# haliphinx/TCE-RVOS

Hardware: AMD Instinct MI355X
Metric: clips/s (T=5, 360×640, Swin-T) at 1/2/4/8 MI355X; mask IoU vs ref (higher is better)
Workload: dtype f32 (3xf16-split MFMA, f32 accumulate); 1 GPU; swin_t_p4w7 T=5 360x640 + 32-token text, B=1 clip per forward, flags --with_box_refine --binary --f_token 8 --qtrans (BASELINE config 2); clips_in_flight_per_gpu=1, clips_per_forward=1, same_clip_in_group=False, ranks_per_gpu=1, parallelism=clip-sharded x1

## Files before the change

### include/tce_rvos.h

```cpp
#ifndef TCE_RVOS_H
#define TCE_RVOS_H
#include <stdint.h>

#ifdef __cplusplus
extern "C" {
#endif

typedef void* tceStream;

int tce_abi_version(void);
const char* tce_last_error(void);

typedef struct {
  const float* A;
  const float* A2;
  const float* W;
  const float* bias;
  const float* res;
  float* C;
  int32_t M, N, K;
  int32_t lda, lda2, ldw, ldc, ldres;
  int32_t act, res_mode;
  int32_t batch;
  int64_t sA, sA2, sW, sBias, sC, sRes;
  int32_t conv;
  int32_t T, H, Wd, Cin, Ho, Wo, kh, kw, stride, pad;
} tceGemmArgs;
int tce_gemm_f32(const tceGemmArgs* args, tceStream stream);
int tce_gemm_splitk_f32(const tceGemmArgs* args, int32_t splits, float* workspace, tceStream stream);
int tce_gemm_splitk_ln_f32(const tceGemmArgs* args, int32_t splits, float* workspace, const float* gamma, const float* beta,
                           float eps, tceStream stream);
int tce_gemm_select_tile(int32_t M, int32_t N, int32_t batch);
int tce_gemm_select_tile_ex(int32_t M, int32_t N, int32_t K, int32_t batch, int32_t conv);
int tce_set_gemm_mode(int32_t mode);
int tce_get_gemm_mode(void);
int tce_set_gemm_mode_thread(int32_t mode);

int tce_set_range_flag(int32_t* flag);

int tce_layernorm_f32(const float* x, const float* r, const float* gamma, const float* beta, float* out,
                      int64_t M, int32_t C, float eps, tceStream stream);

int tce_groupnorm_nsplit(int32_t HW);
int tce_groupnorm_f32(const float* x, const float* gamma, const float* beta, float* out, float* ws, int32_t T,
                      int32_t HW, int32_t C, int32_t G, float eps, int32_t relu, tceStream stream);
int tce_groupnorm_up_add_f32(const float* x, const float* gamma, const float* beta, const float* add, float* out, float* ws,
                             int32_t T, int32_t h, int32_t w, int32_t ho, int32_t wo, int32_t C, int32_t G, float eps,
                             int32_t relu, tceStream stream);

int tce_resnet_stem_f32(const float* frames, const float* w_k64, const float* bias, float* out, int32_t T, int32_t H,
                        int32_t W, tceStream stream);
int tce_maxpool3x3s2_cl_f32(const float* x, float* out, int32_t T, int32_t H, int32_t W, int32_t C, tceStream stream);

int tce_patch_embed_f32(const float* frames, const float* w, const float* b, const float* gamma,
                        const float* beta, float* out, int32_t T, int32_t H, int32_t W, int32_t C, float eps,
                        tceStream stream);

int tce_window_attn_f32(const float* qkv, const float* qkv_bias, const float* bias_table, float* out, int32_t T,
                        int32_t H, int32_t W, int32_t C, int32_t nH, int32_t shift, tceStream stream);

int tce_window_attn3d_f32(const float* qkv, const float* qkv_bias, const float* bias_table, float* out, int32_t T,
                          int32_t H, int32_t W, int32_t C, int32_t nH, int32_t shifted, tceStream stream);

int tce_patch_merge_ln_f32(const float* x, const float* gamma, const float* beta, float* out, int32_t T, int32_t H,
                           int32_t W, int32_t C, float eps, tceStream stream);

int tce_mha_f32(const float* Q, const float* K, const float* V, float* O, int32_t batch, int32_t nheads,
                int32_t Lq, int32_t Lk, int32_t ldq, int32_t ldk, int32_t ldv, int32_t ldo, int64_t sQ, int64_t sK,
                int64_t sV, int64_t sO, const uint8_t* kmask, float scale, tceStream stream);

int64_t tce_mha_ws_bytes(int32_t batch, int32_t nheads, int32_t Lk);
int tce_mha_ws_f32(const float* Q, const float* K, const float* V, float* O, void* ws, int32_t batch, int32_t nheads,
                   int32_t Lq, int32_t Lk, int32_t ldq, int32_t ldk, int32_t ldv, int32_t ldo, int64_t sQ, int64_t sK,
                   int64_t sV, int64_t sO, const uint8_t* kmask, float scale, tceStream stream);

int tce_ms_deform_attn_forward_f32(const float* value, const int64_t* spatial_shapes, const int64_t* level_start_index,
                                   const float* sampling_loc, const float* attn_weight, float* out, int32_t N,
                                   int32_t S, int32_t M, int32_t D, int32_t Lq, int32_t L, int32_t P,
                                   tceStream stream);

int tce_ms_deform_attn_backward_f32(const float* value, const int64_t* spatial_shapes, const int64_t* level_start_index,
                                    const float* sampling_loc, const float* attn_weight, const float* grad_output,
                                    float* grad_value, float* grad_sampling_loc, float* grad_attn_weight, int32_t N,
                                    int32_t S, int32_t M, int32_t D, int32_t Lq, int32_t L, int32_t P, tceStream stream);

int tce_msda_fused_f32(const float* value, const float* proj, const float* ref, float* out,
                       const int32_t* shapes_hw , int32_t N, int32_t S, int32_t M, int32_t Lq,
                       int32_t L, int32_t P, int32_t ref_dim, int32_t ref_per_frame, tceStream stream);
int tce_msda_fused_valid_f32(const float* value, const float* proj, const float* ref, float* out,
                             const int32_t* shapes_hw, const int32_t* valid_hw, int32_t N, int32_t S, int32_t M, int32_t Lq,
                             int32_t L, int32_t P, int32_t ref_dim, int32_t ref_per_frame, tceStream stream);

int tce_msda_fewq_raw_f32(const float* src, const float* wv, const float* bv, const float* proj, const float* ref, float* out,
                          const int32_t* shapes_hw, const int32_t* valid_hw, int32_t N, int32_t S, int32_t M, int32_t Lq,
                          int32_t L, int32_t P, int32_t ref_dim, int32_t ref_per_frame, tceStream stream);

int tce_contrastive_f32(const float* memory, const float* sent, float* out, float* ws, int32_t T, int32_t S, int32_t C,
                        int32_t frames_per_clip, tceStream stream);

int tce_pos_sine2d_f32(float* out, const float* add, int32_t T, int32_t h, int32_t w, int32_t F, tceStream stream);
int tce_pos_sine2d_valid_f32(float* out, const float* add, int32_t T, int32_t h, int32_t w, int32_t F, int32_t hv, int32_t wv,
                             tceStream stream);

int tce_resize_nearest_f32(const float* in, const float* add, float* out, int32_t T, int32_t h, int32_t w, int32_t ho,
                           int32_t wo, int32_t C, tceStream stream);
int tce_resize_bilinear_f32(const float* in, const float* add, float* out, int32_t T, int32_t h, int32_t w,
                            int32_t ho, int32_t wo, int32_t C, tceStream stream);
int tce_resize_bilinear_ln_f32(const float* in, const float* add, const float* gamma, const float* beta, float eps, float* out,
                               int32_t T, int32_t h, int32_t w, int32_t ho, int32_t wo, int32_t C, tceStream stream);

int tce_add_f32(const float* a, const float* b, float* out, int64_t n, int64_t nb, tceStream stream);
int tce_tile_f32(const float* src, float* out, int64_t n_src, int64_t reps, tceStream stream);
int tce_sigmoid_f32(const float* x, float* out, int64_t n, tceStream stream);

#define TCE_COPY_MAX_SEGS 16
typedef struct tceCopySeg {
  const void* src;
  void* dst;
  int64_t rows, row_words, src_pitch_words;
} tceCopySeg;
int tce_copy_segments(const tceCopySeg* segs, int32_t n, tceStream stream);
int tce_box_refine_f32(const float* tmp, const float* ref, float* out, int32_t n, int32_t ref_dim, tceStream stream);

int tce_mask_pack_f32(const float* params, float* w0f, float* tail, int32_t nl, int32_t T, int32_t Q, int32_t Cm,
                      tceStream stream);
int tce_mask_tail_f32(const float* G, const float* tail, const float* refs , int32_t ref_ld,
                      float* masks, int32_t nl, int32_t T, int32_t Q, int32_t h, int32_t w, float img_h, float img_w,
                      int32_t stride_px, tceStream stream);

int tce_select_masks_u8(const float* logits, const float* masks, uint8_t* out, int32_t* best_query, int32_t T,
                        int32_t Q, int32_t K, int32_t h, int32_t w, int32_t H0, int32_t W0, float threshold,
                        tceStream stream);

int tce_resize_h_u8(const uint8_t* in, const int32_t* coef, const int32_t* bounds, uint8_t* tmp, int64_t rows,
                    int32_t Win, int32_t Wout, int32_t ksize, tceStream stream);
int tce_resize_v_norm_f32(const uint8_t* tmp, const int32_t* coef, const int32_t* bounds, const float* lut, float* out,
                          int32_t T, int32_t Hin, int32_t W, int32_t Hout, int32_t ksize, tceStream stream);

int tce_embed_ln_f32(const int64_t* ids, const int64_t* pos_ids, const float* word, const float* pos, const float* type0,
                     const float* gamma, const float* beta, float* out, int32_t L, int32_t C, float eps, int32_t pad_id,
                     tceStream stream);
int tce_embed_ln_seqs_f32(const int64_t* ids, const float* word, const float* pos, const float* type0, const float* gamma,
                          const float* beta, float* out, int32_t nseq, int32_t seq_len, int32_t C, float eps, int32_t pad_id,
                          tceStream stream);
int tce_mha_small64_f32(const float* qkv, float* out, int32_t L, int32_t nheads, float scale, tceStream stream);
int tce_tanh_f32(const float* x, float* out, int64_t n, tceStream stream);

int32_t tce_thin_linear_splits(int32_t M, int32_t N, int32_t K);
int tce_thin_partials_f32(const float* x, int64_t ldx, int32_t xsplits, const float* bias_x, int32_t act_x, const float* W,
                          int64_t ldw, float* ws, int32_t M, int32_t N, int32_t K, tceStream stream);
int tce_splitk_reduce_f32(const float* ws, int32_t splits, int32_t M, int32_t N, const float* bias, int32_t act, const float* res,
                          int32_t ldres, int32_t res_mode, float* C, int32_t ldc, const float* gamma, const float* beta, float eps,
                          tceStream stream);
int tce_mha_small64_splits_f32(const float* qkv_planes, int32_t splits, const float* bias, float* out, int32_t L, int32_t nheads,
                               float scale, tceStream stream);
int tce_mha_small64_seqs_f32(const float* qkv_planes, int32_t splits, const float* bias, float* out, int32_t nseq, int32_t L,
                             int32_t nheads, float scale, tceStream stream);
int tce_mha_small64_lens_f32(const float* qkv_planes, int32_t splits, const float* bias, float* out, int32_t nseq, int32_t L,
                             int32_t nheads, float scale, const int32_t* lens, tceStream stream);
int tce_caption_lens_f32(const int64_t* ids, int32_t nseq, int32_t Lmax, int32_t pad_id, int32_t D, int32_t* lens, uint8_t* kmask,
                         float* pos, tceStream stream);

int64_t tce_ffn_packed_bytes(int32_t C, int32_t Hd);
int tce_ffn_pack_f32(const float* W1, const float* b1, const float* W2, void* packed, int32_t C, int32_t Hd,
                     tceStream stream);
int tce_ffn_pack_batched_f32(const float* W1, const float* b1, const float* W2, void* packed, int32_t C, int32_t Hd,
                             int32_t batch, tceStream stream);
int tce_ffn_fused_f32(const float* x, int64_t ldx, const void* packed, const float* b2, const float* g_in,
                      const float* be_in, float eps_in, const float* g_out, const float* be_out, float eps_out,
                      float* out, int64_t ldo, int32_t M, int32_t C, int32_t Hd, int32_t act, tceStream stream);
int64_t tce_ffn_split_ws_floats(int32_t M, int32_t C, int32_t Hd, int32_t act);
int tce_ffn_set_wg_cap(int32_t cap);
int32_t tce_ffn_capped_grid(int32_t cap, int32_t batch, int32_t blocks, int32_t* persistent);
int32_t tce_ffn_split_counters(int32_t M, int32_t C, int32_t Hd, int32_t act);
int tce_ffn_fused_split_f32(const float* x, int64_t ldx, const void* packed, const float* b2, const float* g_in, const float* be_in,
                            float eps_in, const float* g_out, const float* be_out, float eps_out, float* out, int64_t ldo, int32_t M,
                            int32_t C, int32_t Hd, int32_t act, float* ws, int64_t ws_floats, int32_t* counters, int32_t n_counters,
                            tceStream stream);

typedef struct {
  const float* x;
  const float* a2;
  const void* packed;
  const float* bias;
  const float* res;
  float* out;
  const float *g_in, *be_in, *g_out, *be_out;
  int64_t ldx, lda2, ldres, ldo;
  int64_t sX, sA2, sRes, sOut;
  int32_t M, N, K, batch, a2_rows, act, res_mode;
  float eps_in, eps_out;
} tceRowLinArgs;
int64_t tce_rowlin_packed_bytes(int32_t N, int32_t K);
int tce_rowlin_pack_f32(const float* W, int64_t ldw, void* packed, int32_t N, int32_t K, tceStream stream);
int tce_rowlin_f32(const tceRowLinArgs* args, tceStream stream);

int64_t tce_conv3x3_packed_bytes(int32_t Cin, int32_t N);
int tce_conv3x3_pack_f32(const float* w, void* packed, int32_t Cin, int32_t N, tceStream stream);
int tce_conv3x3_f32(const float* x, int64_t ldx, const void* packed, const float* bias, float* out, int64_t ldo, int32_t T,
                    int32_t H, int32_t W, int32_t Cin, int32_t N, tceStream stream);
int64_t tce_conv3x3_split_ws_floats(int32_t M, int32_t Cin, int32_t N);
int32_t tce_conv3x3_split_pieces(int32_t M, int32_t Cin, int32_t N);
int32_t tce_conv3x3_split_kstep(int32_t pieces, int32_t s);
int tce_conv3x3_split_f32(const float* x, int64_t ldx, const void* packed, const float* bias, float* out, int64_t ldo, int32_t T,
                          int32_t H, int32_t W, int32_t Cin, int32_t N, float* ws, int64_t ws_floats, tceStream stream);

typedef struct {
  const float* x;
  const float* a2;
  const void* packed;
  const float* bo;
  const float* res;
  float* out;
  const float *g_out, *be_out;
  int64_t ldx, lda2, ldres, ldo;
  int64_t sX, sRes, sOut, sW;
  int32_t M, batch, a2_rows, res_mode, group;
  float eps_out;
  int32_t w_div;
} tceXattnArgs;
int tce_xattn_prepare_f32(const float* k, const float* v, const float* wqT_ext, const float* wo, float* W1, float* b1,
                          float* W2, int32_t L, int32_t group, int32_t batch, tceStream stream);
int tce_xattn_fused_f32(const tceXattnArgs* args, tceStream stream);

typedef struct {
  const void* packed;
  const float* b2;
  const float* g_out;
  const float* be_out;
  float* mid;
  int64_t ldmid, sMid;
  int32_t hidden, act;
  float eps_out;
} tceXattnFfnArgs;
int tce_ffn_pack_chain_f32(const float* W1, const float* b1, const float* W2, void* packed, int32_t C, int32_t Hd, tceStream stream);
int tce_xattn_ffn_fused_f32(const tceXattnArgs* args, const tceXattnFfnArgs* ffn, tceStream stream);
int tce_xattn_pack_f32(const float* k, const float* v, const float* wqT_ext, const float* wo, void* packed, int32_t L, int32_t group,
                       int32_t batch, tceStream stream);
int tce_xattn_prepare_lens_f32(const float* k, const float* v, const float* wqT_ext, const float* wo, float* W1, float* b1, float* W2,
                               int32_t L, int32_t group, int32_t batch, const int32_t* lens, tceStream stream);
int tce_xattn_pack_lens_f32(const float* k, const float* v, const float* wqT_ext, const float* wo, void* packed, int32_t L,
                            int32_t group, int32_t batch, const int32_t* lens, tceStream stream);

int64_t tce_swin_attn_packed_bytes(int32_t C);
int tce_swin_attn_pack_f32(const float* Wqkv, const float* Wproj, void* packed, int32_t C, tceStream stream);
int tce_swin_attn_fused_f32(const float* x, int64_t ldx, const void* packed, const float* qkv_bias, const float* proj_bias,
                            const float* bias_table, const float* gamma1, const float* beta1, float eps, float* out, int64_t ldo,
                            int32_t T, int32_t H, int32_t W, int32_t C, int32_t shift, tceStream stream);

int tce_graph_begin(tceStream stream);
int tce_graph_end(tceStream stream, void** graph_exec_out);
int tce_graph_launch(void* graph_exec, tceStream stream);
int tce_graph_destroy(void* graph_exec);
int tce_graph_group(void* const* graphs, int32_t n, void** graph_exec_out);

typedef struct {
  const float* W;
  const float* bias;
  float* out;
  int32_t N, ldw, ldo;
  int32_t use_a2;
  int32_t act;
} tceFewRowSeg;
typedef struct {
  const float* x;
  const float* a2;
  const float* res;
  int64_t ldx, lda2, ldres;
  int32_t a2_rows, R, K, nseg;
  tceFewRowSeg seg[3];
  const float* g_in;
  const float* be_in;
  float* xn_out;
  int64_t ldxn;
  float eps_in;
} tceFewRowArgs;
int tce_fewrow_linear_f32(const tceFewRowArgs* args, tceStream stream);

#ifdef __cplusplus
}
#endif
#endif
```

### tce-rvos_amd/_lib.py

```python
import ctypes as C
import os

HERE = os.path.dirname(os.path.abspath(__file__))
LIB_PATH = os.environ.get("TCE_LIB") or os.path.join(HERE, "lib", "libtce_rvos.so")

c_f = C.c_void_p
i32, i64, f32 = C.c_int32, C.c_int64, C.c_float


class GemmArgs(C.Structure):
    _fields_ = [("A", c_f), ("A2", c_f), ("W", c_f), ("bias", c_f), ("res", c_f), ("C", c_f),
                ("M", i32), ("N", i32), ("K", i32),
                ("lda", i32), ("lda2", i32), ("ldw", i32), ("ldc", i32), ("ldres", i32),
                ("act", i32), ("res_mode", i32), ("batch", i32),
                ("sA", i64), ("sA2", i64), ("sW", i64), ("sBias", i64), ("sC", i64), ("sRes", i64),
                ("conv", i32), ("T", i32), ("H", i32), ("Wd", i32), ("Cin", i32), ("Ho", i32), ("Wo", i32),
                ("kh", i32), ("kw", i32), ("stride", i32), ("pad", i32)]


class RowLinArgs(C.Structure):
    _fields_ = [("x", c_f), ("a2", c_f), ("packed", c_f), ("bias", c_f), ("res", c_f), ("out", c_f),
                ("g_in", c_f), ("be_in", c_f), ("g_out", c_f), ("be_out", c_f),
                ("ldx", i64), ("lda2", i64), ("ldres", i64), ("ldo", i64),
                ("sX", i64), ("sA2", i64), ("sRes", i64), ("sOut", i64),
                ("M", i32), ("N", i32), ("K", i32), ("batch", i32), ("a2_rows", i32), ("act", i32), ("res_mode", i32),
                ("eps_in", f32), ("eps_out", f32)]


class XattnArgs(C.Structure):
    _fields_ = [("x", c_f), ("a2", c_f), ("packed", c_f), ("bo", c_f), ("res", c_f), ("out", c_f),
                ("g_out", c_f), ("be_out", c_f),
                ("ldx", i64), ("lda2", i64), ("ldres", i64), ("ldo", i64),
                ("sX", i64), ("sRes", i64), ("sOut", i64), ("sW", i64),
                ("M", i32), ("batch", i32), ("a2_rows", i32), ("res_mode", i32), ("group", i32), ("eps_out", f32), ("w_div", i32)]



class XattnFfnArgs(C.Structure):
    _fields_ = [("packed", c_f), ("b2", c_f), ("g_out", c_f), ("be_out", c_f), ("mid", c_f), ("ldmid", i64), ("sMid", i64),
                ("hidden", i32), ("act", i32), ("eps_out", f32)]


class FewRowSeg(C.Structure):
    _fields_ = [("W", c_f), ("bias", c_f), ("out", c_f), ("N", i32), ("ldw", i32), ("ldo", i32), ("use_a2", i32), ("act", i32)]


class FewRowArgs(C.Structure):
    _fields_ = [("x", c_f), ("a2", c_f), ("res", c_f),
                ("ldx", i64), ("lda2", i64), ("ldres", i64),
                ("a2_rows", i32), ("R", i32), ("K", i32), ("nseg", i32), ("seg", FewRowSeg * 3),
                ("g_in", c_f), ("be_in", c_f), ("xn_out", c_f), ("ldxn", i64), ("eps_in", f32)]


class CopySeg(C.Structure):
    _fields_ = [("src", c_f), ("dst", c_f), ("rows", i64), ("row_words", i64), ("src_pitch_words", i64)]


class LabelObj(C.Structure):
    _fields_ = [("logits", c_f), ("masks", c_f)]


A2D_GROUP_MAX = 16


class A2dGroupSample(C.Structure):
    _fields_ = [("masks", c_f), ("logits", c_f), ("out", c_f), ("scores", c_f), ("fh", i32), ("fw", i32), ("H0", i32), ("W0", i32),
                ("logit_stride", i32), ("reserved", i32)]


REFEXP_GROUP_MAX = 16
REFEXP_MAX_CAND = 1024


class RefexpSample(C.Structure):
    _fields_ = [("logits", c_f), ("boxes_in", c_f), ("masks", c_f), ("scores", c_f), ("order", c_f), ("boxes_out", c_f), ("out", c_f),
                ("fh", i32), ("fw", i32), ("H0", i32), ("W0", i32)]


SIGNATURES = {
    "tce_abi_version": (i32, []),
    "tce_last_error": (C.c_char_p, []),
    "tce_gemm_f32": (i32, [C.POINTER(GemmArgs), c_f]),
    "tce_gemm_splitk_f32": (i32, [C.POINTER(GemmArgs), i32, c_f, c_f]),
    "tce_gemm_splitk_ln_f32": (i32, [C.POINTER(GemmArgs), i32, c_f, c_f, c_f, f32, c_f]),
    "tce_gemm_select_tile": (i32, [i32, i32, i32]),
    "tce_gemm_select_tile_ex": (i32, [i32, i32, i32, i32, i32]),
    "tce_set_gemm_mode": (i32, [i32]),
    "tce_set_gemm_mode_thread": (i32, [i32]),
    "tce_set_range_flag": (i32, [c_f]),
    "tce_get_gemm_mode": (i32, []),
    "tce_layernorm_f32": (i32, [c_f, c_f, c_f, c_f, c_f, i64, i32, f32, c_f]),
    "tce_groupnorm_nsplit": (i32, [i32]),
    "tce_groupnorm_f32": (i32, [c_f, c_f, c_f, c_f, c_f, i32, i32, i32, i32, f32, i32, c_f]),
    "tce_groupnorm_up_add_f32": (i32, [c_f, c_f, c_f, c_f, c_f, c_f, i32, i32, i32, i32, i32, i32, i32, f32, i32, c_f]),
    "tce_resnet_stem_f32": (i32, [c_f, c_f, c_f, c_f, i32, i32, i32, c_f]),
    "tce_maxpool3x3s2_cl_f32": (i32, [c_f, c_f, i32, i32, i32, i32, c_f]),
    "tce_resize_h_u8": (i32, [c_f, c_f, c_f, c_f, i64, i32, i32, i32, c_f]),
    "tce_resize_v_norm_f32": (i32, [c_f, c_f, c_f, c_f, c_f, i32, i32, i32, i32, i32, c_f]),
    "tce_patch_embed_f32": (i32, [c_f, c_f, c_f, c_f, c_f, c_f, i32, i32, i32, i32, f32, c_f]),
    "tce_window_attn_f32": (i32, [c_f, c_f, c_f, c_f, i32, i32, i32, i32, i32, i32, c_f]),
    "tce_window_attn3d_f32": (i32, [c_f, c_f, c_f, c_f, i32, i32, i32, i32, i32, i32, c_f]),
    "tce_patch_merge_ln_f32": (i32, [c_f, c_f, c_f, c_f, i32, i32, i32, i32, f32, c_f]),
    "tce_mha_f32": (i32, [c_f, c_f, c_f, c_f, i32, i32, i32, i32, i32, i32, i32, i32, i64, i64, i64, i64, c_f, f32, c_f]),
    "tce_mha_ws_bytes": (i64, [i32, i32, i32]),
    "tce_mha_ws_f32": (i32, [c_f, c_f, c_f, c_f, c_f, i32, i32, i32, i32, i32, i32, i32, i32, i64, i64, i64, i64, c_f, f32, c_f]),
    "tce_ms_deform_attn_forward_f32": (i32, [c_f, c_f, c_f, c_f, c_f, c_f, i32, i32, i32, i32, i32, i32, i32, c_f]),
    "tce_ms_deform_attn_backward_f32": (i32, [c_f, c_f, c_f, c_f, c_f, c_f, c_f, c_f, c_f, i32, i32, i32, i32, i32, i32, i32, c_f]),
    "tce_msda_fused_f32": (i32, [c_f, c_f, c_f, c_f, C.POINTER(i32), i32, i32, i32, i32, i32, i32, i32, i32, c_f]),
    "tce_msda_fused_valid_f32": (i32, [c_f, c_f, c_f, c_f, C.POINTER(i32), C.POINTER(i32), i32, i32, i32, i32, i32, i32, i32,
                                       i32, c_f]),
    "tce_msda_fewq_raw_f32": (i32, [c_f, c_f, c_f, c_f, c_f, c_f, C.POINTER(i32), C.POINTER(i32), i32, i32, i32, i32, i32, i32, i32,
                                    i32, c_f]),
    "tce_contrastive_f32": (i32, [c_f, c_f, c_f, c_f, i32, i32, i32, i32, c_f]),
    "tce_pos_sine2d_f32": (i32, [c_f, c_f, i32, i32, i32, i32, c_f]),
    "tce_pos_sine2d_valid_f32": (i32, [c_f, c_f, i32, i32, i32, i32, i32, i32, c_f]),
    "tce_resize_nearest_f32": (i32, [c_f, c_f, c_f, i32, i32, i32, i32, i32, i32, c_f]),
    "tce_resize_bilinear_f32": (i32, [c_f, c_f, c_f, i32, i32, i32, i32, i32, i32, c_f]),
    "tce_resize_bilinear_ln_f32": (i32, [c_f, c_f, c_f, c_f, f32, c_f, i32, i32, i32, i32, i32, i32, c_f]),
    "tce_add_f32": (i32, [c_f, c_f, c_f, i64, i64, c_f]),
    "tce_tile_f32": (i32, [c_f, c_f, i64, i64, c_f]),
    "tce_sigmoid_f32": (i32, [c_f, c_f, i64, c_f]),
    "tce_copy_segments": (i32, [C.POINTER(CopySeg), i32, c_f]),
    "tce_box_refine_f32": (i32, [c_f, c_f, c_f, i32, i32, c_f]),
    "tce_mask_pack_f32": (i32, [c_f, c_f, c_f, i32, i32, i32, i32, c_f]),
    "tce_mask_tail_f32": (i32, [c_f, c_f, c_f, i32, c_f, i32, i32, i32, i32, i32, f32, f32, i32, c_f]),
    "tce_select_masks_u8": (i32, [c_f, c_f, c_f, c_f, i32, i32, i32, i32, i32, i32, i32, f32, c_f]),
    "tce_embed_ln_f32": (i32, [c_f, c_f, c_f, c_f, c_f, c_f, c_f, c_f, i32, i32, f32, i32, c_f]),
    "tce_mha_small64_f32": (i32, [c_f, c_f, i32, i32, f32, c_f]),
    "tce_mha_small64_seqs_f32": (i32, [c_f, i32, c_f, c_f, i32, i32, i32, f32, c_f]),
    "tce_embed_ln_seqs_f32": (i32, [c_f, c_f, c_f, c_f, c_f, c_f, c_f, i32, i32, i32, f32, i32, c_f]),
    "tce_mha_small64_lens_f32": (i32, [c_f, i32, c_f, c_f, i32, i32, i32, f32, c_f, c_f]),
    "tce_caption_lens_f32": (i32, [c_f, i32, i32, i32, i32, c_f, c_f, c_f, c_f]),
    "tce_tanh_f32": (i32, [c_f, c_f, i64, c_f]),
    "tce_ffn_packed_bytes": (i64, [i32, i32]),
    "tce_ffn_pack_f32": (i32, [c_f, c_f, c_f, c_f, i32, i32, c_f]),
    "tce_ffn_fused_f32": (i32, [c_f, i64, c_f, c_f, c_f, c_f, f32, c_f, c_f, f32, c_f, i64, i32, i32, i32, i32, c_f]),
    "tce_ffn_split_ws_floats": (i64, [i32, i32, i32, i32]),
    "tce_ffn_split_counters": (i32, [i32, i32, i32, i32]),
    "tce_ffn_set_wg_cap": (i32, [i32]),
    "tce_ffn_capped_grid": (i32, [i32, i32, i32, C.POINTER(i32)]),
    "tce_ffn_fused_split_f32": (i32, [c_f, i64, c_f, c_f, c_f, c_f, f32, c_f, c_f, f32, c_f, i64, i32, i32, i32, i32, c_f, i64, c_f, i32, c_f]),
    "tce_xattn_prepare_f32": (i32, [c_f, c_f, c_f, c_f, c_f, c_f, c_f, i32, i32, i32, c_f]),
    "tce_ffn_pack_batched_f32": (i32, [c_f, c_f, c_f, c_f, i32, i32, i32, c_f]),
    "tce_xattn_fused_f32": (i32, [C.POINTER(XattnArgs), c_f]),
    "tce_xattn_ffn_fused_f32": (i32, [C.POINTER(XattnArgs), C.POINTER(XattnFfnArgs), c_f]),
    "tce_ffn_pack_chain_f32": (i32, [c_f, c_f, c_f, c_f, i32, i32, c_f]),
    "tce_xattn_pack_f32": (i32, [c_f, c_f, c_f, c_f, c_f, i32, i32, i32, c_f]),
    "tce_xattn_prepare_lens_f32": (i32, [c_f, c_f, c_f, c_f, c_f, c_f, c_f, i32, i32, i32, c_f, c_f]),
    "tce_xattn_pack_lens_f32": (i32, [c_f, c_f, c_f, c_f, c_f, i32, i32, i32, c_f, c_f]),
    "tce_rowlin_packed_bytes": (i64, [i32, i32]),
    "tce_rowlin_pack_f32": (i32, [c_f, i64, c_f, i32, i32, c_f]),
    "tce_rowlin_f32": (i32, [C.POINTER(RowLinArgs), c_f]),
    "tce_conv3x3_packed_bytes": (i64, [i32, i32]),
    "tce_conv3x3_pack_f32": (i32, [c_f, c_f, i32, i32, c_f]),
    "tce_conv3x3_f32": (i32, [c_f, i64, c_f, c_f, c_f, i64, i32, i32, i32, i32, i32, c_f]),
    "tce_conv3x3_split_ws_floats": (i64, [i32, i32, i32]),
    "tce_conv3x3_split_pieces": (i32, [i32, i32, i32]),
    "tce_conv3x3_split_kstep": (i32, [i32, i32]),
    "tce_conv3x3_split_f32": (i32, [c_f, i64, c_f, c_f, c_f, i64, i32, i32, i32, i32, i32, c_f, i64, c_f]),
    "tce_fewrow_linear_f32": (i32, [C.POINTER(FewRowArgs), c_f]),
    "tce_thin_linear_splits": (i32, [i32, i32, i32]),
    "tce_thin_partials_f32": (i32, [c_f, i64, i32, c_f, i32, c_f, i64, c_f, i32, i32, i32, c_f]),
    "tce_splitk_reduce_f32": (i32, [c_f, i32, i32, i32, c_f, i32, c_f, i32, i32, c_f, i32, c_f, c_f, f32, c_f]),
    "tce_mha_small64_splits_f32": (i32, [c_f, i32, c_f, c_f, i32, i32, f32, c_f]),
    "tce_swin_attn_packed_bytes": (i64, [i32]),
    "tce_swin_attn_pack_f32": (i32, [c_f, c_f, c_f, i32, c_f]),
    "tce_swin_attn_fused_f32": (i32, [c_f, i64, c_f, c_f, c_f, c_f, c_f, c_f, f32, c_f, i64, i32, i32, i32, i32, i32, c_f]),
    "tce_graph_begin": (i32, [c_f]),
    "tce_graph_end": (i32, [c_f, C.POINTER(C.c_void_p)]),
    "tce_graph_launch": (i32, [C.c_void_p, c_f]),
    "tce_graph_destroy": (i32, [C.c_void_p]),
    "tce_graph_group": (i32, [C.POINTER(C.c_void_p), i32, C.POINTER(C.c_void_p)]),
}

DEBUG_SIGNATURES = {
    "tce_gemm_force_tile": (i32, [i32]),
    "tce_debug_set_stamp_buffer": (i32, [c_f]),
    "tce_debug_set_epilogue": (i32, [i32]),
    "tce_debug_ffn_set_stamp_buffer": (i32, [c_f]),
    "tce_debug_ffn_set_half": (i32, [i32]),
    "tce_debug_msda_set_lds": (i32, [i32]),
    "tce_debug_window_attn_set_mfma": (i32, [i32]),
    "tce_debug_mha_set_split": (i32, [i32]),
    "tce_debug_msda_set_fewq": (i32, [i32]),
    "tce_debug_conv3x3_set_waves": (i32, [i32]),
    "tce_debug_conv3x3_set_pieces": (i32, [i32]),
}

VIDEO_SIGNATURES = {
    "tce_label_objects_u8": (i32, [C.POINTER(LabelObj), i32, c_f, c_f, i32, i32, i32, i32, i32, i32, i32, f32, f32, c_f]),
}

EVAL_SIGNATURES = {
    "tce_a2d_masks_u8": (i32, [c_f, c_f, i32, i32, i32, i32, i32, i32, i32, f32, c_f]),
    "tce_rle_ws_bytes": (i64, [i32, i32, i32]),
    "tce_rle_counts_u32": (i32, [c_f, c_f, c_f, c_f, i32, i32, i32, c_f]),
    "tce_a2d_group_masks_u8": (i32, [C.POINTER(A2dGroupSample), i32, i32, i32, i32, f32, c_f]),
}

SCORE_SIGNATURES = {
    "tce_jf_ws_bytes": (i64, [i32, i32, i32, i32, i32]),
    "tce_jf_counts_i32": (i32, [c_f, c_f, c_f, c_f, i32, i32, i32, i32, i32, c_f]),
    "tce_rle_decode_ws_bytes": (i64, [i32, i32, i32, i32]),
    "tce_rle_decode_u8": (i32, [c_f, c_f, c_f, c_f, i32, i32, i32, i32, c_f]),
    "tce_mask_overlap_ws_bytes": (i64, [i32, i32, i32]),
    "tce_mask_overlap_i32": (i32, [c_f, c_f, c_f, c_f, i32, i32, i32, c_f]),
}

PNG_SIGNATURES = {
    "tce_png_stream_bound": (i64, [i32, i32, i32]),
    "tce_png_ws_bytes": (i64, [i32, i32, i32, i32]),
    "tce_png_deflate_u8": (i32, [c_f, c_f, c_f, c_f, i32, i32, i32, i32, i32, c_f]),
    "tce_png_deflate_dyn_u8": (i32, [c_f, c_f, c_f, c_f, i32, i32, i32, i32, i32, c_f]),
}

VIS_SIGNATURES = {
    "tce_vis_overlay_u8": (i32, [c_f, c_f, c_f, c_f, c_f, c_f, i32, i32, i32, i32, c_f]),
    "tce_png_filter_rgb_u8": (i32, [c_f, c_f, i32, i32, i32, c_f]),
    "tce_png_deflate_rows_u8": (i32, [c_f, c_f, c_f, c_f, i32, i32, i32, i32, c_f]),
}

PNGFILE_SIGNATURES = {
    "tce_png_file_bound": (i64, [i32, i64]),
    "tce_png_file_ws_bytes": (i64, [i32, i64]),
    "tce_png_file_u8": (i32, [c_f, c_f, c_f, i32, c_f, c_f, c_f, i32, i64, i64, c_f]),
}

REFEXP_SIGNATURES = {
    "tce_refexp_group_u8": (i32, [C.POINTER(RefexpSample), i32, i32, i32, i32, i32, f32, c_f]),
    "tce_refexp_giou_f32": (i32, [c_f, c_f, c_f, c_f, i32, i32, c_f]),
}

HEADERS = {"tce_rvos.h": SIGNATURES, "tce_rvos_debug.h": DEBUG_SIGNATURES, "tce_rvos_video.h": VIDEO_SIGNATURES,
           "tce_rvos_eval.h": EVAL_SIGNATURES, "tce_rvos_score.h": SCORE_SIGNATURES, "tce_rvos_png.h": PNG_SIGNATURES,
           "tce_rvos_vis.h": VIS_SIGNATURES, "tce_rvos_pngfile.h": PNGFILE_SIGNATURES, "tce_rvos_refexp.h": REFEXP_SIGNATURES}

_LIB = None


class TceError(RuntimeError):
    pass


def lib():
    global _LIB
    if _LIB is None:
        if not os.path.exists(LIB_PATH):
            raise TceError(f"{LIB_PATH} not found: build the HIP extension first "
                           f"(python -c 'import __graft_entry__ as g; g.build()'); there is no fallback path")
        hwq = os.environ.get("GPU_MAX_HW_QUEUES")
        if hwq not in (None, "", "4"):
            import warnings
            warnings.warn(f"tce_rvos_amd: GPU_MAX_HW_QUEUES={hwq} is set; the HIP runtime's default (4) is the only value this "
                          f"launch program runs well with (1-3 crash the runtime, 5-16 double the clip time)", RuntimeWarning)
        l = C.CDLL(LIB_PATH)
        for name, (res, args) in [kv for table in HEADERS.values() for kv in table.items()]:
            fn = getattr(l, name)
            fn.restype, fn.argtypes = res, args
        _LIB = l
    return _LIB


def lib_raw():
    l = lib()
    return l.__dict__.get("_real", l)


def check(status, what=""):
    if status != 0:
        msg = lib().tce_last_error().decode(errors="replace")
        raise TceError(f"{what} failed ({status}): {msg}")
```

### tce-rvos_amd/csrc/conv3x3.hip

```cpp
#include "common.h"
#include "gemm_epilogue.h"
#include "frag.h"
#include "tiles.h"
#include "../../include/tce_rvos.h"
#include "../../include/tce_rvos_debug.h"

namespace {

constexpr int CONV_PAD_STAGES = 6;

struct ConvArgs {
  const float* x;
  const unsigned char* wpk;
  const float* bias;
  float* out;
  long long ldx, ldo;
  int H, W, M;
  int* range_flag;
  int single;
  int m_off;
  int nb, pieces;
  float* ws;
};

constexpr int CONV_ITERS = 12;
__host__ __device__ constexpr int conv3x3_piece_iter(const int pieces, const int s) { return s * CONV_ITERS / pieces; }

#ifndef CONV_ABL
#define CONV_ABL 0
#endif

template <int BYTE_OFF>
__device__ __forceinline__ void gload16(f32x4& dst, const float* ptr) {
  asm volatile("global_load_dwordx4 %0, %1, off offset:%2" : "=v"(dst) : "v"(ptr), "n"(BYTE_OFF) : "memory");
}

template <int CIN, bool SINGLE, int WAVES = 4, bool SPLIT = false>
__global__ void __launch_bounds__(64 * WAVES, WAVES / 4) conv3x3_kernel(const ConvArgs p) {
  constexpr int NTL = 8;
  constexpr int PW = 16 / WAVES;
  constexpr int STAGE = 2 * NTL * PIECE;
  constexpr int R = 4;
  constexpr int XS = WAVES == 4 ? 6 : 4, LX = XS + 1;
  constexpr int NW = WAVES == 4 ? CONV_PAD_STAGES - 2 : 3, LW = NW + 2;
  constexpr int INFLIGHT = (2 + PW) * (LW - 3);
  static_assert(LW <= CONV_PAD_STAGES, "the packed stream's zero padding covers the weight lead");
  constexpr int BODY = 12;
  constexpr int ITERS = 3 * (CIN / 64);
  constexpr int KS = BODY * ITERS;
  static_assert(CIN % 64 == 0, "channel chunks come in groups of four");
  static_assert(BODY % R == 0 && BODY % XS == 0 && BODY % NW == 0 && LX >= LW, "ring positions are compile-time");
  static_assert(WAVES * WT_BYTES <= R * STAGE, "the epilogue's staging tiles alias the ring");
  static_assert(!SPLIT || (ITERS == CONV_ITERS && WAVES == 4 && !SINGLE), "split pieces: CIN = 256, 128-pixel workgroups, split fp16");
  __shared__ __attribute__((aligned(16))) unsigned char smem[R * STAGE];

  const int tid = threadIdx.x, lane = tid & 63;
  const int wave = __builtin_amdgcn_readfirstlane(tid >> 6);
  const int hf = lane >> 5;
  const int blk = SPLIT ? (int)blockIdx.x % p.nb : (int)blockIdx.x;
  const int piece = SPLIT ? (int)blockIdx.x / p.nb : 0;
  const int i0 = SPLIT ? conv3x3_piece_iter(p.pieces, piece) : 0;
  const int i1 = SPLIT ? conv3x3_piece_iter(p.pieces, piece + 1) : ITERS;
  const int m0 = p.m_off + blk * (32 * WAVES) + wave * 32;

  const int m = m0 + (lane & 31);
  const int px = m % p.W, py = (m / p.W) % p.H;
  const float* const zeros = reinterpret_cast<const float*>(p.wpk + (long long)(KS + CONV_PAD_STAGES) * STAGE) + 8 * hf;
  const float* const xme = p.x + (long long)min(m, p.M - 1) * p.ldx + 8 * hf;
  auto iter_ptrs = [&](const int it, const float* (&q)[3]) {
    const int dy = it / (CIN / 64) - 1, cq = it % (CIN / 64);
    const bool row_ok = it < i1 && m < p.M && (unsigned)(py + dy) < (unsigned)p.H;
#pragma unroll
    for (int d = 0; d < 3; ++d) {
      const bool ok = row_ok && (unsigned)(px + d - 1) < (unsigned)p.W;
      q[d] = (ok ? xme + (long long)(dy * p.W + d - 1) * p.ldx : zeros) + 64 * cq;
    }
  };

  const float* wp = reinterpret_cast<const float*>(p.wpk + ((long long)i0 * BODY * STAGE) + (long long)(PW * wave) * PIECE + lane * 16);
  unsigned char* const wdst = smem + (PW * wave) * PIECE + lane * 16;
  f32x4 wr[NW][PW];
  auto wload = [&](f32x4 (&dst)[PW]) {
    if (!(CONV_ABL & 8)) {
      gload16<0>(dst[0], wp);
      gload16<PIECE>(dst[1], wp);
      if constexpr (PW == 4) {
        gload16<2 * PIECE>(dst[2], wp);
        gload16<3 * PIECE>(dst[3], wp);
      }
    }
    wp += STAGE / 4;
  };
  auto wstore = [&](const f32x4 (&src)[PW], const int stage) {
#pragma unroll
    for (int q = 0; q < PW; ++q) *reinterpret_cast<f32x4*>(wdst + stage * STAGE + q * PIECE) = src[q];
  };

  f32x4 xr[XS][2];
  const float* cur[3];
  const float* nxt[3];
  iter_ptrs(i0, cur);
  iter_ptrs(i0 + 1, nxt);
  auto xload = [&](auto jjc, f32x4 (&dst)[2]) {
    constexpr int JJ = decltype(jjc)::value;
    constexpr int J = JJ % BODY;
    const float* const src = JJ < BODY ? cur[J % 3] : nxt[J % 3];
    if (CONV_ABL & 16) return;
    gload16<64 * (J / 3)>(dst[0], src);
    gload16<64 * (J / 3) + 16>(dst[1], src);
  };
  auto wait_loads = [&](auto nc, f32x4 (&xs)[2], f32x4 (&ws)[PW]) {
    constexpr int N = (CONV_ABL & 24) ? 0 : decltype(nc)::value;
    if constexpr (PW == 4) {
      asm volatile("s_waitcnt vmcnt(%6)"
                   : "+v"(xs[0]), "+v"(xs[1]), "+v"(ws[0]), "+v"(ws[1]), "+v"(ws[2]), "+v"(ws[3])
                   : "n"(N)
                   : "memory");
    } else {
      asm volatile("s_waitcnt vmcnt(%4)" : "+v"(xs[0]), "+v"(xs[1]), "+v"(ws[0]), "+v"(ws[1]) : "n"(N) : "memory");
    }
  };
  using nfl = std::integral_constant<int, INFLIGHT>;

  f32x16 acc[NTL];
#pragma unroll
  for (int t = 0; t < NTL; ++t)
#pragma unroll
    for (int i = 0; i < 16; ++i) acc[t][i] = 0.f;
  h16x8 bh, bl;
  static_for<0, LX>([&](auto mc) {
    constexpr int m = decltype(mc)::value - LX;
    if constexpr (m + 2 >= 0) {
      wait_loads(nfl{}, xr[(m + 2) % XS], wr[(m + 2) % NW]);
      wstore(wr[(m + 2) % NW], (m + 2) % R);
      if constexpr (m + 2 == 0) {
        const float f[8] = {xr[0][0][0], xr[0][0][1], xr[0][0][2], xr[0][0][3], xr[0][1][0], xr[0][1][1], xr[0][1][2], xr[0][1][3]};
        const HL b = split8(f, SINGLE ? 1 : 0);
        bh = b.hi;
        bl = b.lo;
        asm volatile("" : "+v"(bh), "+v"(bl));
      }
    }
    if constexpr (m + LX >= 0) xload(std::integral_constant<int, m + LX>{}, xr[(m + LX) % XS]);
    if constexpr (m + LW >= 0) wload(wr[(m + LW) % NW]);
  });
  __syncthreads();
  h16x8 fh[4], fl[4];
  {
    const unsigned char* const st = smem + lane * 16;
    fh[0] = *reinterpret_cast<const h16x8*>(st);
    fl[0] = *reinterpret_cast<const h16x8*>(st + PIECE);
    fh[1] = *reinterpret_cast<const h16x8*>(st + 2 * PIECE);
    fl[1] = *reinterpret_cast<const h16x8*>(st + 3 * PIECE);
  }

  for (int it = i0; it < i1; ++it) {
    static_for<0, BODY>([&](auto jc) {
      constexpr int j = decltype(jc)::value;
      constexpr int nslot = (j + 1) % XS;
      const unsigned char* const st = smem + (j % R) * STAGE + lane * 16;
      unsigned nh[4], nl[4];
      auto tile = [&](auto tc) {
        constexpr int t = decltype(tc)::value;
#if CONV_ABL & 4
        const h16x8 k0 = fh[t % 4], k1 = fl[t % 4], k2 = bh, k3 = bl;
        asm volatile("" : : "v"(k0), "v"(k1), "v"(k2), "v"(k3));
#else
        if constexpr (!SINGLE) {
          acc[t] = __builtin_amdgcn_mfma_f32_32x32x16_f16(fh[t % 4], bl, acc[t], 0, 0, 0);
          acc[t] = __builtin_amdgcn_mfma_f32_32x32x16_f16(fl[t % 4], bh, acc[t], 0, 0, 0);
        }
        acc[t] = __builtin_amdgcn_mfma_f32_32x32x16_f16(fh[t % 4], bh, acc[t], 0, 0, 0);
#endif
      };
      static_for<0, 6>([&](auto tc) {
        constexpr int t = decltype(tc)::value;
        fh[(t + 2) % 4] = *reinterpret_cast<const h16x8*>(st + (2 * t + 4) * PIECE);
        fl[(t + 2) % 4] = *reinterpret_cast<const h16x8*>(st + (2 * t + 5) * PIECE);
        __builtin_amdgcn_sched_barrier(0);
        tile(tc);
        if constexpr (t < 4) {
          const float a = xr[nslot][t >> 1][2 * (t & 1)], b = xr[nslot][t >> 1][2 * (t & 1) + 1];
          if constexpr (SINGLE) {
            nh[t] = __builtin_bit_cast(unsigned, fp16x2_t{(__fp16)a, (__fp16)b});
            nl[t] = 0u;
          } else {
            const fp16x2_t h = __builtin_amdgcn_cvt_pkrtz(a, b);
            nh[t] = __builtin_bit_cast(unsigned, h);
            nl[t] = __builtin_bit_cast(unsigned, __builtin_amdgcn_cvt_pkrtz(a - (float)h[0], b - (float)h[1]));
          }
          asm volatile("" : "+v"(nh[t]), "+v"(nl[t]));
        }
        __builtin_amdgcn_sched_barrier(0);
      });
      wait_loads(nfl{}, xr[(j + 2) % XS], wr[(j + 2) % NW]);
      wstore(wr[(j + 2) % NW], (j + 2) % R);
      if (!(CONV_ABL & 2)) __syncthreads();
      xload(std::integral_constant<int, j + LX>{}, xr[(j + LX) % XS]);
      wload(wr[(j + LW) % NW]);
      {
        const unsigned char* const sn = smem + ((j + 1) % R) * STAGE + lane * 16;
        fh[0] = *reinterpret_cast<const h16x8*>(sn);
        fl[0] = *reinterpret_cast<const h16x8*>(sn + PIECE);
        fh[1] = *reinterpret_cast<const h16x8*>(sn + 2 * PIECE);
        fl[1] = *reinterpret_cast<const h16x8*>(sn + 3 * PIECE);
      }
      __builtin_amdgcn_sched_barrier(0);
      tile(std::integral_constant<int, 6>{});
      tile(std::integral_constant<int, 7>{});
      __builtin_amdgcn_sched_barrier(0);
      bh = __builtin_bit_cast(h16x8, u32x4{nh[0], nh[1], nh[2], nh[3]});
      bl = __builtin_bit_cast(h16x8, u32x4{nl[0], nl[1], nl[2], nl[3]});
    });
#pragma unroll
    for (int d = 0; d < 3; ++d) cur[d] = nxt[d];
    iter_ptrs(it + 2, nxt);
  }
  asm volatile("s_waitcnt vmcnt(0)" ::: "memory");
  __syncthreads();

  float* const wt = reinterpret_cast<float*>(smem + wave * WT_BYTES);
  tce_amax_t amax = 0;
  if constexpr (SPLIT) {
    float* const part = p.ws + (long long)piece * (p.M - p.m_off) * 256;
#pragma unroll
    for (int t = 0; t < NTL; ++t) tile_store(acc[t], part, 256, m0 - p.m_off, p.M - p.m_off, 32 * t, wt, lane, amax);
    return;
  }
  const ResTile none = {};
#pragma unroll
  for (int t = 0; t < NTL; ++t) {
    tile_bias_res<0>(acc[t], tile_bias_load(p.bias, 32 * t, lane), none, wt, lane);
    tile_store(acc[t], p.out, p.ldo, m0, p.M, 32 * t, wt, lane, amax);
  }
  tce_range_report(p.range_flag, amax);
}

__global__ void __launch_bounds__(256) conv3x3_reduce_kernel(const float* __restrict__ ws, const int pieces, const int rows,
                                                             const float* __restrict__ bias, float* __restrict__ out,
                                                             const long long ldo, const int m_off, int* range_flag) {
  const long long n4 = (long long)rows * 64, stride = (long long)gridDim.x * 256;
  tce_amax_t amax = 0;
  for (long long i = (long long)blockIdx.x * 256 + threadIdx.x; i < n4; i += stride) {
    const f32x4* src = reinterpret_cast<const f32x4*>(ws) + i;
    f32x4 v = src[0];
    for (int s = 1; s < pieces; ++s) v += src[(long long)s * n4];
    const int c4 = (int)(i & 63);
    if (bias) v += reinterpret_cast<const f32x4*>(bias)[c4];
    amax = tce_amax4(amax, v);
    *reinterpret_cast<f32x4*>(out + (m_off + (i >> 6)) * ldo + 4 * c4) = v;
  }
  tce_range_report(range_flag, amax);
}

__global__ void __launch_bounds__(256) conv3x3_pack_kernel(const float* __restrict__ w, unsigned char* __restrict__ out,
                                                           const int CIN, const long long units, const int single) {
  const long long u = (long long)blockIdx.x * 256 + threadIdx.x;
  if (u >= units) return;
  const int lane = (int)(u & 63);
  const long long pg = u >> 6;
  const int piece = (int)(pg & 15);
  const long long s = pg >> 4;
  const int r = lane & 31, hf = lane >> 5, t = piece >> 1;
  u32x4 o = {0u, 0u, 0u, 0u};
  if (s < 9 * CIN / 16) {
    const int it = (int)(s / 12), j = (int)(s % 12);
    const int dy = it / (CIN / 64), cc = 4 * (it % (CIN / 64)) + j / 3, dx = j % 3;
    float v[8];
#pragma unroll
    for (int e = 0; e < 8; ++e) v[e] = w[(long long)(32 * t + r) * (9 * CIN) + (3 * dy + dx) * CIN + 16 * cc + 8 * hf + e];
    const HL f = split8(v, single);
    o = __builtin_bit_cast(u32x4, (piece & 1) ? f.lo : f.hi);
  }
  reinterpret_cast<u32x4*>(out)[u] = o;
}

inline bool conv3x3_shape_ok(int Cin, int N) { return Cin == 256 && N == 256; }
inline long long conv3x3_units(int Cin) { return (long long)(9 * Cin / 16 + CONV_PAD_STAGES) * 16 * 64 + 128; }

}

extern "C" int64_t tce_conv3x3_packed_bytes(int32_t Cin, int32_t N) { return conv3x3_shape_ok(Cin, N) ? conv3x3_units(Cin) * 16 : -1; }

extern "C" int tce_conv3x3_pack_f32(const float* w, void* packed, int32_t Cin, int32_t N, tceStream stream) {
  TCE_CHECK_ARG(conv3x3_shape_ok(Cin, N), "tce_conv3x3_pack_f32: unsupported shape Cin=%d N=%d (256 -> 256)", Cin, N);
  TCE_CHECK_ARG(w && packed && tce_aligned16(packed), "tce_conv3x3_pack_f32: null / misaligned pointer");
  const long long units = conv3x3_units(Cin);
  hipLaunchKernelGGL(conv3x3_pack_kernel, dim3(tce_cdiv(units, 256)), dim3(256), 0, (hipStream_t)stream, w,
                     (unsigned char*)packed, Cin, units, tce_gemm_single_pass());
  TCE_CHECK_LAUNCH("tce_conv3x3_pack_f32");
  return TCE_OK;
}

static int g_conv3_waves = 0;
extern "C" int tce_debug_conv3x3_set_waves(int32_t waves) {
  TCE_CHECK_ARG(waves == 0 || waves == 4 || waves == 8, "tce_debug_conv3x3_set_waves: 0 (automatic), 4 or 8");
  g_conv3_waves = waves;
  return TCE_OK;
}

struct Conv3Plan {
  int wide = 4;
  int full8 = 0;
  int m_narrow = 0;
  int nb = 0;
  int pieces = 1;
  long long ws_floats = 0;
};
inline Conv3Plan conv3x3_plan(const int M, const int cus, const int single, const int force_waves, const int split, const int force_pieces) {
  Conv3Plan pl;
  const int r4 = tce_cdiv(tce_cdiv(M, 128), cus), r8 = tce_cdiv(tce_cdiv(M, 256), cus);
  const int full8 = tce_cdiv(M, 256) / cus;
  const int rem_px = M - full8 * 256 * cus;
  const int mixed4 = 7 * full8 + 4 * tce_cdiv(tce_cdiv(rem_px, 128), cus);
  if (!force_waves && !single && full8 >= 1 && rem_px > 0 && mixed4 < 4 * r4 && mixed4 < 7 * r8) {
    pl.full8 = full8 * cus;
    pl.m_narrow = full8 * 256 * cus;
  } else {
    pl.wide = force_waves ? force_waves : (4 * r4 > 7 * r8 ? 8 : 4);
    if (single) pl.wide = 4;
    if (pl.wide == 8) return pl;
  }
  pl.nb = tce_cdiv(M - pl.m_narrow, 128);
  if (!split || single || pl.nb >= cus) return pl;
  const double OVH = 0.5, LAUNCH = 0.3, RED_BPI = 8.0 * (3u << 20);
  const long long px = M - pl.m_narrow;
  auto cost = [&](int p) {
    const double walk = (double)tce_cdiv((long long)pl.nb * p, cus) * (tce_cdiv(CONV_ITERS, p) + OVH);
    return p == 1 ? walk : walk + LAUNCH + (double)(p + 1) * px * 1024.0 / RED_BPI;
  };
  int best = 1;
  for (int p = 2; p <= 6; ++p)
    if ((long long)pl.nb * p <= 2ll * cus && cost(p) < cost(best)) best = p;
  if (force_pieces > 0) best = force_pieces;
  if (best > 1) {
    pl.pieces = best;
    pl.ws_floats = (long long)best * px * 256;
  }
  return pl;
}

static int g_conv3_pieces = 0;
extern "C" int tce_debug_conv3x3_set_pieces(int32_t pieces) {
  TCE_CHECK_ARG(pieces >= 0 && pieces <= CONV_ITERS, "tce_debug_conv3x3_set_pieces: 0 (automatic) .. 12");
  g_conv3_pieces = pieces;
  return TCE_OK;
}

static int conv3_force_waves() {
  static const int env_force = []() { const char* e = getenv("TCE_CONV3_WAVES"); return e ? atoi(e) : 0; }();
  return g_conv3_waves ? g_conv3_waves : env_force;
}

static Conv3Plan conv3x3_plan_for(const int M, const bool split) {
  return conv3x3_plan(M, tce_cu_count(), tce_gemm_single_pass(), conv3_force_waves(), split, g_conv3_pieces);
}

extern "C" int64_t tce_conv3x3_split_ws_floats(int32_t M, int32_t Cin, int32_t N) {
  return conv3x3_shape_ok(Cin, N) && M > 0 ? conv3x3_plan_for(M, true).ws_floats : 0;
}
extern "C" int32_t tce_conv3x3_split_pieces(int32_t M, int32_t Cin, int32_t N) {
  return conv3x3_shape_ok(Cin, N) && M > 0 ? conv3x3_plan_for(M, true).pieces : 0;
}
extern "C" int32_t tce_conv3x3_split_kstep(int32_t pieces, int32_t s) {
  return pieces >= 1 && pieces <= CONV_ITERS && s >= 0 && s <= pieces ? 12 * conv3x3_piece_iter(pieces, s) : -1;
}

static int conv3x3_launch(const float* x, int64_t ldx, const void* packed, const float* bias, float* out, int64_t ldo, int32_t T,
                          int32_t H, int32_t W, int32_t Cin, int32_t N, float* ws, int64_t ws_floats, const bool split, tceStream stream,
                          const char* name) {
  TCE_CHECK_ARG(conv3x3_shape_ok(Cin, N), "%s: unsupported shape Cin=%d N=%d (256 -> 256)", name, Cin, N);
  TCE_CHECK_ARG(x && packed && out && T > 0 && H > 0 && W > 0 && (long long)T * H * W < (1ll << 31),
                "%s: null pointer or bad sizes", name);
  TCE_CHECK_ARG(ldx >= Cin && ldx % 4 == 0 && ldo >= N && ldo % 4 == 0, "%s: bad row pitch", name);
  TCE_CHECK_ARG(tce_aligned16(x) && tce_aligned16(out) && tce_aligned16(packed) && (!bias || tce_aligned16(bias)),
                "%s: pointers must be 16-byte aligned", name);
  ConvArgs a;
  a.x = x; a.wpk = (const unsigned char*)packed; a.bias = bias; a.out = out;
  a.ldx = ldx; a.ldo = ldo; a.H = H; a.W = W; a.M = T * H * W;
  a.range_flag = tce_range_flag(); a.single = tce_gemm_single_pass();
  a.m_off = 0; a.nb = 0; a.pieces = 1; a.ws = nullptr;
  hipStream_t s = (hipStream_t)stream;
  const Conv3Plan pl = conv3x3_plan_for(a.M, split);
  if (pl.pieces > 1)
    TCE_CHECK_ARG(ws && tce_aligned16(ws) && ws_floats >= pl.ws_floats,
                  "%s: workspace of %lld floats needed (tce_conv3x3_split_ws_floats), %lld given", name, pl.ws_floats, (long long)ws_floats);
  if (pl.full8) hipLaunchKernelGGL((conv3x3_kernel<256, false, 8>), dim3(pl.full8), dim3(512), 0, s, a);
  a.m_off = pl.m_narrow;
  if (pl.wide == 8) hipLaunchKernelGGL((conv3x3_kernel<256, false, 8>), dim3(tce_cdiv(a.M, 256)), dim3(512), 0, s, a);
  else if (a.single) hipLaunchKernelGGL((conv3x3_kernel<256, true>), dim3(pl.nb), dim3(256), 0, s, a);
  else if (pl.pieces == 1) hipLaunchKernelGGL((conv3x3_kernel<256, false>), dim3(pl.nb), dim3(256), 0, s, a);
  else {
    a.nb = pl.nb; a.pieces = pl.pieces; a.ws = ws;
    hipLaunchKernelGGL((conv3x3_kernel<256, false, 4, true>), dim3(pl.nb * pl.pieces), dim3(256), 0, s, a);
    const int rows = a.M - a.m_off;
    hipLaunchKernelGGL(conv3x3_reduce_kernel, dim3(std::min(tce_cdiv((long long)rows * 64, 256), 8 * tce_cu_count())), dim3(256), 0, s,
                       (const float*)ws, pl.pieces, rows, bias, out, ldo, a.m_off, a.range_flag);
  }
  TCE_CHECK_LAUNCH(name);
  return TCE_OK;
}

extern "C" int tce_conv3x3_f32(const float* x, int64_t ldx, const void* packed, const float* bias, float* out, int64_t ldo,
                               int32_t T, int32_t H, int32_t W, int32_t Cin, int32_t N, tceStream stream) {
  return conv3x3_launch(x, ldx, packed, bias, out, ldo, T, H, W, Cin, N, nullptr, 0, false, stream, "tce_conv3x3_f32");
}

extern "C" int tce_conv3x3_split_f32(const float* x, int64_t ldx, const void* packed, const float* bias, float* out, int64_t ldo,
                                     int32_t T, int32_t H, int32_t W, int32_t Cin, int32_t N, float* ws, int64_t ws_floats,
                                     tceStream stream) {
  return conv3x3_launch(x, ldx, packed, bias, out, ldo, T, H, W, Cin, N, ws, ws_floats, true, stream, "tce_conv3x3_split_f32");
}
```

### tce-rvos_amd/csrc/norm.hip

```cpp
#include "common.h"
#include "gemm_epilogue.h"
#include "../../include/tce_rvos.h"

namespace {

__global__ void __launch_bounds__(256) layernorm_kernel(const float* __restrict__ x, const float* __restrict__ r,
                                                        const float* __restrict__ gamma,
                                                        const float* __restrict__ beta, float* __restrict__ out,
                                                        long long M, int C, float eps) {
  const int lane = threadIdx.x & 63;
  const long long row = (long long)blockIdx.x * 4 + (threadIdx.x >> 6);
  if (row >= M) return;
  const f32x4* xr = reinterpret_cast<const f32x4*>(x + row * C);
  const f32x4* rr = r ? reinterpret_cast<const f32x4*>(r + row * C) : nullptr;
  const int n4 = C >> 2;
  float s = 0.f;
  for (int i = lane; i < n4; i += 64) {
    f32x4 v = xr[i];
    if (rr) v += rr[i];
    s += (v[0] + v[1]) + (v[2] + v[3]);
  }
  const float mean = wave_sum(s) / (float)C;
  float q = 0.f;
  for (int i = lane; i < n4; i += 64) {
// ... 401 lines not shown
        sMean[g] = mean;
        sRstd[g] = rsqrtf(m2 / n + eps);
      }
    }
  }
  __syncthreads();
  for (int c = threadIdx.x; c < C; c += 256) {
    const int g = c / cg;
    const float mean = sMean[g], rstd = sRstd[g];
    const float sc = rstd * gamma[c];
    scale[c] = sc;
    shift[c] = beta[c] - mean * sc;
  }
  __syncthreads();
}

__global__ void __launch_bounds__(256) groupnorm_apply_kernel(const float* __restrict__ x,
                                                              const float* __restrict__ ws,
                                                              const float* __restrict__ gamma,
                                                              const float* __restrict__ beta, float* __restrict__ out,
                                                              int HW, int C, int G, int relu, int rows_per_block,
                                                              int nsplit, float eps) {
  extern __shared__ float sm[];
  float* scale = sm;
  float* shift = sm + C;
  const int t = blockIdx.y;
  groupnorm_scale_shift(ws, gamma, beta, scale, shift, t, C, G, nsplit, eps);
  const int c4 = C >> 2;
  const long long r0 = (long long)blockIdx.x * rows_per_block;
  const long long r1 = min((long long)HW, r0 + rows_per_block);
  const f32x4* x4 = reinterpret_cast<const f32x4*>(x + (long long)t * HW * C);
  f32x4* o4 = reinterpret_cast<f32x4*>(out + (long long)t * HW * C);
  const f32x4* sc4 = reinterpret_cast<const f32x4*>(scale);
  const f32x4* sh4 = reinterpret_cast<const f32x4*>(shift);
  for (long long i = r0 * c4 + threadIdx.x; i < r1 * c4; i += 256) {
    const int c = (int)(i % c4);
    const f32x4 v = x4[i], a = sc4[c], b = sh4[c];
    f32x4 o;
#pragma unroll
    for (int j = 0; j < 4; ++j) {
      o[j] = v[j] * a[j] + b[j];
      if (relu) o[j] = fmaxf(o[j], 0.f);
    }
    o4[i] = o;
  }
}

__global__ void __launch_bounds__(256) groupnorm_apply_up_kernel(const float* __restrict__ x, const float* __restrict__ ws,
                                                                 const float* __restrict__ gamma, const float* __restrict__ beta,
                                                                 const float* add, float* out, int h, int w, int ho, int wo,
                                                                 int C, int G, int relu, int rows_per_block, int nsplit, float eps) {
  extern __shared__ float sm[];
  float* scale = sm;
  float* shift = sm + C;
  const int t = blockIdx.y;
  groupnorm_scale_shift(ws, gamma, beta, scale, shift, t, C, G, nsplit, eps);
  const int c4 = C >> 2;
  const long long HWo = (long long)ho * wo;
  const long long r0 = (long long)blockIdx.x * rows_per_block;
  const long long r1 = min(HWo, r0 + rows_per_block);
  const f32x4* x4 = reinterpret_cast<const f32x4*>(x + (long long)t * h * w * C);
  const f32x4* a4 = reinterpret_cast<const f32x4*>(add + (long long)t * HWo * C);
  f32x4* o4 = reinterpret_cast<f32x4*>(out + (long long)t * HWo * C);
  const f32x4* sc4 = reinterpret_cast<const f32x4*>(scale);
  const f32x4* sh4 = reinterpret_cast<const f32x4*>(shift);
  const float sy = (float)h / (float)ho, sx = (float)w / (float)wo;
  for (long long i = r0 * c4 + threadIdx.x; i < r1 * c4; i += 256) {
    const int c = (int)(i % c4);
    const int ro = (int)(i / c4);
    const int yo = ro / wo, xo = ro - yo * wo;
    const int yi = min((int)floorf((float)yo * sy), h - 1), xi = min((int)floorf((float)xo * sx), w - 1);
    const f32x4 v = x4[((long long)yi * w + xi) * c4 + c], a = sc4[c], b = sh4[c];
    f32x4 o;
#pragma unroll
    for (int j = 0; j < 4; ++j) {
      o[j] = v[j] * a[j] + b[j];
      if (relu) o[j] = fmaxf(o[j], 0.f);
    }
    o += a4[i];
    o4[i] = o;
  }
}


}

extern "C" int tce_layernorm_f32(const float* x, const float* r, const float* gamma, const float* beta, float* out,
                                 int64_t M, int32_t C, float eps, tceStream stream) {
  TCE_CHECK_ARG(x && gamma && beta && out, "tce_layernorm_f32: null pointer");
  TCE_CHECK_ARG(M > 0 && C > 0 && C % 4 == 0, "tce_layernorm_f32: need M>0, C%%4==0 (M=%lld C=%d)", (long long)M, C);
  TCE_CHECK_ARG(tce_aligned16(x) && tce_aligned16(out) && tce_aligned16(gamma) && tce_aligned16(beta) &&
                    (!r || tce_aligned16(r)),
                "tce_layernorm_f32: pointers must be 16-byte aligned");
  if (C <= 128)
    hipLaunchKernelGGL(layernorm_reg_kernel<32>, dim3(tce_cdiv(M, 8)), dim3(256), 0, (hipStream_t)stream, x, r, gamma, beta,
                       out, (long long)M, C, eps);
  else if (C <= 256)
    hipLaunchKernelGGL(layernorm_reg_kernel<64>, dim3(tce_cdiv(M, 4)), dim3(256), 0, (hipStream_t)stream, x, r, gamma, beta,
                       out, (long long)M, C, eps);
  else
    hipLaunchKernelGGL(layernorm_kernel, dim3(tce_cdiv(M, 4)), dim3(256), 0, (hipStream_t)stream, x, r, gamma, beta, out,
                     (long long)M, C, eps);
  TCE_CHECK_LAUNCH("tce_layernorm_f32");
  return TCE_OK;
}

extern "C" int tce_patch_merge_ln_f32(const float* x, const float* gamma, const float* beta, float* out, int32_t T,
                                      int32_t H, int32_t W, int32_t C, float eps, tceStream stream) {
  TCE_CHECK_ARG(x && gamma && beta && out, "tce_patch_merge_ln_f32: null pointer");
  TCE_CHECK_ARG(T > 0 && H > 0 && W > 0 && C > 0 && C % 4 == 0, "tce_patch_merge_ln_f32: bad shape");
  TCE_CHECK_ARG(tce_aligned16(x) && tce_aligned16(out) && tce_aligned16(gamma) && tce_aligned16(beta),
                "tce_patch_merge_ln_f32: pointers must be 16-byte aligned");
  const long long rows = (long long)T * ((H + 1) / 2) * ((W + 1) / 2);
  hipLaunchKernelGGL(patch_merge_ln_kernel, dim3(tce_cdiv(rows, 4)), dim3(256), 0, (hipStream_t)stream, x, gamma, beta,
                     out, T, H, W, C, eps);
  TCE_CHECK_LAUNCH("tce_patch_merge_ln_f32");
  return TCE_OK;
}

extern "C" int tce_patch_embed_f32(const float* frames, const float* w, const float* b, const float* gamma,
                                   const float* beta, float* out, int32_t T, int32_t H, int32_t W, int32_t C, float eps,
                                   tceStream stream) {
  TCE_CHECK_ARG(frames && w && b && gamma && beta && out, "tce_patch_embed_f32: null pointer");
  TCE_CHECK_ARG(T > 0 && H > 0 && W > 0 && C > 0 && C <= 256, "tce_patch_embed_f32: need 0 < C <= 256 (C=%d)", C);
  const int Hp = (H + 3) / 4, Wp = (W + 3) / 4;
  const long long ntok = (long long)T * Hp * Wp;
  if (tce_get_gemm_mode() != 0 &&
      tce_patch_embed_mfma(frames, w, b, gamma, beta, out, H, W, C, eps, ntok, Hp, Wp, (hipStream_t)stream)) {
    TCE_CHECK_LAUNCH("tce_patch_embed_f32");
    return TCE_OK;
  }
  int* const rf = tce_get_gemm_mode() != 0 ? tce_range_flag() : nullptr;
  if (C % 8 == 0 && C <= 120 && tce_aligned16(frames) && tce_aligned16(out) && tce_aligned16(gamma) && tce_aligned16(beta)) {
    constexpr int TOK = 128;
    const size_t lds = (size_t)(TOK * (C + 4) + 2 * TOK) * sizeof(float);
    hipLaunchKernelGGL((patch_embed_lane_kernel<8, TOK>), dim3(tce_cdiv(ntok, TOK)), dim3(TOK), lds, (hipStream_t)stream, frames, w, b,
                       gamma, beta, out, H, W, C, eps, ntok, Hp, Wp, rf);
    TCE_CHECK_LAUNCH("tce_patch_embed_f32");
    return TCE_OK;
  }
  const int tpb = 64;
  const size_t smem = (size_t)(48 * C + 4 * 48) * sizeof(float);
  hipLaunchKernelGGL((patch_embed_kernel<4>), dim3(tce_cdiv(ntok, tpb)), dim3(256), smem, (hipStream_t)stream, frames, w,
                     b, gamma, beta, out, T, H, W, C, eps, tpb, rf);
  TCE_CHECK_LAUNCH("tce_patch_embed_f32");
  return TCE_OK;
}

static int groupnorm_rows_per(int HW) { return HW >= 4096 ? 128 : (HW >= 512 ? 32 : 8); }
extern "C" int tce_groupnorm_nsplit(int32_t HW) { return tce_cdiv(HW, groupnorm_rows_per(HW)); }

static void groupnorm_stats_launch(const float* x, float* ws, int T, int HW, int C, int G, hipStream_t s);

extern "C" int tce_groupnorm_up_add_f32(const float* x, const float* gamma, const float* beta, const float* add, float* out,
                                        float* ws, int32_t T, int32_t h, int32_t w, int32_t ho, int32_t wo, int32_t C, int32_t G,
                                        float eps, int32_t relu, tceStream stream) {
  TCE_CHECK_ARG(x && gamma && beta && add && out && ws, "tce_groupnorm_up_add_f32: null pointer");
  TCE_CHECK_ARG(T > 0 && h > 0 && w > 0 && ho > 0 && wo > 0 && C > 0 && G > 0 && G <= 64 && C % G == 0 && C % 4 == 0,
                "tce_groupnorm_up_add_f32: bad shape (G <= 64)");
  TCE_CHECK_ARG(tce_aligned16(x) && tce_aligned16(out) && tce_aligned16(add), "tce_groupnorm_up_add_f32: x/add/out must be 16-byte aligned");
  TCE_CHECK_ARG(x != out, "tce_groupnorm_up_add_f32: out may alias add, not x");
  const int HW = h * w, nsplit = tce_cdiv(HW, groupnorm_rows_per(HW));
  hipStream_t s = (hipStream_t)stream;
  groupnorm_stats_launch(x, ws, T, HW, C, G, s);
  const int rows_per_block = 64;
  hipLaunchKernelGGL(groupnorm_apply_up_kernel, dim3(tce_cdiv(ho * wo, rows_per_block), T), dim3(256), (size_t)2 * C * sizeof(float), s,
                     x, ws, gamma, beta, add, out, h, w, ho, wo, C, G, relu, rows_per_block, nsplit, eps);
  TCE_CHECK_LAUNCH("tce_groupnorm_up_add_f32");
  return TCE_OK;
}

static void groupnorm_stats_launch(const float* x, float* ws, int T, int HW, int C, int G, hipStream_t s) {
  const int rows_per = groupnorm_rows_per(HW), nsplit = tce_cdiv(HW, rows_per);
  if (C == 256 && (G == 8 || G == 16 || G == 32 || G == 64)) {
    const dim3 grid(nsplit, T);
    if (rows_per == 128) hipLaunchKernelGGL(groupnorm_stats_rows_kernel<32>, grid, dim3(256), 0, s, x, ws, HW, G, rows_per, nsplit);
    else if (rows_per == 32) hipLaunchKernelGGL(groupnorm_stats_rows_kernel<8>, grid, dim3(256), 0, s, x, ws, HW, G, rows_per, nsplit);
    else hipLaunchKernelGGL(groupnorm_stats_rows_kernel<2>, grid, dim3(256), 0, s, x, ws, HW, G, rows_per, nsplit);
  } else {
    hipLaunchKernelGGL(groupnorm_stats_kernel, dim3(T * G, nsplit), dim3(256), 0, s, x, ws, HW, C, G, nsplit);
  }
}

extern "C" int tce_groupnorm_f32(const float* x, const float* gamma, const float* beta, float* out, float* ws, int32_t T,
                                 int32_t HW, int32_t C, int32_t G, float eps, int32_t relu, tceStream stream) {
  TCE_CHECK_ARG(x && gamma && beta && out && ws, "tce_groupnorm_f32: null pointer");
  TCE_CHECK_ARG(T > 0 && HW > 0 && C > 0 && G > 0 && G <= 64 && C % G == 0 && C % 4 == 0, "tce_groupnorm_f32: bad shape (G <= 64)");
  TCE_CHECK_ARG(tce_aligned16(x) && tce_aligned16(out), "tce_groupnorm_f32: x/out must be 16-byte aligned");
  const int rows_per = groupnorm_rows_per(HW), nsplit = tce_cdiv(HW, rows_per);
  hipStream_t s = (hipStream_t)stream;
  if (C == 256 && (G == 8 || G == 16 || G == 32 || G == 64)) {
    const dim3 grid(nsplit, T);
    if (rows_per == 128) hipLaunchKernelGGL(groupnorm_stats_rows_kernel<32>, grid, dim3(256), 0, s, x, ws, HW, G, rows_per, nsplit);
    else if (rows_per == 32) hipLaunchKernelGGL(groupnorm_stats_rows_kernel<8>, grid, dim3(256), 0, s, x, ws, HW, G, rows_per, nsplit);
    else hipLaunchKernelGGL(groupnorm_stats_rows_kernel<2>, grid, dim3(256), 0, s, x, ws, HW, G, rows_per, nsplit);
  } else {
    hipLaunchKernelGGL(groupnorm_stats_kernel, dim3(T * G, nsplit), dim3(256), 0, s, x, ws, HW, C, G, nsplit);
  }
  const int rows_per_block = 64;
  hipLaunchKernelGGL(groupnorm_apply_kernel, dim3(tce_cdiv(HW, rows_per_block), T), dim3(256),
                     (size_t)2 * C * sizeof(float), s, x, ws, gamma, beta, out, HW, C, G, relu, rows_per_block, nsplit, eps);
  TCE_CHECK_LAUNCH("tce_groupnorm_f32");
  return TCE_OK;
}
```

### tce-rvos_amd/hazard.py

```python
import contextlib
import traceback

import numpy as np
import torch

from . import _lib

F = 4


def strided(ptr, run_bytes, *dims):
    if not ptr or run_bytes <= 0 or any(c <= 0 for c, _ in dims):
        return np.zeros((0, 2), dtype=np.int64)
    starts = np.array([int(ptr)], dtype=np.int64)
    for count, stride in dims:
        if count == 1 or stride == 0:
            continue
        starts = (starts[:, None] + (np.arange(int(count), dtype=np.int64) * int(stride))[None, :]).reshape(-1)
    iv = np.stack([starts, starts + int(run_bytes)], 1)
    return merge(iv)


def dense(ptr, nbytes):
    return strided(ptr, int(nbytes))
# ... 50 lines not shown

def _table(ptr, what):
    n = TABLES.get(_p(ptr))
    if n is None:
        raise RuntimeError(f"hazard checker: the extent of {what} at {_p(ptr):#x} is unknown (hazard.recording(tables=...))")
    return dense(_p(ptr), n)


def _gemm(g, ws=None, splits=1, ln=None):
    b = max(1, g.batch)
    if g.conv:
        rd = [dense(_p(g.A), g.T * g.H * g.Wd * g.Cin * F)]
    else:
        rd = [strided(_p(g.A), g.K * F, (b, g.sA * F), (g.M, g.lda * F))]
        if g.A2:
            rd.append(strided(_p(g.A2), g.K * F, (b, g.sA2 * F), (g.M, g.lda2 * F)))
    rd.append(strided(_p(g.W), g.K * F, (b, g.sW * F), (g.N, g.ldw * F)))
    if g.bias:
        rd.append(strided(_p(g.bias), g.N * F, (b, g.sBias * F)))
    if g.res and g.res_mode:
        rd.append(strided(_p(g.res), g.N * F, (b, g.sRes * F), (g.M, g.ldres * F)))
    wr = [strided(_p(g.C), g.N * F, (b, g.sC * F), (g.M, g.ldc * F))]
    if ws:
        w = dense(_p(ws), splits * g.M * g.N * F)
        rd.append(w)
        wr.append(w)
    if ln:
        rd += [dense(_p(ln[0]), g.N * F), dense(_p(ln[1]), g.N * F)]
    return rd, wr


def _rowlin(q):
    b = max(1, q.batch)
    L = _lib.lib_raw()
    rd = [strided(_p(q.x), q.K * F, (b, q.sX * F), (q.M, q.ldx * F)),
          dense(_p(q.packed), L.tce_rowlin_packed_bytes(q.N, q.K))]
    if q.a2:
        rd.append(strided(_p(q.a2), q.K * F, (b, q.sA2 * F), (q.a2_rows if q.a2_rows > 0 else q.M, q.lda2 * F)))
    if q.bias:
        rd.append(dense(_p(q.bias), q.N * F))
    if q.res and q.res_mode:
        rd.append(strided(_p(q.res), q.N * F, (b, q.sRes * F), (q.M, q.ldres * F)))
    for g_, n in ((q.g_in, q.K), (q.be_in, q.K), (q.g_out, q.N), (q.be_out, q.N)):
        if g_:
            rd.append(dense(_p(g_), n * F))
    return rd, [strided(_p(q.out), q.N * F, (b, q.sOut * F), (q.M, q.ldo * F))]


def _xattn(q):
    b = max(1, q.batch)
    L = _lib.lib_raw()
    nb = L.tce_ffn_packed_bytes(256, 8 * q.group)
    wd = q.w_div if q.w_div > 0 else 1
    rd = [strided(_p(q.x), 256 * F, (b, q.sX * F), (q.M, q.ldx * F)),
          strided(_p(q.packed), nb, ((b + wd - 1) // wd if q.sW else 1, q.sW)), dense(_p(q.bo), 256 * F)]
    if q.a2:
        rd.append(strided(_p(q.a2), 256 * F, (q.a2_rows if q.a2_rows > 0 else q.M, q.lda2 * F)))
    if q.res:
        rd.append(strided(_p(q.res), 256 * F, (b, q.sRes * F), (q.M, q.ldres * F)))
    for g_ in (q.g_out, q.be_out):
        if g_:
            rd.append(dense(_p(g_), 256 * F))
    return rd, [strided(_p(q.out), 256 * F, (b, q.sOut * F), (q.M, q.ldo * F))]


def _xattn_ffn(q, f):
    rd, wr = _xattn(q)
    b = max(1, q.batch)
    rd += [dense(_p(f.packed), _lib.lib_raw().tce_ffn_packed_bytes(256, f.hidden)), dense(_p(f.b2), 256 * F)]
    for g_ in (f.g_out, f.be_out):
        if g_:
            rd.append(dense(_p(g_), 256 * F))
    wr.append(strided(_p(f.mid), 256 * F, (b, f.sMid * F), (q.M, f.ldmid * F)))
    return rd, wr


def _fewrow(q):
    rd = [strided(_p(q.x), q.K * F, (q.R, q.ldx * F))]
    wr = []
    use_a2 = False
    for i in range(q.nseg):
        sg = q.seg[i]
        rd.append(strided(_p(sg.W), q.K * F, (sg.N, sg.ldw * F)))
        if sg.bias:
            rd.append(dense(_p(sg.bias), sg.N * F))
        wr.append(strided(_p(sg.out), sg.N * F, (q.R, sg.ldo * F)))
        use_a2 = use_a2 or bool(sg.use_a2)
    if q.a2 and use_a2:
        rd.append(strided(_p(q.a2), q.K * F, (q.a2_rows if q.a2_rows > 0 else q.R, q.lda2 * F)))
    if q.res:
        rd.append(strided(_p(q.res), q.seg[0].N * F, (q.R, q.ldres * F)))
    if q.g_in:
        rd += [dense(_p(q.g_in), q.K * F), dense(_p(q.be_in), q.K * F)]
        if q.xn_out:
            wr.append(strided(_p(q.xn_out), q.K * F, (q.R, q.ldxn * F)))
    return rd, wr


def _mha(Q, K, V, O, ws, batch, nh, Lq, Lk, ldq, ldk, ldv, ldo, sQ, sK, sV, sO, kmask):
    run = nh * 32 * F
    rd = [strided(_p(Q), run, (batch, sQ * F), (Lq, ldq * F)), strided(_p(K), run, (batch, sK * F), (Lk, ldk * F)),
          strided(_p(V), run, (batch, sV * F), (Lk, ldv * F))]
    if kmask:
        rd.append(dense(_p(kmask), batch * Lk))
    wr = [strided(_p(O), run, (batch, sO * F), (Lq, ldo * F))]
    if ws:
        w = dense(_p(ws), _lib.lib_raw().tce_mha_ws_bytes(batch, nh, Lk))
        rd.append(w)
        wr.append(w)
    return rd, wr


def _msda(value, proj, ref, out, N, S, M, Lq, L, P, ref_dim, ref_per_frame):
    return ([dense(_p(value), N * S * M * 32 * F), dense(_p(proj), N * Lq * M * L * P * 3 * F),
             dense(_p(ref), (N if ref_per_frame else 1) * Lq * ref_dim * F)], [dense(_p(out), N * Lq * M * 32 * F)])


def _copy_segments(a):
    segs, n = a[0], a[1]
    rd, wr = [], []
    for i in range(n):
        sg = segs[i]
        rd.append(strided(_p(sg.src), sg.row_words * 4, (sg.rows, sg.src_pitch_words * 4)))
        wr.append(dense(_p(sg.dst), sg.rows * sg.row_words * 4))
    return rd, wr


def _ffn_fused(a):
    x, ldx, packed, b2, g_in, be_in, _, g_out, be_out, _, out, ldo, M, Cn, Hd = a[:15]
    rd = [strided(_p(x), Cn * F, (M, ldx * F)), dense(_p(packed), _lib.lib_raw().tce_ffn_packed_bytes(Cn, Hd)),
          dense(_p(b2), Cn * F)]
    for g_ in (g_in, be_in, g_out, be_out):
        if g_:
            rd.append(dense(_p(g_), Cn * F))
    return rd, [strided(_p(out), Cn * F, (M, ldo * F))]


def _ffn_fused_split(a):
    rd, wr = _ffn_fused(a)
    ws, ws_floats, cnt, ncnt = a[16:20]
    return rd + [dense(_p(cnt), ncnt * 4)], wr + [dense(_p(ws), ws_floats * F), dense(_p(cnt), ncnt * 4)]


def _ffn_pack(a, batched):
    W1, b1, W2, packed, Cn, Hd = a[:6]
    b = a[6] if batched else 1
    nb = _lib.lib_raw().tce_ffn_packed_bytes(Cn, Hd)
    rd = [dense(_p(W1), b * Hd * Cn * F), dense(_p(W2), b * Hd * Cn * F)]
    if b1:
        rd.append(dense(_p(b1), b * Hd * F))
    return rd, [dense(_p(packed), b * nb)]


def _groupnorm(a):
    x, gamma, beta, out, ws, T, HW, Cn, G = a[:9]
    nsplit = _lib.lib_raw().tce_groupnorm_nsplit(HW)
    w = dense(_p(ws), T * G * (nsplit * 3 + 2) * F)
    return ([dense(_p(x), T * HW * Cn * F), dense(_p(gamma), Cn * F), dense(_p(beta), Cn * F), w],
            [dense(_p(out), T * HW * Cn * F), w])


def _groupnorm_up_add(a):
    x, gamma, beta, add, out, ws, T, h, w_, ho, wo, Cn, G = a[:13]
    nsplit = _lib.lib_raw().tce_groupnorm_nsplit(h * w_)
    w = dense(_p(ws), T * G * (nsplit * 3 + 2) * F)
    return ([dense(_p(x), T * h * w_ * Cn * F), dense(_p(gamma), Cn * F), dense(_p(beta), Cn * F), dense(_p(add), T * ho * wo * Cn * F), w],
            [dense(_p(out), T * ho * wo * Cn * F), w])


def _mask_pack(a):
    params, w0f, tail, nl, T, Q, Cm = a[:7]
    npar = 8 * (Cm + 2) + 64 + 8 + 8 + 8 + 1
    return [dense(_p(params), nl * T * Q * npar * F)], [dense(_p(w0f), T * nl * Q * 8 * Cm * F), dense(_p(tail), nl * T * Q * 112 * F)]


def _mask_tail(a):
    G, tail, refs, ref_ld, masks, nl, T, Q, h, w = a[:10]
    return ([dense(_p(G), T * h * w * nl * Q * 8 * F), dense(_p(tail), nl * T * Q * 112 * F), dense(_p(refs), nl * T * Q * ref_ld * F)],
            [dense(_p(masks), nl * T * Q * h * w * F)])


def _resize(a):
    src, add, out, T, h, w, ho, wo, Cn = a[:9]
    rd = [dense(_p(src), T * h * w * Cn * F)]
    if add:
        rd.append(dense(_p(add), T * ho * wo * Cn * F))
    return rd, [dense(_p(out), T * ho * wo * Cn * F)]


def _resize_ln(a):
    src, add, gamma, beta, _, out, T, h, w, ho, wo, Cn = a[:12]
    return ([dense(_p(src), T * h * w * Cn * F), dense(_p(add), T * ho * wo * Cn * F), dense(_p(gamma), Cn * F), dense(_p(beta), Cn * F)],
            [dense(_p(out), T * ho * wo * Cn * F)])


def _win(a, rows):
    qkv, qb, table, out, T, H, W, Cn, nH = a[:9]
    return ([dense(_p(qkv), T * H * W * 3 * Cn * F), dense(_p(qb), 3 * Cn * F), dense(_p(table), rows * nH * F)],
            [dense(_p(out), T * H * W * Cn * F)])


def _embed(ids, pos_ids, word, pos, type0, gamma, beta, out, L, Cn, pad_id, seq_len):
    rd = [dense(_p(ids), L * 8), _table(word, "the word embedding table"), dense(_p(type0), Cn * F), dense(_p(gamma), Cn * F),
          dense(_p(beta), Cn * F)]
    if pos_ids:
        rd += [dense(_p(pos_ids), L * 8), _table(pos, "the position embedding table")]
    else:
        rd.append(dense(_p(pos), (pad_id + seq_len + 1) * Cn * F))
    return rd, [dense(_p(out), L * Cn * F)]


def _pos(a, valid):
    out, add, T, h, w, Fh = a[:6]
    return ([dense(_p(add), 2 * Fh * F)] if add else []), [dense(_p(out), T * h * w * 2 * Fh * F)]


def _label_objects(a):
    objs, n, labels, best, T, Q, K, h, w, H0, W0 = a[:11]
    rd = []
    for i in range(n):
        rd += [dense(_p(objs[i].logits), T * Q * K * F), dense(_p(objs[i].masks), T * Q * h * w * F)]
    return rd, [dense(_p(labels), T * H0 * W0), dense(_p(best), n * 4)]


def _a2d_masks(a):
    masks, out, N, h, w, fh, fw, H0, W0 = a[:9]
    return [dense(_p(masks), N * h * w * F)], [dense(_p(out), N * H0 * W0)]


def _rle_counts(a):
    masks, counts, nruns, ws, P, H, W = a[:7]
    wsb = dense(_p(ws), _lib.lib_raw().tce_rle_ws_bytes(P, H, W))
    return [dense(_p(masks), P * H * W), wsb], [dense(_p(counts), P * (H * W + 1) * 4), dense(_p(nruns), P * 4), wsb]


def _jf_counts(a):
    pred, gt, counts, ws, T, n, H, W, radius = a[:9]
    wsb = dense(_p(ws), _lib.lib_raw().tce_jf_ws_bytes(T, n, H, W, radius))
    return [dense(_p(pred), T * H * W), dense(_p(gt), T * H * W), wsb], [dense(_p(counts), n * T * 6 * 4), wsb]


def _rle_decode(a):
    counts, nruns, out, ws, P, H, W, stride = a[:8]
    wsb = dense(_p(ws), _lib.lib_raw().tce_rle_decode_ws_bytes(P, H, W, stride))
    return [dense(_p(counts), P * stride * 4), dense(_p(nruns), P * 4), wsb], [dense(_p(out), P * H * W), wsb]


def _mask_overlap(a):
    pred, gt, counts, ws, N, H, W = a[:7]
    wsb = dense(_p(ws), _lib.lib_raw().tce_mask_overlap_ws_bytes(N, H, W))
    return [dense(_p(pred), N * H * W), dense(_p(gt), H * W), wsb], [dense(_p(counts), N * 3 * 4), wsb]


def _png_deflate(a):
    planes, streams, nbytes, ws, P, H, W, S = a[:8]
    L = _lib.lib_raw()
    wsb = dense(_p(ws), L.tce_png_ws_bytes(P, H, W, S))
    return [dense(_p(planes), P * H * W), wsb], [dense(_p(streams), P * L.tce_png_stream_bound(H, W, S)), dense(_p(nbytes), P * 4), wsb]


def _png_filter_rgb(a):
    img, rows, P, H, W = a[:5]
    return [dense(_p(img), P * H * W * 3)], [dense(_p(rows), P * H * (3 * W + 1))]


def _png_deflate_rows(a):
    rows, streams, nbytes, ws, P, H, R, S = a[:8]
    L = _lib.lib_raw()
    wsb = dense(_p(ws), L.tce_png_ws_bytes(P, H, R - 1, S))
    return [dense(_p(rows), P * H * R), wsb], [dense(_p(streams), P * L.tce_png_stream_bound(H, R - 1, S)), dense(_p(nbytes), P * 4), wsb]


def _vis_overlay(a):
    frames, out, masks, boxes, points, colors, L, N, H0, W0 = a[:10]
    return ([dense(_p(frames), N * H0 * W0 * 3), dense(_p(masks), L * N * H0 * W0), dense(_p(boxes), L * N * 4 * F),
             dense(_p(points), L * N * 2 * F), dense(_p(colors), L * 3)], [dense(_p(out), N * H0 * W0 * 3)])


def _a2d_group_masks(a):
    samples, B, N, h, w = a[:5]
    rd, wr = [], []
    for b in range(B):
        e = samples[b]
        rd += [dense(_p(e.masks), N * h * w * F), strided(_p(e.logits), F, (N, e.logit_stride * F))]
        wr += [dense(_p(e.out), N * e.H0 * e.W0), dense(_p(e.scores), N * F)]
    return rd, wr


def _png_file(a):
    streams, nbytes, head, head_bytes, files, file_bytes, ws, P, sstride, fstride = a[:10]
    L = _lib.lib_raw()
    wsb = dense(_p(ws), L.tce_png_file_ws_bytes(P, sstride))
    return ([dense(_p(streams), P * sstride), dense(_p(nbytes), P * 4), dense(_p(head), head_bytes), wsb],
            [strided(_p(files), L.tce_png_file_bound(head_bytes, sstride), (P, fstride)), dense(_p(file_bytes), P * 4), wsb])


def _refexp_group(a):
    samples, B, Q, K, h, w = a[:6]
    rd, wr = [], []
    for b in range(B):
        e = samples[b]
        if _p(e.logits):
            rd += [dense(_p(e.logits), Q * K * F), dense(_p(e.boxes_in), Q * 4 * F)]
            wr += [dense(_p(e.scores), Q * F), dense(_p(e.order), Q * 4), dense(_p(e.boxes_out), Q * 4 * F)]
        else:
            rd.append(dense(_p(e.order), Q * 4))
        if _p(e.masks) and _p(e.out):
            rd.append(dense(_p(e.masks), Q * h * w * F))
            wr.append(dense(_p(e.out), Q * e.H0 * e.W0))
    return rd, wr


def _refexp_giou(a):
    boxes, gt, giou, best, M, Q = a[:6]
    return [dense(_p(boxes), M * Q * 4 * F), dense(_p(gt), M * 4 * F)], [dense(_p(giou), M * Q * F), dense(_p(best), M * Q * F)]


MODELS = {
    "tce_gemm_f32": lambda a: _gemm(_st(a[0])),
    "tce_gemm_splitk_f32": lambda a: _gemm(_st(a[0]), ws=a[2], splits=a[1]),
    "tce_gemm_splitk_ln_f32": lambda a: _gemm(_st(a[0]), ws=a[2], splits=a[1], ln=(a[3], a[4])),
    "tce_layernorm_f32": lambda a: ([dense(_p(a[0]), a[5] * a[6] * F), dense(_p(a[1]), a[5] * a[6] * F), dense(_p(a[2]), a[6] * F),
                                     dense(_p(a[3]), a[6] * F)], [dense(_p(a[4]), a[5] * a[6] * F)]),
    "tce_groupnorm_f32": _groupnorm,
    "tce_groupnorm_up_add_f32": _groupnorm_up_add,
    "tce_resnet_stem_f32": lambda a: ([dense(_p(a[0]), a[4] * 3 * a[5] * a[6] * F), dense(_p(a[1]), 147 * 64 * F), dense(_p(a[2]), 64 * F)],
                                      [dense(_p(a[3]), a[4] * ((a[5] - 1) // 2 + 1) * ((a[6] - 1) // 2 + 1) * 64 * F)]),
    "tce_maxpool3x3s2_cl_f32": lambda a: ([dense(_p(a[0]), a[2] * a[3] * a[4] * a[5] * F)],
                                          [dense(_p(a[1]), a[2] * ((a[3] - 1) // 2 + 1) * ((a[4] - 1) // 2 + 1) * a[5] * F)]),
    "tce_patch_embed_f32": lambda a: ([dense(_p(a[0]), a[6] * 3 * a[7] * a[8] * F), dense(_p(a[1]), a[9] * 48 * F),
                                       dense(_p(a[2]), a[9] * F), dense(_p(a[3]), a[9] * F), dense(_p(a[4]), a[9] * F)],
                                      [dense(_p(a[5]), a[6] * ((a[7] + 3) // 4) * ((a[8] + 3) // 4) * a[9] * F)]),
    "tce_window_attn_f32": lambda a: _win(a, 169),
    "tce_window_attn3d_f32": lambda a: _win(a, 15 * 169),
    "tce_patch_merge_ln_f32": lambda a: ([dense(_p(a[0]), a[4] * a[5] * a[6] * a[7] * F), dense(_p(a[1]), 4 * a[7] * F),
                                          dense(_p(a[2]), 4 * a[7] * F)],
                                         [dense(_p(a[3]), a[4] * ((a[5] + 1) // 2) * ((a[6] + 1) // 2) * 4 * a[7] * F)]),
    "tce_mha_f32": lambda a: _mha(a[0], a[1], a[2], a[3], None, *a[4:17]),
    "tce_mha_ws_f32": lambda a: _mha(a[0], a[1], a[2], a[3], a[4], *a[5:18]),
    "tce_ms_deform_attn_forward_f32": lambda a: (
        [dense(_p(a[0]), a[6] * a[7] * a[8] * a[9] * F), dense(_p(a[1]), a[11] * 16), dense(_p(a[2]), a[11] * 8),
         dense(_p(a[3]), a[6] * a[10] * a[8] * a[11] * a[12] * 2 * F), dense(_p(a[4]), a[6] * a[10] * a[8] * a[11] * a[12] * F)],
        [dense(_p(a[5]), a[6] * a[10] * a[8] * a[9] * F)]),
    "tce_ms_deform_attn_backward_f32": lambda a: (
        [dense(_p(a[0]), a[9] * a[10] * a[11] * a[12] * F), dense(_p(a[1]), a[14] * 16), dense(_p(a[2]), a[14] * 8),
         dense(_p(a[3]), a[9] * a[13] * a[11] * a[14] * a[15] * 2 * F),
         dense(_p(a[4]), a[9] * a[13] * a[11] * a[14] * a[15] * F), dense(_p(a[5]), a[9] * a[13] * a[11] * a[12] * F)],
        [dense(_p(a[6]), a[9] * a[10] * a[11] * a[12] * F), dense(_p(a[7]), a[9] * a[13] * a[11] * a[14] * a[15] * 2 * F),
         dense(_p(a[8]), a[9] * a[13] * a[11] * a[14] * a[15] * F)]),
    "tce_msda_fused_f32": lambda a: _msda(a[0], a[1], a[2], a[3], *a[5:13]),
    "tce_msda_fused_valid_f32": lambda a: _msda(a[0], a[1], a[2], a[3], *a[6:14]),
    "tce_msda_fewq_raw_f32": lambda a: (
        [dense(_p(a[0]), a[8] * a[9] * 256 * F), dense(_p(a[1]), 256 * 256 * F), dense(_p(a[2]), 256 * F),
         dense(_p(a[3]), a[8] * a[11] * a[10] * a[12] * a[13] * 3 * F), dense(_p(a[4]), (a[8] if a[15] else 1) * a[11] * a[14] * F)],
        [dense(_p(a[5]), a[8] * a[11] * 256 * F)]),
    "tce_contrastive_f32": lambda a: ([dense(_p(a[0]), a[4] * a[5] * a[6] * F), dense(_p(a[1]), (a[4] // a[7]) * a[6] * F)],
                                      [dense(_p(a[2]), a[4] * F), dense(_p(a[3]), a[4] * 32 * a[6] * F)]),
    "tce_pos_sine2d_f32": lambda a: _pos(a, False),
    "tce_pos_sine2d_valid_f32": lambda a: _pos(a, True),
    "tce_resize_nearest_f32": _resize,
    "tce_resize_bilinear_f32": _resize,
    "tce_resize_bilinear_ln_f32": _resize_ln,
    "tce_add_f32": lambda a: ([dense(_p(a[0]), a[3] * F), dense(_p(a[1]), a[4] * F)], [dense(_p(a[2]), a[3] * F)]),
    "tce_tile_f32": lambda a: ([dense(_p(a[0]), a[2] * F)], [dense(_p(a[1]), a[2] * a[3] * F)]),
    "tce_sigmoid_f32": lambda a: ([dense(_p(a[0]), a[2] * F)], [dense(_p(a[1]), a[2] * F)]),
    "tce_tanh_f32": lambda a: ([dense(_p(a[0]), a[2] * F)], [dense(_p(a[1]), a[2] * F)]),
    "tce_copy_segments": _copy_segments,
    "tce_box_refine_f32": lambda a: ([dense(_p(a[0]), a[3] * 4 * F), dense(_p(a[1]), a[3] * a[4] * F)], [dense(_p(a[2]), a[3] * 4 * F)]),
    "tce_mask_pack_f32": _mask_pack,
    "tce_mask_tail_f32": _mask_tail,
    "tce_select_masks_u8": lambda a: ([dense(_p(a[0]), a[4] * a[5] * a[6] * F), dense(_p(a[1]), a[4] * a[5] * a[7] * a[8] * F)],
                                      [dense(_p(a[2]), a[4] * a[9] * a[10]), dense(_p(a[3]), 4)]),
    "tce_resize_h_u8": lambda a: ([dense(_p(a[0]), a[4] * a[5] * 3), dense(_p(a[1]), a[6] * a[7] * 4), dense(_p(a[2]), a[6] * 8)],
                                  [dense(_p(a[3]), a[4] * a[6] * 3)]),
    "tce_resize_v_norm_f32": lambda a: ([dense(_p(a[0]), a[5] * a[6] * a[7] * 3), dense(_p(a[1]), a[8] * a[9] * 4), dense(_p(a[2]), a[8] * 8),
                                         dense(_p(a[3]), 3 * 256 * F)],
                                        [dense(_p(a[4]), a[5] * 3 * a[8] * a[7] * F)]),
    "tce_embed_ln_f32": lambda a: _embed(*a[:10], a[11], a[8]),
    "tce_mha_small64_f32": lambda a: ([dense(_p(a[0]), a[2] * 3 * a[3] * 64 * F)], [dense(_p(a[1]), a[2] * a[3] * 64 * F)]),
    "tce_ffn_pack_f32": lambda a: _ffn_pack(a, False),
    "tce_ffn_pack_batched_f32": lambda a: _ffn_pack(a, True),
    "tce_ffn_fused_f32": _ffn_fused,
    "tce_ffn_fused_split_f32": _ffn_fused_split,
    "tce_xattn_prepare_f32": lambda a: (
        [dense(_p(a[0]), a[9] * a[7] * 256 * F), dense(_p(a[1]), a[9] * a[7] * 256 * F), dense(_p(a[2]), 257 * 256 * F),
         dense(_p(a[3]), 256 * 256 * F)],
        [dense(_p(a[4]), a[9] * 8 * a[8] * 256 * F), dense(_p(a[5]), a[9] * 8 * a[8] * F), dense(_p(a[6]), a[9] * 8 * a[8] * 256 * F)]),
    "tce_xattn_fused_f32": lambda a: _xattn(_st(a[0])),
    "tce_xattn_ffn_fused_f32": lambda a: _xattn_ffn(_st(a[0]), _st(a[1])),
    "tce_ffn_pack_chain_f32": lambda a: _ffn_pack(a, False),
    "tce_xattn_pack_f32": lambda a: (
        [dense(_p(a[0]), a[7] * a[5] * 256 * F), dense(_p(a[1]), a[7] * a[5] * 256 * F), dense(_p(a[2]), 257 * 256 * F), dense(_p(a[3]), 256 * 256 * F)],
        [dense(_p(a[4]), a[7] * _lib.lib_raw().tce_ffn_packed_bytes(256, 8 * a[6]))]),
    "tce_xattn_prepare_lens_f32": lambda a: (
        [dense(_p(a[0]), a[9] * a[7] * 256 * F), dense(_p(a[1]), a[9] * a[7] * 256 * F), dense(_p(a[2]), 257 * 256 * F),
         dense(_p(a[3]), 256 * 256 * F), dense(_p(a[10]), a[9] * 4)],
        [dense(_p(a[4]), a[9] * 8 * a[8] * 256 * F), dense(_p(a[5]), a[9] * 8 * a[8] * F), dense(_p(a[6]), a[9] * 8 * a[8] * 256 * F)]),
    "tce_xattn_pack_lens_f32": lambda a: (
        [dense(_p(a[0]), a[7] * a[5] * 256 * F), dense(_p(a[1]), a[7] * a[5] * 256 * F), dense(_p(a[2]), 257 * 256 * F), dense(_p(a[3]), 256 * 256 * F),
         dense(_p(a[8]), a[7] * 4)],
        [dense(_p(a[4]), a[7] * _lib.lib_raw().tce_ffn_packed_bytes(256, 8 * a[6]))]),
    "tce_rowlin_pack_f32": lambda a: ([strided(_p(a[0]), a[4] * F, (a[3], a[1] * F))],
                                      [dense(_p(a[2]), _lib.lib_raw().tce_rowlin_packed_bytes(a[3], a[4]))]),
    "tce_rowlin_f32": lambda a: _rowlin(_st(a[0])),
    "tce_conv3x3_pack_f32": lambda a: ([dense(_p(a[0]), a[3] * 9 * a[2] * F)],
                                       [dense(_p(a[1]), _lib.lib_raw().tce_conv3x3_packed_bytes(a[2], a[3]))]),
    "tce_conv3x3_f32": lambda a: (
        [strided(_p(a[0]), a[9] * F, (a[6] * a[7] * a[8], a[1] * F)), dense(_p(a[2]), _lib.lib_raw().tce_conv3x3_packed_bytes(a[9], a[10])),
         dense(_p(a[3]), a[10] * F)],
        [strided(_p(a[4]), a[10] * F, (a[6] * a[7] * a[8], a[5] * F))]),
    "tce_conv3x3_split_f32": lambda a: (
        [strided(_p(a[0]), a[9] * F, (a[6] * a[7] * a[8], a[1] * F)), dense(_p(a[2]), _lib.lib_raw().tce_conv3x3_packed_bytes(a[9], a[10])),
         dense(_p(a[3]), a[10] * F)],
        [strided(_p(a[4]), a[10] * F, (a[6] * a[7] * a[8], a[5] * F)),
         dense(_p(a[11]), _lib.lib_raw().tce_conv3x3_split_ws_floats(a[6] * a[7] * a[8], a[9], a[10]) * F)]),
    "tce_fewrow_linear_f32": lambda a: _fewrow(_st(a[0])),
    "tce_thin_partials_f32": lambda a: (
        [(strided(_p(a[0]), a[10] * F, (a[8], a[1] * F)) if a[2] == 0 else dense(_p(a[0]), a[2] * a[8] * a[10] * F)),
         dense(_p(a[3]), a[10] * F), strided(_p(a[5]), a[10] * F, (a[9], a[6] * F))],
        [dense(_p(a[7]), (a[10] // 256) * a[8] * a[9] * F)]),
    "tce_splitk_reduce_f32": lambda a: (
        [dense(_p(a[0]), a[1] * a[2] * a[3] * F), dense(_p(a[4]), a[3] * F), dense(_p(a[11]), a[3] * F), dense(_p(a[12]), a[3] * F)] +
        ([strided(_p(a[6]), a[3] * F, (a[2], a[7] * F))] if a[8] else []),
        [strided(_p(a[9]), a[3] * F, (a[2], a[10] * F))]),
    "tce_mha_small64_splits_f32": lambda a: ([dense(_p(a[0]), a[1] * a[4] * 3 * a[5] * 64 * F), dense(_p(a[2]), 3 * a[5] * 64 * F)],
                                             [dense(_p(a[3]), a[4] * a[5] * 64 * F)]),
    "tce_mha_small64_seqs_f32": lambda a: ([dense(_p(a[0]), a[1] * a[4] * a[5] * 3 * a[6] * 64 * F), dense(_p(a[2]), 3 * a[6] * 64 * F)],
                                           [dense(_p(a[3]), a[4] * a[5] * a[6] * 64 * F)]),
    "tce_mha_small64_lens_f32": lambda a: ([dense(_p(a[0]), a[1] * a[4] * a[5] * 3 * a[6] * 64 * F), dense(_p(a[2]), 3 * a[6] * 64 * F),
                                            dense(_p(a[8]), a[4] * 4)],
                                           [dense(_p(a[3]), a[4] * a[5] * a[6] * 64 * F)]),
    "tce_caption_lens_f32": lambda a: ([dense(_p(a[0]), a[1] * a[2] * 8)],
                                       [dense(_p(a[5]), a[1] * 4), dense(_p(a[6]), a[1] * a[2]), dense(_p(a[7]), a[1] * a[2] * a[4] * F)]),
    "tce_embed_ln_seqs_f32": lambda a: _embed(a[0], None, a[1], a[2], a[3], a[4], a[5], a[6], a[7] * a[8], a[9], a[11], a[8]),
    "tce_swin_attn_pack_f32": lambda a: ([dense(_p(a[0]), 3 * a[3] * a[3] * F), dense(_p(a[1]), a[3] * a[3] * F)],
                                         [dense(_p(a[2]), _lib.lib_raw().tce_swin_attn_packed_bytes(a[3]))]),
    "tce_swin_attn_fused_f32": lambda a: (
        [strided(_p(a[0]), a[14] * F, (a[11] * a[12] * a[13], a[1] * F)), dense(_p(a[2]), _lib.lib_raw().tce_swin_attn_packed_bytes(a[14])),
         dense(_p(a[3]), 3 * a[14] * F), dense(_p(a[4]), a[14] * F), dense(_p(a[5]), 169 * (a[14] // 32) * F),
         dense(_p(a[6]), a[14] * F), dense(_p(a[7]), a[14] * F)],
        [strided(_p(a[9]), a[14] * F, (a[11] * a[12] * a[13], a[10] * F))]),
    "tce_label_objects_u8": _label_objects,
    "tce_a2d_masks_u8": _a2d_masks,
    "tce_rle_counts_u32": _rle_counts,
    "tce_jf_counts_i32": _jf_counts,
    "tce_rle_decode_u8": _rle_decode,
    "tce_mask_overlap_i32": _mask_overlap,
    "tce_png_deflate_u8": _png_deflate,
    "tce_png_deflate_dyn_u8": _png_deflate,
    "tce_a2d_group_masks_u8": _a2d_group_masks,
    "tce_vis_overlay_u8": _vis_overlay,
    "tce_png_filter_rgb_u8": _png_filter_rgb,
    "tce_png_deflate_rows_u8": _png_deflate_rows,
    "tce_png_file_u8": _png_file,
    "tce_refexp_group_u8": _refexp_group,
    "tce_refexp_giou_f32": _refexp_giou,
}

NOT_LAUNCHES = {"tce_abi_version", "tce_last_error", "tce_gemm_select_tile", "tce_gemm_select_tile_ex", "tce_set_gemm_mode", "tce_set_gemm_mode_thread",
                "tce_get_gemm_mode", "tce_set_range_flag", "tce_groupnorm_nsplit", "tce_mha_ws_bytes", "tce_ffn_packed_bytes", "tce_ffn_split_ws_floats", "tce_ffn_split_counters",
                "tce_ffn_set_wg_cap", "tce_ffn_capped_grid",
                "tce_rowlin_packed_bytes", "tce_conv3x3_packed_bytes", "tce_conv3x3_split_ws_floats",
                "tce_conv3x3_split_pieces", "tce_conv3x3_split_kstep", "tce_swin_attn_packed_bytes", "tce_thin_linear_splits", "tce_graph_begin", "tce_graph_end", "tce_graph_launch",
                "tce_graph_destroy", "tce_graph_group", "tce_rle_ws_bytes", "tce_jf_ws_bytes", "tce_rle_decode_ws_bytes", "tce_mask_overlap_ws_bytes",
                "tce_png_stream_bound", "tce_png_ws_bytes", "tce_png_file_bound", "tce_png_file_ws_bytes"} | set(_lib.DEBUG_SIGNATURES)


class Launch:
    __slots__ = ("idx", "name", "stream", "tick", "clock", "reads", "writes", "site")

    def __repr__(self):
        return f"#{self.idx} {self.name} on stream {self.stream:#x} at {self.site}"


class Recorder:

    def __init__(self):
        self.launches = []
        self.clock = {}
        self.events = {}
        self.edges = 0
        self.host_syncs = 0

    def _clk(self, s):
        c = self.clock.get(int(s))
        if c is None:
            c = self.clock[int(s)] = dict(getattr(self, "_future", {}))
        return c

    def launch(self, name, stream, reads, writes, site):
        s = int(stream or 0)
        c = self._clk(s)
        c[s] = c.get(s, 0) + 1
        L = Launch()
        L.idx, L.name, L.stream, L.tick, L.clock = len(self.launches), name, s, c[s], dict(c)
        L.reads, L.writes, L.site = union(*reads), union(*writes), site
        self.launches.append(L)

    def record_event(self, ev, stream):
        self.events[id(ev)] = (ev, dict(self._clk(stream)))

    @staticmethod
    def _merge(c, snap):
        for k, v in snap.items():
            if v > c.get(k, 0):
                c[k] = v

    def wait_event(self, ev, stream):
        ent = self.events.get(id(ev))
        if ent is None:
            return
        self._merge(self._clk(stream), ent[1])
        self.edges += 1

    def host_sync(self, snap=None):
        if snap is None:
            snap = {}
            for c in self.clock.values():
                self._merge(snap, c)
        snap = dict(snap)
        self._future = getattr(self, "_future", {})
        self._merge(self._future, snap)
        for s in list(self.clock):
            self._merge(self.clock[s], snap)
        self.host_syncs += 1

    @staticmethod
    def ordered(a, b):
        return b.clock.get(a.stream, 0) >= a.tick

    def analyse(self, max_report=20):
        L = self.launches
        conflicts, pairs = [], 0
        by_stream = {}
        for x in L:
            by_stream.setdefault(x.stream, []).append(x)
        for j, b in enumerate(L):
            for s, lst in by_stream.items():
                if s == b.stream:
                    continue
                seen = b.clock.get(s, 0)
                for a in lst:
                    if a.idx >= b.idx:
                        break
                    if a.tick <= seen:
                        continue
                    pairs += 1
                    for kind, x, y in (("write/write", a.writes, b.writes), ("write/read", a.writes, b.reads),
                                       ("read/write", a.reads, b.writes)):
                        ov = overlap(x, y)
                        if ov is not None:
                            conflicts.append((kind, a, b, ov))
                            break
        return Report(len(L), len(by_stream), self.edges, self.host_syncs, pairs, conflicts[:max_report], len(conflicts))


class Report:
    def __init__(self, launches, streams, edges, host_syncs, pairs, conflicts, n_conflicts):
        self.launches, self.streams, self.edges, self.host_syncs = launches, streams, edges, host_syncs
        self.unordered_pairs, self.conflicts, self.n_conflicts = pairs, conflicts, n_conflicts

    @property
    def clean(self):
        return self.n_conflicts == 0

    def __str__(self):
        head = (f"hazard check: {self.launches} launches on {self.streams} streams, {self.edges} cross-stream edges, "
                f"{self.host_syncs} host syncs, {self.unordered_pairs} unordered launch pairs compared: "
                f"{'NO conflicting pair (race free)' if self.clean else str(self.n_conflicts) + ' CONFLICTS'}")
        lines = [head]
        for kind, a, b, (lo, hi) in self.conflicts:
            lines.append(f"  {kind} on [{lo:#x}, {hi:#x}) ({hi - lo} bytes):\n    {a}\n    {b}")
        return "\n".join(lines)


def _site():
    best = "?"
    for fr in traceback.extract_stack(limit=24)[:-3]:
        fn = fr.filename.rsplit("/", 1)[-1]
        if fn in ("pipeline.py", "text_encoder.py", "model.py", "video.py", "postprocess.py", "score.py", "a2d_score.py", "png.py", "refexp.py",
                  "refexp_score.py"):
            best = f"{fn}:{fr.lineno} {fr.name}"
    return best


class _LibProxy:

    def __init__(self, real, rec, dry=False):
        self._real, self._rec, self._dry = real, rec, dry

    def __getattr__(self, name):
        fn = getattr(self._real, name)
        if name in NOT_LAUNCHES or not name.startswith("tce_"):
            return fn
        model = MODELS.get(name)
        if model is None:
            raise RuntimeError(f"hazard checker: no access model for {name} (add one to hazard.MODELS)")
        rec, dry = self._rec, self._dry

        def call(*a):
            rd, wr = model(a)
            rec.launch(name, a[-1], rd, wr, _site())
            return 0 if dry else fn(*a)
        return call


@contextlib.contextmanager
def recording(dry=False, tables=()):
    rec = Recorder()
    TABLES.clear()
    TABLES.update({int(t.data_ptr()): int(t.numel() * t.element_size()) for t in tables})
    real = _lib.lib()
    Event, Stream = torch.cuda.Event, torch.cuda.Stream
    ev_record, ev_wait, ev_sync, st_sync, dev_sync = Event.record, Event.wait, Event.synchronize, Stream.synchronize, torch.cuda.synchronize

    def record(self, stream=None):
        stream = torch.cuda.current_stream() if stream is None else stream
        rec.record_event(self, stream.cuda_stream)
        return ev_record(self, stream)

    def wait(self, stream=None):
        stream = torch.cuda.current_stream() if stream is None else stream
        rec.wait_event(self, stream.cuda_stream)
        return ev_wait(self, stream)

    def sync_ev(self):
        r = ev_sync(self)
        ent = rec.events.get(id(self))
        if ent is not None:
            rec.host_sync(ent[1])
        return r

    def sync_st(self):
        r = st_sync(self)
        rec.host_sync(rec._clk(self.cuda_stream))
        return r

    def sync_dev(*a, **k):
        r = dev_sync(*a, **k)
        rec.host_sync()
        return r

    _lib._LIB = _LibProxy(real, rec, dry)
    Event.record, Event.wait, Event.synchronize, Stream.synchronize, torch.cuda.synchronize = record, wait, sync_ev, sync_st, sync_dev
    try:
        yield rec
    finally:
        TABLES.clear()
        _lib._LIB = real
        Event.record, Event.wait, Event.synchronize, Stream.synchronize, torch.cuda.synchronize = ev_record, ev_wait, ev_sync, st_sync, dev_sync
```

### tce-rvos_amd/ops.py

```python
import ctypes as C

import os
import threading

import torch

from ._lib import GemmArgs, check, lib
from .stage_ops import (A2D_GROUP_MAX, LABEL_MAX_OBJS, PNG_FILE_MAX_HEAD, PNG_FILE_MIN_HEAD, PNG_FILE_PIECE, PNG_FILE_SEGMENT,
                        REFEXP_GROUP_MAX, REFEXP_MAX_CAND, VIS_MAX_LAYERS, a2d_group_masks, a2d_masks, jf_counts, label_objects,
                        mask_overlap, png_deflate, png_deflate_rows, png_file, png_filter_rgb, refexp_giou, refexp_group, rle_counts,
                        rle_decode, select_masks, select_window_masks, vis_overlay)
from .train_ops import criterion_head_grads, criterion_mask_grad, criterion_mask_sums, criterion_match_losses

ACT_NONE, ACT_RELU, ACT_GELU, ACT_RELU_AFTER_RES = 0, 1, 2, 3
RES_NONE, RES_ADD, RES_MUL = 0, 1, 2


class Arena:

    ALIGN = 256
    FLAGS = 1 << 14

    def __init__(self, device, nbytes):
        self.device = torch.device(device)
# ... 105 lines not shown
        return self

    def __exit__(self, *exc):
        if self.n != self.prev:
            _ARITH_TL.wg_cap = self.prev
            check(lib().tce_ffn_set_wg_cap(self.prev), "tce_ffn_set_wg_cap")
        return False


def _stream():
    return torch.cuda.current_stream().cuda_stream


FP16_RANGE_LIMIT = 60000.0
_RANGE = {}


class RangeError(RuntimeError):
    pass


def range_flag(device=None):
    dev = torch.device("cuda", torch.cuda.current_device()) if device is None else torch.device(device)
    if dev.index is None:
        dev = torch.device("cuda", torch.cuda.current_device())
    st = _RANGE.get(dev)
    if st is None:
        st = {"flag": torch.zeros(1, dtype=torch.int32, device=dev), "host": torch.zeros(1, dtype=torch.int32).pin_memory(),
              "event": None}
        _RANGE[dev] = st
        check(lib().tce_set_range_flag(st["flag"].data_ptr()), "tce_set_range_flag")
    return st


def range_snapshot_async(device=None):
    st = range_flag(device)
    st["host"].copy_(st["flag"], non_blocking=True)
    st["event"] = torch.cuda.Event()
    st["event"].record()


def range_poll(device=None, wait=False):
    st = range_flag(device)
    ev = st["event"]
    if ev is None:
        return
    if wait:
        ev.synchronize()
    elif not ev.query():
        return
    st["event"] = None
    if int(st["host"][0]) != 0:
        st["flag"].zero_()
        st["host"].zero_()
        raise RangeError("an activation left the fp16 range of the split-fp16 GEMM arithmetic (|x| >= 60000, Inf or NaN) in a "
                         "previous launch: its results are invalid.  Run with ops.set_gemm_mode('f32') (exact fp32 MFMA).")


def check_range(device=None):
    range_snapshot_async(device)
    range_poll(device, wait=True)


def check_weight_range(named_tensors):
    bad = []
    for name, t in named_tensors:
        if t.is_floating_point() and t.numel() and not bool(t.abs().max() < FP16_RANGE_LIMIT):
            bad.append(name)
    if bad and get_gemm_mode() != "f32":
        raise RangeError(f"parameters outside the fp16 range of the split-fp16 GEMM arithmetic (|w| >= {FP16_RANGE_LIMIT:g} or "
                         f"non-finite): {bad[:5]}{'...' if len(bad) > 5 else ''}.  Select the exact fp32 kernels with "
                         f"ops.set_gemm_mode('f32') before loading these weights.")


def _hbm_timed(name, rows, nbytes, go):
    if HBM_PROFILE is None:
        go()
        return
    e0, e1 = torch.cuda.Event(enable_timing=True), torch.cuda.Event(enable_timing=True)
    e0.record()
    go()
    e1.record()
    HBM_PROFILE.append((name, rows, float(nbytes), e0, e1))


def _chk(t, name):
    if t.dtype != torch.float32 or not t.is_cuda:
        raise TypeError(f"{name}: expected a CUDA float32 tensor, got {t.dtype} on {t.device}")


def _rows(t, name):
    _chk(t, name)
    if t.dim() == 2 and t.stride(1) == 1:
        return t.data_ptr(), t.shape[0], t.shape[1], t.stride(0)
    if not t.is_contiguous():
        raise ValueError(f"{name}: must be contiguous or a 2-D row-strided view")
    c = t.shape[-1]
    return t.data_ptr(), t.numel() // c, c, c


def gemm(a, w, bias=None, a2=None, act=ACT_NONE, res=None, res_mode=RES_NONE, out=None, alloc=None):
    ap, M, K, lda = _rows(a, "a")
    wp, N, Kw, ldw = _rows(w, "w")
    if K != Kw:
        raise ValueError(f"gemm: K mismatch {K} vs {Kw}")
    if out is None:
        out = alloc(M, N) if alloc else torch.empty(M, N, dtype=torch.float32, device=a.device)
    op, Mo, No, ldc = _rows(out, "out")
    if Mo != M or No != N:
        raise ValueError("gemm: out shape mismatch")
    g = GemmArgs()
    g.A, g.W, g.C = ap, wp, op
    g.M, g.N, g.K = M, N, K
    g.lda, g.ldw, g.ldc = lda, ldw, ldc
    if a2 is not None:
        p2, M2, K2, ld2 = _rows(a2, "a2")
        if M2 != M or K2 != K:
            raise ValueError("gemm: a2 shape mismatch")
        g.A2, g.lda2 = p2, ld2
    if bias is not None:
        _chk(bias, "bias")
        g.bias = bias.data_ptr()
    if res_mode != RES_NONE:
        rp, Mr, Nr, ldr = _rows(res, "res")
        if Mr != M or Nr != N:
            raise ValueError("gemm: res shape mismatch")
        g.res, g.ldres = rp, ldr
    g.act, g.res_mode, g.batch = act, res_mode, 1
    _gemm_launch(g)
    return out


def gemm_batched(a, w, out, bias=None, act=ACT_NONE):
    for t, n in ((a, "a"), (w, "w"), (out, "out")):
        _chk(t, n)
        if not t.is_contiguous() or t.dim() != 3:
            raise ValueError(f"gemm_batched: {n} must be contiguous 3-D")
    B, M, K = a.shape
    _, N, _ = w.shape
    g = GemmArgs()
    g.A, g.W, g.C = a.data_ptr(), w.data_ptr(), out.data_ptr()
    g.M, g.N, g.K = M, N, K
    g.lda, g.ldw, g.ldc = K, K, N
    g.batch = B
    g.sA, g.sW, g.sC = M * K, N * K, M * N
    if bias is not None:
        g.bias, g.sBias = bias.data_ptr(), N
    g.act = act
    _gemm_launch(g)
    return out


def conv2d_cl(x, w_packed, T, H, W, Cin, kh, kw, stride, pad, bias=None, act=ACT_NONE, out=None, alloc=None, res=None,
              res_mode=RES_NONE, splitk=1, ws=None):
    _chk(x, "x")
    _chk(w_packed, "w")
    N = w_packed.shape[0]
    Ho = (H + 2 * pad - kh) // stride + 1
    Wo = (W + 2 * pad - kw) // stride + 1
    M = T * Ho * Wo
    if (kh == 3 and kw == 3 and stride == 1 and pad == 1 and act == ACT_NONE and res_mode == RES_NONE and splitk == 1
            and M >= CONV3_MIN_PIXELS and get_gemm_mode() != "f32"):
        pk = _ROUTES.conv3.get((w_packed.data_ptr(), N, w_packed.shape[1], get_gemm_mode()))
        if pk is not None and x.stride(0) % 4 == 0:
            return conv3x3(x, pk, T, H, W, Cin, N, bias=bias, out=out, alloc=alloc), Ho, Wo
    if out is None:
        out = alloc(M, N) if alloc else torch.empty(M, N, dtype=torch.float32, device=x.device)
    g = GemmArgs()
    g.A, g.W, g.C = x.data_ptr(), w_packed.data_ptr(), out.data_ptr()
    g.M, g.N, g.K = M, N, kh * kw * Cin
    g.lda, g.ldw, g.ldc = Cin, kh * kw * Cin, N
    if bias is not None:
        g.bias = bias.data_ptr()
    if res_mode != RES_NONE:
        _chk(res, "res")
        g.res, g.ldres = res.data_ptr(), N
    g.act, g.res_mode, g.batch, g.conv = act, res_mode, 1, 1
    g.T, g.H, g.Wd, g.Cin, g.Ho, g.Wo = T, H, W, Cin, Ho, Wo
    g.kh, g.kw, g.stride, g.pad = kh, kw, stride, pad
    _gemm_launch(g, splitk, ws)
    return out, Ho, Wo


def layernorm(x, gamma, beta, eps=1e-5, r=None, out=None, alloc=None):
    _chk(x, "x")
    Cn = x.shape[-1]
    M = x.numel() // Cn
    if out is None:
        out = alloc(*x.shape) if alloc else torch.empty_like(x)
    check(lib().tce_layernorm_f32(x.data_ptr(), r.data_ptr() if r is not None else None, gamma.data_ptr(),
                                  beta.data_ptr(), out.data_ptr(), M, Cn, eps, _stream()), "tce_layernorm_f32")
    return out


def groupnorm_cl(x, gamma, beta, T, HW, Cn, G, eps=1e-5, relu=False, out=None, ws=None, alloc=None):
    _chk(x, "x")
    nsplit = lib().tce_groupnorm_nsplit(HW)
    if ws is None:
        ws = alloc(T * G * (nsplit * 3 + 2)) if alloc else torch.empty(T * G * (nsplit * 3 + 2), dtype=torch.float32, device=x.device)
    if out is None:
        out = alloc(T * HW, Cn) if alloc else torch.empty(T * HW, Cn, dtype=torch.float32, device=x.device)
    _hbm_timed("groupnorm (stats + apply)", T * HW, 3.0 * T * HW * Cn * 4, lambda: check(
        lib().tce_groupnorm_f32(x.data_ptr(), gamma.data_ptr(), beta.data_ptr(), out.data_ptr(), ws.data_ptr(), T, HW, Cn, G, eps,
                                1 if relu else 0, _stream()), "tce_groupnorm_f32"))
    return out


GN_UP_FUSE = os.environ.get("TCE_GN_UP_FUSE", "1") != "0"


def groupnorm_up_add(x, gamma, beta, T, h, w, ho, wo, Cn, G, add, out, eps=1e-5, relu=True, ws=None, alloc=None):
    _chk(x, "x")
    nsplit = lib().tce_groupnorm_nsplit(h * w)
    if ws is None:
        ws = alloc(T * G * (nsplit * 3 + 2)) if alloc else torch.empty(T * G * (nsplit * 3 + 2), dtype=torch.float32, device=x.device)
    check(lib().tce_groupnorm_up_add_f32(x.data_ptr(), gamma.data_ptr(), beta.data_ptr(), add.data_ptr(), out.data_ptr(), ws.data_ptr(),
                                         T, h, w, ho, wo, Cn, G, eps, 1 if relu else 0, _stream()), "tce_groupnorm_up_add_f32")
    return out


def resnet_stem(frames, w_k64, bias, out=None, alloc=None):
    _chk(frames, "frames")
    T, c3, H, W = frames.shape
    if c3 != 3 or not frames.is_contiguous():
        raise ValueError("resnet_stem: frames must be contiguous [T,3,H,W]")
    Ho, Wo = (H - 1) // 2 + 1, (W - 1) // 2 + 1
    if out is None:
        out = alloc(T * Ho * Wo, 64) if alloc else torch.empty(T * Ho * Wo, 64, dtype=torch.float32, device=frames.device)
    check(lib().tce_resnet_stem_f32(frames.data_ptr(), w_k64.data_ptr(), bias.data_ptr(), out.data_ptr(), T, H, W,
                                    _stream()), "tce_resnet_stem_f32")
    return out, Ho, Wo


def maxpool3x3s2_cl(x, T, H, W, Cn, out=None, alloc=None):
    _chk(x, "x")
    Ho, Wo = (H - 1) // 2 + 1, (W - 1) // 2 + 1
    if out is None:
        out = alloc(T * Ho * Wo, Cn) if alloc else torch.empty(T * Ho * Wo, Cn, dtype=torch.float32, device=x.device)
    check(lib().tce_maxpool3x3s2_cl_f32(x.data_ptr(), out.data_ptr(), T, H, W, Cn, _stream()), "tce_maxpool3x3s2_cl_f32")
    return out, Ho, Wo


def patch_embed(frames, w, b, gamma, beta, eps=1e-5, out=None, alloc=None):
    _chk(frames, "frames")
    T, c3, H, W = frames.shape
    if c3 != 3 or not frames.is_contiguous():
        raise ValueError("patch_embed: frames must be contiguous [T,3,H,W]")
    Cn = w.shape[0]
    Hp, Wp = (H + 3) // 4, (W + 3) // 4
    if out is None:
        out = alloc(T * Hp * Wp, Cn) if alloc else torch.empty(T * Hp * Wp, Cn, dtype=torch.float32, device=frames.device)
    _hbm_timed("patch_embed", T * Hp * Wp, 4.0 * (T * 3 * H * W + T * Hp * Wp * Cn), lambda: check(
        lib().tce_patch_embed_f32(frames.data_ptr(), w.data_ptr(), b.data_ptr(), gamma.data_ptr(), beta.data_ptr(), out.data_ptr(),
                                  T, H, W, Cn, eps, _stream()), "tce_patch_embed_f32"))
    return out, Hp, Wp


def window_attn(qkv, qkv_bias, table, T, H, W, Cn, nH, shift, out=None, alloc=None):
    _chk(qkv, "qkv")
    if out is None:
        out = alloc(T * H * W, Cn) if alloc else torch.empty(T * H * W, Cn, dtype=torch.float32, device=qkv.device)
    _hbm_timed("window_attn", T * H * W, 4.0 * T * H * W * 4 * Cn, lambda: check(
        lib().tce_window_attn_f32(qkv.data_ptr(), qkv_bias.data_ptr(), table.data_ptr(), out.data_ptr(), T, H, W, Cn, nH, shift,
                                  _stream()), "tce_window_attn_f32"))
    return out


def window_attn3d(qkv, qkv_bias, table, T, H, W, Cn, nH, shifted, out=None, alloc=None):
    _chk(qkv, "qkv")
    if out is None:
        out = alloc(T * H * W, Cn) if alloc else torch.empty(T * H * W, Cn, dtype=torch.float32, device=qkv.device)
    check(lib().tce_window_attn3d_f32(qkv.data_ptr(), qkv_bias.data_ptr(), table.data_ptr(), out.data_ptr(), T, H, W,
                                      Cn, nH, 1 if shifted else 0, _stream()), "tce_window_attn3d_f32")
    return out


def patch_merge_ln(x, gamma, beta, T, H, W, Cn, eps=1e-5, out=None, alloc=None):
    _chk(x, "x")
    H2, W2 = (H + 1) // 2, (W + 1) // 2
    if out is None:
        out = alloc(T * H2 * W2, 4 * Cn) if alloc else torch.empty(T * H2 * W2, 4 * Cn, dtype=torch.float32, device=x.device)
    check(lib().tce_patch_merge_ln_f32(x.data_ptr(), gamma.data_ptr(), beta.data_ptr(), out.data_ptr(), T, H, W, Cn, eps,
                                       _stream()), "tce_patch_merge_ln_f32")
    return out, H2, W2


SWIN_FUSED_C = (96, 128, 192, 256)
SWIN_FUSED = os.environ.get("TCE_SWIN_FUSED", "1") != "0"


def swin_attn_pack(wqkv, wproj):
    _chk(wqkv, "wqkv")
    _chk(wproj, "wproj")
    Cn = wproj.shape[0]
    nbytes = lib().tce_swin_attn_packed_bytes(Cn)
    if nbytes < 0 or tuple(wqkv.shape) != (3 * Cn, Cn) or tuple(wproj.shape) != (Cn, Cn):
        raise ValueError(f"swin_attn_pack: unsupported shapes {tuple(wqkv.shape)}, {tuple(wproj.shape)}")
    out = torch.empty(nbytes, dtype=torch.uint8, device=wqkv.device)
    check(lib().tce_swin_attn_pack_f32(wqkv.contiguous().data_ptr(), wproj.contiguous().data_ptr(), out.data_ptr(), Cn, _stream()),
          "tce_swin_attn_pack_f32")
    return out


def swin_attn_fused(x, pk, qkv_bias, proj_bias, table, g1, b1, T, H, W, Cn, shift, eps=1e-5, out=None):
    _chk(x, "x")
    if out is None:
        out = x
    ldx = x.stride(0) if x.dim() == 2 else Cn
    ldo = out.stride(0) if out.dim() == 2 else Cn

    def go():
        check(lib().tce_swin_attn_fused_f32(x.data_ptr(), ldx, pk.data_ptr(), qkv_bias.data_ptr(), proj_bias.data_ptr(), table.data_ptr(),
                                            g1.data_ptr(), b1.data_ptr(), eps, out.data_ptr(), ldo, T, H, W, Cn, shift, _stream()),
              "tce_swin_attn_fused_f32")
    if GEMM_PROFILE is None:
        go()
        return out
    e0, e1 = torch.cuda.Event(enable_timing=True), torch.cuda.Event(enable_timing=True)
    e0.record()
    go()
    e1.record()
    nwin = T * ((H + 6) // 7) * ((W + 6) // 7)
    GEMM_PROFILE.append((f"swin_attn_fused_kernel<{Cn}", False, 8.0 * T * H * W * Cn * Cn + 4.0 * nwin * 49 * 49 * Cn, e0, e1))
    return out


_MHA_SPLIT_OFF = os.environ.get("TCE_MHA_SPLIT", "1") == "0"
_mha_split_applied = False


def _apply_mha_split():
    global _mha_split_applied
    if not _mha_split_applied:
        _mha_split_applied = True
        if _MHA_SPLIT_OFF:
            lib().tce_debug_mha_set_split(0)


MHA_WS_MIN_KEYS = int(os.environ.get("TCE_MHA_WS_MIN_KEYS", 1024))


def mha_core(q, k, v, batch, nheads, Lq, Lk, ldq, ldk, ldv, sQ, sK, sV, out, ldo, sO, kmask=None, scale=None, alloc=None):
    if scale is None:
        scale = 32 ** -0.5
    _apply_mha_split()
    if alloc is not None and Lk >= MHA_WS_MIN_KEYS and get_gemm_mode() != "f32":
        ws = alloc(lib().tce_mha_ws_bytes(batch, nheads, Lk) // 4)
        check(lib().tce_mha_ws_f32(q.data_ptr(), k.data_ptr(), v.data_ptr(), out.data_ptr(), ws.data_ptr(), batch, nheads, Lq, Lk,
                                   ldq, ldk, ldv, ldo, sQ, sK, sV, sO, kmask.data_ptr() if kmask is not None else None, scale,
                                   _stream()), "tce_mha_ws_f32")
        return out
    check(lib().tce_mha_f32(q.data_ptr(), k.data_ptr(), v.data_ptr(), out.data_ptr(), batch, nheads, Lq, Lk, ldq, ldk,
                            ldv, ldo, sQ, sK, sV, sO, kmask.data_ptr() if kmask is not None else None, scale,
                            _stream()), "tce_mha_f32")
    return out


def caption_lens(ids, pad_id, alloc, D=256):
    if ids.dtype != torch.int64 or ids.dim() != 2 or not ids.is_contiguous():
        raise ValueError("caption_lens: contiguous int64 ids [G, Lmax]")
    G, Lmax = int(ids.shape[0]), int(ids.shape[1])
    lens, kmask, pos = alloc(G, dtype=torch.int32), alloc(G, Lmax, dtype=torch.uint8), alloc(G * Lmax, D)
    check(lib().tce_caption_lens_f32(ids.data_ptr(), G, Lmax, int(pad_id), D, lens.data_ptr(), kmask.data_ptr(), pos.data_ptr(),
                                     _stream()), "tce_caption_lens_f32")
    return lens, kmask, pos

# ... 413 lines not shown
    ldo = out.stride(0) if out.dim() == 2 else Cn
    gi, bi = (ln_in[0].data_ptr(), ln_in[1].data_ptr()) if ln_in is not None else (None, None)
    go, bo = (ln_out[0].data_ptr(), ln_out[1].data_ptr()) if ln_out is not None else (None, None)
    def go_():
        if split is not None:
            ws, cnt = split
            assert cnt.dtype == torch.int32 and ws.dtype == torch.float32
            check(lib().tce_ffn_fused_split_f32(x.data_ptr(), ldx, packed.data_ptr(), b2.data_ptr(), gi, bi, eps_in, go, bo, eps_out,
                                                out.data_ptr(), ldo, M, Cn, Hd, act, ws.data_ptr(), ws.numel(), cnt.data_ptr(),
                                                cnt.numel(), _stream()), "tce_ffn_fused_split_f32")
            return
        check(lib().tce_ffn_fused_f32(x.data_ptr(), ldx, packed.data_ptr(), b2.data_ptr(), gi, bi, eps_in, go, bo, eps_out,
                                      out.data_ptr(), ldo, M, Cn, Hd, act, _stream()), "tce_ffn_fused_f32")
    if GEMM_PROFILE is None:
        go_()
        return out
    e0, e1 = torch.cuda.Event(enable_timing=True), torch.cuda.Event(enable_timing=True)
    e0.record()
    go_()
    e1.record()
    GEMM_PROFILE.append((f"ffn_fused_kernel<{Cn}", False, 4.0 * M * Cn * Hd, e0, e1))
    return out


class Routes:
    def __init__(self):
        self.rowlin = {}
        self.conv3 = {}
        self.keep = []

    def clear(self):
        self.rowlin.clear()
        self.conv3.clear()
        del self.keep[:]


DEFAULT_ROUTES = Routes()
_ROUTES = DEFAULT_ROUTES


class routes:

    def __init__(self, r):
        self.r, self.prev = r, None

    def __enter__(self):
        global _ROUTES
        self.prev, _ROUTES = _ROUTES, (self.r if self.r is not None else DEFAULT_ROUTES)
        return self

    def __exit__(self, *exc):
        global _ROUTES
        _ROUTES = self.prev
        return False


def current_routes():
    return _ROUTES


ROWLIN_MIN_ROWS = int(os.environ.get("TCE_ROWLIN_MIN_ROWS", 12000))
ROWLIN384_MAX_ROWS = int(os.environ.get("TCE_ROWLIN384_MAX_ROWS", 12000))
ROWLIN_K = (96, 128, 192, 256) + ((384,) if os.environ.get("TCE_ROWLIN_K384", "1") != "0" else ()) \
    + ((512,) if os.environ.get("TCE_ROWLIN_K512", "1") != "0" else ())


def rowlin_pack(w, N=None, K=None, ldw=None):
    _chk(w, "w")
    N = w.shape[0] if N is None else N
    K = w.shape[1] if K is None else K
    ldw = w.stride(0) if ldw is None else ldw
    nbytes = lib().tce_rowlin_packed_bytes(N, K)
    if nbytes < 0:
        raise ValueError(f"rowlin_pack: unsupported shape N={N} K={K}")
    out = torch.empty(nbytes, dtype=torch.uint8, device=w.device)
    check(lib().tce_rowlin_pack_f32(w.data_ptr(), ldw, out.data_ptr(), N, K, _stream()), "tce_rowlin_pack_f32")
    return out


def rowlin_register(w, table=None):
    if w.dim() != 2 or w.stride(1) != 1 or w.shape[1] not in ROWLIN_K or w.shape[0] % 32 or not w.is_cuda:
        return None
    r = _ROUTES if table is None else table
    key = (w.data_ptr(), w.shape[0], w.shape[1], w.stride(0), get_gemm_mode())
    if key not in r.rowlin:
        r.rowlin[key] = rowlin_pack(w)
        r.keep.append(w)
    return r.rowlin[key]


def rowlin(x, pk, out, M, N, K, ldx, ldo, bias=None, a2=None, lda2=0, a2_rows=0, act=ACT_NONE, res=None, ldres=0,
           res_mode=RES_NONE, ln_in=None, ln_out=None, eps_in=1e-5, eps_out=1e-5, batch=1, sX=0, sA2=0, sRes=0, sOut=0):
    from ._lib import RowLinArgs
    q = RowLinArgs()
    q.x, q.packed, q.out = x.data_ptr(), pk.data_ptr(), out.data_ptr()
    q.M, q.N, q.K, q.batch = M, N, K, batch
    q.ldx, q.ldo = ldx, ldo
    if a2 is not None:
        q.a2, q.lda2, q.a2_rows = a2.data_ptr(), lda2, a2_rows
    if bias is not None:
        q.bias = bias.data_ptr()
    if res_mode != RES_NONE:
        q.res, q.ldres = res.data_ptr(), ldres
    if ln_in is not None:
        q.g_in, q.be_in = ln_in[0].data_ptr(), ln_in[1].data_ptr()
    if ln_out is not None:
        q.g_out, q.be_out = ln_out[0].data_ptr(), ln_out[1].data_ptr()
    q.act, q.res_mode, q.eps_in, q.eps_out = act, res_mode, eps_in, eps_out
    q.sX, q.sA2, q.sRes, q.sOut = sX, sA2, sRes, sOut

    def go():
        check(lib().tce_rowlin_f32(C.byref(q), _stream()), "tce_rowlin_f32")
    if GEMM_PROFILE is None:
        go()
        return out
    e0, e1 = torch.cuda.Event(enable_timing=True), torch.cuda.Event(enable_timing=True)
    e0.record()
    go()
    e1.record()
    GEMM_PROFILE.append((f"rowlin_kernel<{K}", False, 2.0 * M * N * K * batch, e0, e1))
    return out


CONV3_MIN_PIXELS = int(os.environ.get("TCE_CONV3_MIN_PIXELS", 12000))
CONV3_SPLIT = os.environ.get("TCE_CONV3_SPLIT", "1") != "0"


def conv3x3_split_ws_floats(M, Cin=256, N=256):
    return int(lib().tce_conv3x3_split_ws_floats(M, Cin, N)) if CONV3_SPLIT else 0


def conv3x3_pack(w_cl, Cin):
    _chk(w_cl, "w")
    N = w_cl.shape[0]
    nbytes = lib().tce_conv3x3_packed_bytes(Cin, N)
    if nbytes < 0 or w_cl.shape[1] != 9 * Cin or not w_cl.is_contiguous():
        raise ValueError(f"conv3x3_pack: unsupported shape N={N} Cin={Cin}")
    out = torch.empty(nbytes, dtype=torch.uint8, device=w_cl.device)
    check(lib().tce_conv3x3_pack_f32(w_cl.data_ptr(), out.data_ptr(), Cin, N, _stream()), "tce_conv3x3_pack_f32")
    return out


def conv3x3_register(w_cl, Cin, table=None):
    if lib().tce_conv3x3_packed_bytes(Cin, w_cl.shape[0]) < 0 or w_cl.shape[1] != 9 * Cin:
        return None
    r = _ROUTES if table is None else table
    key = (w_cl.data_ptr(), w_cl.shape[0], w_cl.shape[1], get_gemm_mode())
    if key not in r.conv3:
        r.conv3[key] = conv3x3_pack(w_cl, Cin)
        r.keep.append(w_cl)
    return r.conv3[key]


def conv3x3(x, pk, T, H, W, Cin, N, bias=None, out=None, alloc=None):
    _chk(x, "x")
    M = T * H * W
    if out is None:
        out = alloc(M, N) if alloc else torch.empty(M, N, dtype=torch.float32, device=x.device)

    nws = conv3x3_split_ws_floats(M, Cin, N) if alloc else 0
    ws = alloc(nws) if nws else None

    def go():
        bp = bias.data_ptr() if bias is not None else None
        if ws is not None:
            check(lib().tce_conv3x3_split_f32(x.data_ptr(), x.stride(0), pk.data_ptr(), bp, out.data_ptr(), out.stride(0), T, H, W,
                                              Cin, N, ws.data_ptr(), nws, _stream()), "tce_conv3x3_split_f32")
        else:
            check(lib().tce_conv3x3_f32(x.data_ptr(), x.stride(0), pk.data_ptr(), bp, out.data_ptr(), out.stride(0), T, H, W, Cin,
                                        N, _stream()), "tce_conv3x3_f32")
    if GEMM_PROFILE is None:
        go()
        return out
    e0, e1 = torch.cuda.Event(enable_timing=True), torch.cuda.Event(enable_timing=True)
    e0.record()
    go()
    e1.record()
    GEMM_PROFILE.append((f"conv3x3_kernel<{Cin}", True, 2.0 * M * N * 9 * Cin, e0, e1))
    return out


XATTN_MIN_ROWS = int(os.environ.get("TCE_XATTN_MIN_ROWS", 4000))
XATTN_PACK_FUSED = os.environ.get("TCE_XATTN_PACK_FUSED", "1") != "0"


def xattn_static(wq, bq, scale=32 ** -0.5):
    return (torch.cat([wq.t(), bq[None]], 0) * scale).contiguous()


def xattn_pack(k, v, wqT_ext, wo, L, alloc, group=32, batch=1, lens=None):
    _chk(k, "k")
    _chk(v, "v")
    Hd = 8 * group
    if XATTN_PACK_FUSED:
        pk = alloc(batch, lib().tce_ffn_packed_bytes(256, Hd), dtype=torch.uint8)
        if lens is not None:
            check(lib().tce_xattn_pack_lens_f32(k.data_ptr(), v.data_ptr(), wqT_ext.data_ptr(), wo.data_ptr(), pk.data_ptr(), L, group,
                                                batch, lens.data_ptr(), _stream()), "tce_xattn_pack_lens_f32")
            return pk
        check(lib().tce_xattn_pack_f32(k.data_ptr(), v.data_ptr(), wqT_ext.data_ptr(), wo.data_ptr(), pk.data_ptr(), L, group, batch,
                                       _stream()), "tce_xattn_pack_f32")
        return pk
    W1, b1, W2 = alloc(batch, Hd, 256), alloc(batch, Hd), alloc(batch, 256, Hd)
    if lens is not None:
        check(lib().tce_xattn_prepare_lens_f32(k.data_ptr(), v.data_ptr(), wqT_ext.data_ptr(), wo.data_ptr(), W1.data_ptr(),
                                               b1.data_ptr(), W2.data_ptr(), L, group, batch, lens.data_ptr(), _stream()),
              "tce_xattn_prepare_lens_f32")
    else:
        check(lib().tce_xattn_prepare_f32(k.data_ptr(), v.data_ptr(), wqT_ext.data_ptr(), wo.data_ptr(), W1.data_ptr(), b1.data_ptr(),
                                          W2.data_ptr(), L, group, batch, _stream()), "tce_xattn_prepare_f32")
    nbytes = lib().tce_ffn_packed_bytes(256, Hd)
    pk = alloc(batch, nbytes, dtype=torch.uint8)
    check(lib().tce_ffn_pack_batched_f32(W1.data_ptr(), b1.data_ptr(), W2.data_ptr(), pk.data_ptr(), 256, Hd, batch, _stream()),
          "tce_ffn_pack_batched_f32")
    return pk




def ffn_pack_chain(w1, b1, w2):
    _chk(w1, "w1")
    _chk(w2, "w2")
    Hd, Cn = w1.shape
    nbytes = lib().tce_ffn_packed_bytes(Cn, Hd)
    if Cn != 256 or nbytes < 0 or tuple(w2.shape) != (Cn, Hd):
        raise ValueError(f"ffn_pack_chain: unsupported shape C={Cn} hidden={Hd}")
    out = torch.empty(nbytes, dtype=torch.uint8, device=w1.device)
    check(lib().tce_ffn_pack_chain_f32(w1.contiguous().data_ptr(), b1.contiguous().data_ptr() if b1 is not None else None,
                                       w2.contiguous().data_ptr(), out.data_ptr(), Cn, Hd, _stream()), "tce_ffn_pack_chain_f32")
    return out


def xattn_fused(x, pk, bo, M, out, a2=None, lda2=256, a2_rows=0, res=None, res_mode=RES_ADD, ln_out=None, eps_out=1e-5,
                batch=1, sX=0, sRes=0, sOut=0, ldx=256, ldo=256, ldres=256, group=32, per_batch_weights=False, w_div=1, ffn=None):
    from ._lib import XattnArgs, XattnFfnArgs
    q = XattnArgs()
    q.x, q.packed, q.bo, q.out = x.data_ptr(), pk.data_ptr(), bo.data_ptr(), out.data_ptr()
    q.M, q.batch, q.res_mode, q.eps_out, q.group = M, batch, res_mode, eps_out, group
    q.sW = pk.stride(0) if (per_batch_weights and pk.dim() == 2) else 0
    q.w_div = max(1, int(w_div))
    q.ldx, q.ldo, q.ldres, q.lda2 = ldx, ldo, ldres, lda2
    q.sX, q.sRes, q.sOut = sX, sRes, sOut
    if a2 is not None:
        q.a2, q.a2_rows = a2.data_ptr(), a2_rows
    if res is not None:
        q.res = res.data_ptr()
    if ln_out is not None:
        q.g_out, q.be_out = ln_out[0].data_ptr(), ln_out[1].data_ptr()

    fq = None
    if ffn is not None:
        pk2, b2, hidden, ln2, mid, s_mid = ffn
        fq = XattnFfnArgs()
        fq.packed, fq.b2, fq.mid, fq.ldmid, fq.sMid, fq.hidden, fq.act = pk2.data_ptr(), b2.data_ptr(), mid.data_ptr(), 256, s_mid, hidden, 1
        if ln2 is not None:
            fq.g_out, fq.be_out, fq.eps_out = ln2[0].data_ptr(), ln2[1].data_ptr(), 1e-5

    def go():
        if fq is not None:
            check(lib().tce_xattn_ffn_fused_f32(C.byref(q), C.byref(fq), _stream()), "tce_xattn_ffn_fused_f32")
        else:
            check(lib().tce_xattn_fused_f32(C.byref(q), _stream()), "tce_xattn_fused_f32")
    if GEMM_PROFILE is None:
        go()
        return out
    e0, e1 = torch.cuda.Event(enable_timing=True), torch.cuda.Event(enable_timing=True)
    e0.record()
    go()
    e1.record()
    if fq is not None:
        GEMM_PROFILE.append(("xattn+ffn(ffn_fused_kernel<256,4,3|4,1>", False, 4.0 * M * 256 * (8 * group + hidden) * batch, e0, e1))
    else:
        GEMM_PROFILE.append(("xattn(ffn_fused_kernel<256,4,3|4>", False, 4.0 * M * 256 * 8 * group * batch, e0, e1))
    return out


FEWROW_MAX_ROWS = int(os.environ.get("TCE_FEWROW_MAX_ROWS", 128))
FR_NONE, FR_RELU, FR_SIGMOID, FR_GELU = 0, 1, 2, 3


def fewrow_linear(x, R, K, segs, ldx=None, a2=None, lda2=0, a2_rows=0, res=None, ldres=0, ln_in=None, eps_in=1e-5, xn_out=None):
    from ._lib import FewRowArgs
    q = FewRowArgs()
    if ln_in is not None:
        q.g_in, q.be_in, q.eps_in = ln_in[0].data_ptr(), ln_in[1].data_ptr(), eps_in
        if xn_out is not None:
            q.xn_out, q.ldxn = xn_out.data_ptr(), (xn_out.stride(0) if xn_out.dim() == 2 else K)
    q.x, q.ldx, q.R, q.K, q.nseg = x.data_ptr(), (K if ldx is None else ldx), R, K, len(segs)
    if a2 is not None:
        q.a2, q.lda2, q.a2_rows = a2.data_ptr(), lda2, a2_rows
    if res is not None:
        q.res, q.ldres = res.data_ptr(), ldres
    for i, (W, b, out, N, ldo, use_a2, act) in enumerate(segs):
        sg = q.seg[i]
        sg.W, sg.bias, sg.out = W.data_ptr(), (b.data_ptr() if b is not None else None), out.data_ptr()
        sg.N, sg.ldw, sg.ldo, sg.use_a2, sg.act = N, (W.stride(0) if W.dim() == 2 else K), ldo, 1 if use_a2 else 0, act
    check(lib().tce_fewrow_linear_f32(C.byref(q), _stream()), "tce_fewrow_linear_f32")
```

### tce-rvos_amd/pipeline.py

```python
import os

import torch

from . import ops
from .ops import ACT_GELU, ACT_RELU, ACT_RELU_AFTER_RES, RES_ADD, RES_MUL, gemm_ex

D = 256
NH = 8
FFN_FUSED_MIN_ROWS = int(os.environ.get("TCE_FFN_FUSED_MIN_ROWS", 16000))
SWIN_FUSED_MIN_TOKENS = int(os.environ.get("TCE_SWIN_FUSED_MIN_TOKENS", 2000))


def _proj_res_ln(x, wt, bias, resid, M, norm_w, norm_b):
    pk = ops.rowlin_lookup(wt, D, D) if M >= FFN_FUSED_MIN_ROWS else None
    if pk is not None:
        ops.rowlin(x, pk, resid, M, D, D, D, D, bias=bias, res=resid, ldres=D, res_mode=RES_ADD, ln_out=(norm_w, norm_b))
        return
    gemm_ex(x, wt, resid, M, D, D, D, D, D, bias=bias, res=resid, ldres=D, res_mode=RES_ADD)
    ops.layernorm(resid, norm_w, norm_b, 1e-5, out=resid)


def _lin(A, x, M, K, w, b, N, **kw):
    out = A(M, N)
    gemm_ex(x, w, out, M, N, K, K, K, N, bias=b, **kw)
# ... 870 lines not shown
        if cfg.video:
            feats.append(x if rep == 1 else ops.tile(x, rep, out=out_i))
            finish = None
        else:
            def finish(x=x, i=i, out_i=out_i, ntok=ntok):
                ops.layernorm(x, w[f"{b}norm{i}.weight"], w[f"{b}norm{i}.bias"], out=out_i[:ntok])
                if rep > 1:
                    ops.tile(out_i[:ntok], rep - 1, out=out_i[ntok:])
            if on_stage is None or i not in norm_handed_over:
                finish()
                finish = None
            feats.append(out_i)
        if on_stage is not None:
            on_stage(i, feats[-1], finish)
        if x_next is not None:
            m0 = ar.mark()
            p = f"{b}downsamples.{i}." if cfg.video else f"{b}layers.{i}.downsample."
            xm, _, _ = ops.patch_merge_ln(x, w[p + "norm.weight"], w[p + "norm.bias"], T, H, W, C, alloc=A)
            with model.arith("backbone.merge"):
                gemm_ex(xm, w[p + "reduction.weight"], x_next, x_next.shape[0], 2 * C, 4 * C, 4 * C, 4 * C, 2 * C)
            ar.release(m0)
            x = x_next
            C *= 2
    return feats


def _resnet_backbone(model, frames, ar, sizes, rep=1):
    cfg, w = model.cfg, model._packed
    A = ar.alloc
    T = frames.shape[0]
    b = "backbone.0.body."
    full = [A(rep * T * h * ww, c) for (h, ww), c in zip(sizes, cfg.num_channels)]
    feats = [f[:T * h * ww] for f, (h, ww) in zip(full, sizes)]
    m_all = ar.mark()
    stem, H1, W1 = ops.resnet_stem(frames, w[b + "conv1:f"], w[b + "conv1:b"], alloc=A)
    x, H, W = ops.maxpool3x3s2_cl(stem, T, H1, W1, 64, alloc=A)
    assert (H, W) == tuple(sizes[0])
    cin = 64
    for li, blocks in enumerate(cfg.resnet_blocks):
        width = 64 * 2 ** li
        Ho, Wo = sizes[li]
        for j in range(blocks):
            p = f"{b}layer{li + 1}.{j}."
            stride = 2 if (j == 0 and li > 0) else 1
            out = feats[li] if j == blocks - 1 else A(T * Ho * Wo, 4 * width)
            m0 = ar.mark()
            if j == 0:
                idt, _, _ = ops.conv2d_cl(x, w[p + "downsample.0:f"], T, H, W, cin, 1, 1, stride, 0,
                                          bias=w[p + "downsample.0:b"], alloc=A)
            else:
                idt = x
            y1 = A(T * H * W, width)
            gemm_ex(x, w[p + "conv1:f"], y1, T * H * W, width, cin, cin, cin, width, bias=w[p + "conv1:b"], act=ACT_RELU)
            y2, _, _ = ops.conv2d_cl(y1, w[p + "conv2:f"], T, H, W, width, 3, 3, stride, 1, bias=w[p + "conv2:b"],
                                     act=ACT_RELU, alloc=A)
            gemm_ex(y2, w[p + "conv3:f"], out, T * Ho * Wo, 4 * width, width, width, width, 4 * width,
                    bias=w[p + "conv3:b"], act=ACT_RELU_AFTER_RES, res=idt, ldres=4 * width, res_mode=RES_ADD)
            ar.release(m0)
            x, H, W, cin = out, Ho, Wo, 4 * width
    ar.release(m_all)
    if rep > 1:
        for f, part in zip(full, feats):
            ops.tile(part, rep - 1, out=f[part.shape[0]:])
    return full


def _lateral(c, stage, arx):
    model, cfg, w, sc, T, G, L = c.model, c.cfg, c.w, c.sc, c.T, c.G, c.L
    sizes, S, starts = c.sizes, c.S, c.starts
    pd = "pixel_decoder."
    A = arx.alloc
    h, ww = sizes[stage - 1]
    hw = h * ww
    pos = sc["pos"][stage - 1]
    vis = A(T * hw, D)
    with model.arith("pixel.conv"):
        if stage > 1:
            l = stage - 2
            gemm_ex(c.memory[starts[l]:], w[f"{pd}adapter_{stage}.weight"], vis, hw, D, D, D, D, D, batch=T, sA=S * D,
                    sC=hw * D)
        else:
            c0 = cfg.num_channels[0]
            gemm_ex(c.feats[0], w[f"{pd}adapter_1.weight"], vis, T * hw, D, c0, c0, c0, D)
    m1 = arx.mark()
    tgt = ops.groupnorm_cl(vis, w[f"{pd}adapter_{stage}.norm.weight"], w[f"{pd}adapter_{stage}.norm.bias"], T, hw, D, 8,
                           out=vis, alloc=A)
    arx.release(m1)
    if not cfg.vlblock:
        return tgt
    bp = f"{pd}cross_attn_{stage}."
    pre = bp + "self_attn."
    red = sc["red"].get(stage)
    normed = False
    with model.arith("pixel.attn"):
        m1 = arx.mark()
        if red is not None:
            nh_, nw_, pos_low = red
            n_low = T * nh_ * nw_
            x_low = ops.resize_nearest(tgt, T, h, ww, nh_, nw_, D, alloc=A)
            qk = A(n_low, 2 * D)
            gemm_ex(x_low, w[pre + "qk.w"], qk, nh_ * nw_, 2 * D, D, D, D, 2 * D, bias=w[pre + "qk.b"], a2=pos_low,
                    lda2=D, batch=T, sA=nh_ * nw_ * D, sA2=0, sC=nh_ * nw_ * 2 * D)
            v = _lin(A, x_low, n_low, D, w[pre + "v.w"], w[pre + "v.b"], D)
            att = A(n_low, D)
            nc = n_low // G
            ops.mha_core(qk, qk[:, D:], v, G, NH, nc, nc, 2 * D, 2 * D, D, nc * 2 * D, nc * 2 * D, nc * D, att, D, nc * D, alloc=A,
                         kmask=sc["kmask"].get(stage))
            o_low = _lin(A, att, n_low, D, w[pre + "out_proj.weight"], w[pre + "out_proj.bias"], D)
            ops.resize_bilinear(o_low, T, nh_, nw_, h, ww, D, add=tgt, out=tgt, ln=(w[bp + "norm1.weight"], w[bp + "norm1.bias"]))
            normed = True
        else:
            n = T * hw
            qk = A(n, 2 * D)
            gemm_ex(tgt, w[pre + "qk.w"], qk, hw, 2 * D, D, D, D, 2 * D, bias=w[pre + "qk.b"], a2=pos, lda2=D,
                    batch=T, sA=hw * D, sA2=0, sC=hw * 2 * D)
            v = _lin(A, tgt, n, D, w[pre + "v.w"], w[pre + "v.b"], D)
            att = A(n, D)
            nc = n // G
            ops.mha_core(qk, qk[:, D:], v, G, NH, nc, nc, 2 * D, 2 * D, D, nc * 2 * D, nc * 2 * D, nc * D, att, D, nc * D, alloc=A,
                         kmask=sc["kmask"].get(stage))
            gemm_ex(att, w[pre + "out_proj.weight"], tgt, n, D, D, D, D, D, bias=w[pre + "out_proj.bias"], res=tgt,
                    ldres=D, res_mode=RES_ADD)
        arx.release(m1)
    if not normed:
        c.ln_(tgt, bp + "norm1")
    pre = bp + "multihead_attn."
    with model.arith("pixel.xattn"):
        m1 = arx.mark()
        tk, tv, pk, tkm = c.vl_sites[stage]
        Mc = (T // G) * hw
        if pk is not None:
            ops.xattn_fused(tgt, pk, w[pre + "out_proj.bias"], Mc, tgt, a2=pos, a2_rows=hw,
                            ln_out=(w[bp + "norm2.weight"], w[bp + "norm2.bias"]), batch=G, sX=Mc * D, sOut=Mc * D,
                            per_batch_weights=G > 1)
        else:
            q = A(T * hw, D)
            gemm_ex(tgt, w[pre + "q.w"], q, hw, D, D, D, D, D, bias=w[pre + "q.b"], a2=pos, lda2=D, batch=T, sA=hw * D,
                    sA2=0, sC=hw * D)
            att = A(T * hw, D)
            ops.mha_core(q, tk, tv, G, NH, Mc, L, D, D, D, Mc * D, L * D, L * D, att, D, Mc * D, kmask=tkm)
            _proj_res_ln(att, w[pre + "out_proj.weight"], w[pre + "out_proj.bias"], tgt, T * hw, w[bp + "norm2.weight"],
                         w[bp + "norm2.bias"])
        arx.release(m1)
    c.ffn(tgt, T * hw, bp, norm=bp + "norm3", ar=arx, group="pixel.ffn")
    c.tap(f"vl{stage}", tgt)
    return tgt


def _pixel_decoder(c):
    model, w, ar, T, sizes, lat1, par = c.model, c.w, c.ar, c.T, c.sizes, c.lat1, c.fork3
    A = ar.alloc
    pd = "pixel_decoder."

    def merge_conv(tgt, stage, y, y_hw, due, arx, y_new):
        h, ww = sizes[stage - 1]
        if y is not None:
            if due is not None:
                ops.groupnorm_up_add(y, w[f"{pd}layer_{due}.norm.weight"], w[f"{pd}layer_{due}.norm.bias"], T, y_hw[0], y_hw[1], h, ww,
                                     D, 8, add=tgt, out=tgt, relu=True, alloc=arx.alloc)
            else:
                ops.resize_nearest(y, T, y_hw[0], y_hw[1], h, ww, D, add=tgt, out=tgt)
        if ops.GN_UP_FUSE and stage > 1:
            with model.arith("pixel.conv"):
                ops.conv2d_cl(tgt, w[f"{pd}layer_{stage}.weight:cl"], T, h, ww, D, 3, 3, 1, 1, out=y_new, alloc=arx.alloc)
            return stage
        with model.arith("pixel.conv"):
            conv, _, _ = ops.conv2d_cl(tgt, w[f"{pd}layer_{stage}.weight:cl"], T, h, ww, D, 3, 3, 1, 1, alloc=arx.alloc)
        ops.groupnorm_cl(conv, w[f"{pd}layer_{stage}.norm.weight"], w[f"{pd}layer_{stage}.norm.bias"], T, h * ww, D, 8,
                         relu=True, out=y_new, alloc=arx.alloc)
        return None

    y = y_hw = due = None
    stages = (4, 3, 2, 1)
    if par is not None and par[0][1] is not None and par[1][1] is not None:
        (ar3, st3), (ar4, st4) = par
        ar3.reset()
        ar4.reset()
        fk_l3 = _Fork(st4)
        with fk_l3:
            tgt3 = _lateral(c, 3, ar4)
        fk_c = _Fork(st3)
        with fk_c:
            (h4, w4), (h3, w3) = sizes[3], sizes[2]
            y4, y3 = ar3.alloc(T * h4 * w4, D), ar3.alloc(T * h3 * w3, D)
            tgt4 = _lateral(c, 4, ar3)
            due = merge_conv(tgt4, 4, None, None, None, ar3, y4)
            fk_l3.join()
            due = merge_conv(tgt3, 3, y4, (h4, w4), due, ar3, y3)
        h, ww = sizes[1]
        y2 = A(T * h * ww, D)
        m0 = ar.mark()
        tgt2 = _lateral(c, 2, ar)
        fk_c.join()
        due = merge_conv(tgt2, 2, y3, (h3, w3), due, ar, y2)
        ar.release(m0)
        y, y_hw = y2, (h, ww)
        stages = (1,)
    for stage in stages:
        h, ww = sizes[stage - 1]
        hw = h * ww
        y_new = A(T * hw, D)
        m0 = ar.mark()
        if stage == 1 and lat1 is not None:
            lat1[0].join()
            tgt = lat1[1]
        else:
            tgt = _lateral(c, stage, ar)
        due = merge_conv(tgt, stage, y, y_hw, due, ar, y_new)
        ar.release(m0)
        y, y_hw = y_new, (h, ww)
    assert due is None, f"pixel decoder: the GroupNorm + ReLU of stage {due} was never applied to the map mask_features reads"
    h, ww = sizes[0]
    with model.arith("pixel.conv"):
        out_final, _, _ = ops.conv2d_cl(y, w[pd + "mask_features.weight:cl"], T, h, ww, D, 3, 3, 1, 1,
                                        bias=w[pd + "mask_features.bias"], alloc=A)
    return out_final
```

Baseline: 179.1 clips/s.

## Compute GroupNorm partial statistics in conv3x3 epilogue, skip separate stats pass

The 3x3 conv kernel, and its split-K reduce kernel, now compute per-group mean and M2 partials over 128-pixel granules in the epilogue and write them into a workspace. The following GroupNorm (plain or up-add) consumes these precomputed partials through a one-shot thread-local flag and skips its own statistics kernel, which re-read the whole conv output. This removes one full read pass and one launch per pixel-decoder stage. In exchange the conv epilogue gains extra reductions and barriers, there is a new stateful handoff between API calls, and the hazard model is extended to cover it.

```diff
diff --git a/include/tce_rvos.h b/include/tce_rvos.h
--- a/include/tce_rvos.h
+++ b/include/tce_rvos.h
@@ -47,6 +47,8 @@
 int tce_groupnorm_up_add_f32(const float* x, const float* gamma, const float* beta, const float* add, float* out, float* ws,
                              int32_t T, int32_t h, int32_t w, int32_t ho, int32_t wo, int32_t C, int32_t G, float eps,
                              int32_t relu, tceStream stream);
+int tce_groupnorm_stats_given_next(int32_t nsplit);
+int32_t tce_groupnorm_stats_given_pending(void);
 
 int tce_resnet_stem_f32(const float* frames, const float* w_k64, const float* bias, float* out, int32_t T, int32_t H,
                         int32_t W, tceStream stream);
@@ -204,6 +206,9 @@
 int32_t tce_conv3x3_split_kstep(int32_t pieces, int32_t s);
 int tce_conv3x3_split_f32(const float* x, int64_t ldx, const void* packed, const float* bias, float* out, int64_t ldo, int32_t T,
                           int32_t H, int32_t W, int32_t Cin, int32_t N, float* ws, int64_t ws_floats, tceStream stream);
+int32_t tce_conv3x3_gn_nsplit(int32_t HW);
+int tce_conv3x3_gn_stats_next(float* gn_ws);
+int64_t tce_conv3x3_gn_stats_pending(void);
 
 typedef struct {
   const float* x;
diff --git a/tce-rvos_amd/_lib.py b/tce-rvos_amd/_lib.py
--- a/tce-rvos_amd/_lib.py
+++ b/tce-rvos_amd/_lib.py
@@ -93,6 +93,8 @@
     "tce_groupnorm_nsplit": (i32, [i32]),
     "tce_groupnorm_f32": (i32, [c_f, c_f, c_f, c_f, c_f, i32, i32, i32, i32, f32, i32, c_f]),
     "tce_groupnorm_up_add_f32": (i32, [c_f, c_f, c_f, c_f, c_f, c_f, i32, i32, i32, i32, i32, i32, i32, f32, i32, c_f]),
+    "tce_groupnorm_stats_given_next": (i32, [i32]),
+    "tce_groupnorm_stats_given_pending": (i32, []),
     "tce_resnet_stem_f32": (i32, [c_f, c_f, c_f, c_f, i32, i32, i32, c_f]),
     "tce_maxpool3x3s2_cl_f32": (i32, [c_f, c_f, i32, i32, i32, i32, c_f]),
     "tce_resize_h_u8": (i32, [c_f, c_f, c_f, c_f, i64, i32, i32, i32, c_f]),
@@ -158,6 +160,9 @@
     "tce_conv3x3_split_pieces": (i32, [i32, i32, i32]),
     "tce_conv3x3_split_kstep": (i32, [i32, i32]),
     "tce_conv3x3_split_f32": (i32, [c_f, i64, c_f, c_f, c_f, i64, i32, i32, i32, i32, i32, c_f, i64, c_f]),
+    "tce_conv3x3_gn_nsplit": (i32, [i32]),
+    "tce_conv3x3_gn_stats_next": (i32, [c_f]),
+    "tce_conv3x3_gn_stats_pending": (i64, []),
     "tce_fewrow_linear_f32": (i32, [C.POINTER(FewRowArgs), c_f]),
     "tce_thin_linear_splits": (i32, [i32, i32, i32]),
     "tce_thin_partials_f32": (i32, [c_f, i64, i32, c_f, i32, c_f, i64, c_f, i32, i32, i32, c_f]),
diff --git a/tce-rvos_amd/csrc/conv3x3.hip b/tce-rvos_amd/csrc/conv3x3.hip
--- a/tce-rvos_amd/csrc/conv3x3.hip
+++ b/tce-rvos_amd/csrc/conv3x3.hip
@@ -21,7 +21,32 @@
   int m_off;
   int nb, pieces;
   float* ws;
+  float* gn_ws;
+  int gn_nsp;
 };
+
+constexpr int GN_GRAN = 128;
+__host__ __device__ constexpr int conv3x3_gn_nsp(const int HW) { return (HW + GN_GRAN - 1) / GN_GRAN + 1; }
+
+__device__ __forceinline__ void gn_slot_write(float* __restrict__ ws, const int nsp, const int HW, const int q, const int f, const int g,
+                                              const int cnt, const float mean, const float m2) {
+  const int slot = q - (int)((long long)f * HW / GN_GRAN);
+  float* o = ws + ((long long)(f * 8 + g) * nsp + slot) * 3;
+  o[0] = (float)(cnt * 32);
+  o[1] = mean;
+  o[2] = m2;
+  if ((long long)(f + 1) * HW <= (long long)(q + 1) * GN_GRAN)
+    for (int s = slot + 1; s < nsp; ++s) {
+      o += 3;
+      o[0] = 0.f;
+      o[1] = 0.f;
+      o[2] = 0.f;
+    }
+}
+__device__ __forceinline__ int gn_granule_count(const int gb, const int f, const int HW, const int M) {
+  const long long lo = max((long long)gb, (long long)f * HW), hi = min(min((long long)gb + GN_GRAN, (long long)(f + 1) * HW), (long long)M);
+  return (int)max(hi - lo, 0ll);
+}
 
 constexpr int CONV_ITERS = 12;
 __host__ __device__ constexpr int conv3x3_piece_iter(const int pieces, const int s) { return s * CONV_ITERS / pieces; }
@@ -50,7 +75,7 @@
   constexpr int KS = BODY * ITERS;
   static_assert(CIN % 64 == 0, "channel chunks come in groups of four");
   static_assert(BODY % R == 0 && BODY % XS == 0 && BODY % NW == 0 && LX >= LW, "ring positions are compile-time");
-  static_assert(WAVES * WT_BYTES <= R * STAGE, "the epilogue's staging tiles alias the ring");
+  static_assert(WAVES * WT_BYTES + 2 * WAVES * 8 * 4 <= R * STAGE, "the epilogue's staging tiles and statistics scratch alias the ring");
   static_assert(!SPLIT || (ITERS == CONV_ITERS && WAVES == 4 && !SINGLE), "split pieces: CIN = 256, 128-pixel workgroups, split fp16");
   __shared__ __attribute__((aligned(16))) unsigned char smem[R * STAGE];
 
@@ -234,6 +259,51 @@
     tile_store(acc[t], p.out, p.ldo, m0, p.M, 32 * t, wt, lane, amax);
   }
   tce_range_report(p.range_flag, amax);
+  if (p.gn_ws == nullptr) return;
+  float* const redA = reinterpret_cast<float*>(smem + WAVES * WT_BYTES);
+  float* const redB = redA + WAVES * 8;
+  const int HW = p.H * p.W;
+  const int wg_lo = p.m_off + blk * (32 * WAVES), wg_hi = min(wg_lo + 32 * WAVES, p.M) - 1;
+  const int gw = wave & ~3;
+  const int gb = wg_lo + 32 * gw, q = gb / GN_GRAN;
+  for (int f = wg_lo / HW; f <= wg_hi / HW; ++f) {
+    const bool mine = m >= f * HW && m < min((f + 1) * HW, p.M);
+    const int cnt = gn_granule_count(gb, f, HW, p.M);
+    float s[NTL];
+#pragma unroll
+    for (int t = 0; t < NTL; ++t) {
+      float a = 0.f;
+#pragma unroll
+      for (int i = 0; i < 16; i += 4) a += (acc[t][i] + acc[t][i + 1]) + (acc[t][i + 2] + acc[t][i + 3]);
+      s[t] = wave_sum(mine ? a : 0.f);
+    }
+    if (lane == 0)
+#pragma unroll
+      for (int t = 0; t < NTL; ++t) redA[wave * 8 + t] = s[t];
+    __syncthreads();
+    const float rn = cnt > 0 ? 1.f / (float)(cnt * 32) : 0.f;
+#pragma unroll
+    for (int t = 0; t < NTL; ++t) {
+      const float mean = ((redA[gw * 8 + t] + redA[(gw + 1) * 8 + t]) + (redA[(gw + 2) * 8 + t] + redA[(gw + 3) * 8 + t])) * rn;
+      float a = 0.f;
+#pragma unroll
+      for (int i = 0; i < 16; ++i) {
+        const float d = acc[t][i] - mean;
+        a = fmaf(d, d, a);
+      }
+      s[t] = wave_sum(mine ? a : 0.f);
+    }
+    if (lane == 0)
+#pragma unroll
+      for (int t = 0; t < NTL; ++t) redB[wave * 8 + t] = s[t];
+    __syncthreads();
+    if (wave == gw && lane < 8 && cnt > 0) {
+      const int t = lane;
+      const float mean = ((redA[gw * 8 + t] + redA[(gw + 1) * 8 + t]) + (redA[(gw + 2) * 8 + t] + redA[(gw + 3) * 8 + t])) * rn;
+      const float m2 = (redB[gw * 8 + t] + redB[(gw + 1) * 8 + t]) + (redB[(gw + 2) * 8 + t] + redB[(gw + 3) * 8 + t]);
+      gn_slot_write(p.gn_ws, p.gn_nsp, HW, q, f, t, cnt, mean, m2);
+    }
+  }
 }
 
 __global__ void __launch_bounds__(256) conv3x3_reduce_kernel(const float* __restrict__ ws, const int pieces, const int rows,
@@ -251,6 +321,86 @@
     *reinterpret_cast<f32x4*>(out + (m_off + (i >> 6)) * ldo + 4 * c4) = v;
   }
   tce_range_report(range_flag, amax);
+}
+
+__global__ void __launch_bounds__(256) conv3x3_reduce_stats_kernel(const float* __restrict__ ws, const int pieces, const int rows,
+                                                                   const float* __restrict__ bias, float* __restrict__ out,
+                                                                   const long long ldo, const int m_off, int* range_flag,
+                                                                   float* __restrict__ gn_ws, const int gn_nsp, const int HW) {
+  constexpr int RK = GN_GRAN / 16;
+  __shared__ float redA[4][2], redB[4][2];
+  const int tid = threadIdx.x, lane = tid & 63, wave = tid >> 6;
+  const int c4 = 16 * (int)blockIdx.y + (tid & 15), gl = (tid >> 3) & 1;
+  const int r0 = blockIdx.x * GN_GRAN + (tid >> 4);
+  const long long n4 = (long long)rows * 64;
+  const f32x4* src = reinterpret_cast<const f32x4*>(ws) + c4;
+  f32x4 v[RK];
+#pragma unroll
+  for (int k = 0; k < RK; ++k) v[k] = src[(long long)min(r0 + 16 * k, rows - 1) * 64];
+  for (int s = 1; s < pieces; ++s) {
+    src += n4;
+    f32x4 a[RK];
+#pragma unroll
+    for (int k = 0; k < RK; ++k) a[k] = src[(long long)min(r0 + 16 * k, rows - 1) * 64];
+#pragma unroll
+    for (int k = 0; k < RK; ++k) v[k] += a[k];
+  }
+  if (bias) {
+    const f32x4 bv = reinterpret_cast<const f32x4*>(bias)[c4];
+#pragma unroll
+    for (int k = 0; k < RK; ++k) v[k] += bv;
+  }
+  tce_amax_t amax = 0;
+#pragma unroll
+  for (int k = 0; k < RK; ++k)
+    if (r0 + 16 * k < rows) {
+      amax = tce_amax4(amax, v[k]);
+      *reinterpret_cast<f32x4*>(out + (long long)(m_off + r0 + 16 * k) * ldo + 4 * c4) = v[k];
+    }
+  tce_range_report(range_flag, amax);
+  const int M = m_off + rows, gb = m_off + blockIdx.x * GN_GRAN, q = gb / GN_GRAN;
+  auto group_sum = [](float x) {
+    x += __shfl_xor(x, 1, 64);
+    x += __shfl_xor(x, 2, 64);
+    x += __shfl_xor(x, 4, 64);
+    x += __shfl_xor(x, 16, 64);
+    x += __shfl_xor(x, 32, 64);
+    return x;
+  };
+  for (int f = gb / HW; f <= (min(gb + GN_GRAN, M) - 1) / HW; ++f) {
+    const int cnt = gn_granule_count(gb, f, HW, M);
+    const int f_lo = f * HW, f_hi = min((f + 1) * HW, M);
+    float sm = 0.f;
+#pragma unroll
+    for (int k = 0; k < RK; ++k) {
+      const int m = m_off + r0 + 16 * k;
+      if (m >= f_lo && m < f_hi) sm += (v[k][0] + v[k][1]) + (v[k][2] + v[k][3]);
+    }
+    sm = group_sum(sm);
+    if ((lane & 0x37) == 0) redA[wave][gl] = sm;
+    __syncthreads();
+    const float rn = 1.f / (float)(cnt * 32);
+    const float mean = ((redA[0][gl] + redA[1][gl]) + (redA[2][gl] + redA[3][gl])) * rn;
+    float d2 = 0.f;
+#pragma unroll
+    for (int k = 0; k < RK; ++k) {
+      const int m = m_off + r0 + 16 * k;
+      if (m >= f_lo && m < f_hi) {
+#pragma unroll
+        for (int e = 0; e < 4; ++e) {
+          const float d = v[k][e] - mean;
+          d2 = fmaf(d, d, d2);
+        }
+      }
+    }
+    d2 = group_sum(d2);
+    if ((lane & 0x37) == 0) redB[wave][gl] = d2;
+    __syncthreads();
+    if (tid < 2) {
+      const float mn = ((redA[0][tid] + redA[1][tid]) + (redA[2][tid] + redA[3][tid])) * rn;
+      gn_slot_write(gn_ws, gn_nsp, HW, q, f, 2 * (int)blockIdx.y + tid, cnt, mn, (redB[0][tid] + redB[1][tid]) + (redB[2][tid] + redB[3][tid]));
+    }
+  }
 }
 
 __global__ void __launch_bounds__(256) conv3x3_pack_kernel(const float* __restrict__ w, unsigned char* __restrict__ out,
@@ -366,9 +516,19 @@
   return pieces >= 1 && pieces <= CONV_ITERS && s >= 0 && s <= pieces ? 12 * conv3x3_piece_iter(pieces, s) : -1;
 }
 
+static thread_local float* t_gn_next = nullptr;
+extern "C" int32_t tce_conv3x3_gn_nsplit(int32_t HW) { return HW > 0 ? conv3x3_gn_nsp(HW) : 0; }
+extern "C" int tce_conv3x3_gn_stats_next(float* ws) {
+  t_gn_next = ws;
+  return TCE_OK;
+}
+extern "C" int64_t tce_conv3x3_gn_stats_pending(void) { return (int64_t)(intptr_t)t_gn_next; }
+
 static int conv3x3_launch(const float* x, int64_t ldx, const void* packed, const float* bias, float* out, int64_t ldo, int32_t T,
                           int32_t H, int32_t W, int32_t Cin, int32_t N, float* ws, int64_t ws_floats, const bool split, tceStream stream,
                           const char* name) {
+  float* const gn = t_gn_next;
+  t_gn_next = nullptr;
   TCE_CHECK_ARG(conv3x3_shape_ok(Cin, N), "%s: unsupported shape Cin=%d N=%d (256 -> 256)", name, Cin, N);
   TCE_CHECK_ARG(x && packed && out && T > 0 && H > 0 && W > 0 && (long long)T * H * W < (1ll << 31),
                 "%s: null pointer or bad sizes", name);
@@ -380,6 +540,7 @@
   a.ldx = ldx; a.ldo = ldo; a.H = H; a.W = W; a.M = T * H * W;
   a.range_flag = tce_range_flag(); a.single = tce_gemm_single_pass();
   a.m_off = 0; a.nb = 0; a.pieces = 1; a.ws = nullptr;
+  a.gn_ws = gn; a.gn_nsp = conv3x3_gn_nsp(H * W);
   hipStream_t s = (hipStream_t)stream;
   const Conv3Plan pl = conv3x3_plan_for(a.M, split);
   if (pl.pieces > 1)
@@ -394,7 +555,11 @@
     a.nb = pl.nb; a.pieces = pl.pieces; a.ws = ws;
     hipLaunchKernelGGL((conv3x3_kernel<256, false, 4, true>), dim3(pl.nb * pl.pieces), dim3(256), 0, s, a);
     const int rows = a.M - a.m_off;
-    hipLaunchKernelGGL(conv3x3_reduce_kernel, dim3(std::min(tce_cdiv((long long)rows * 64, 256), 8 * tce_cu_count())), dim3(256), 0, s,
+    if (gn)
+      hipLaunchKernelGGL(conv3x3_reduce_stats_kernel, dim3(tce_cdiv(rows, GN_GRAN), 4), dim3(256), 0, s, (const float*)ws, pl.pieces, rows, bias,
+                         out, ldo, a.m_off, a.range_flag, gn, a.gn_nsp, H * W);
+    else
+      hipLaunchKernelGGL(conv3x3_reduce_kernel, dim3(std::min(tce_cdiv((long long)rows * 64, 256), 8 * tce_cu_count())), dim3(256), 0, s,
                        (const float*)ws, pl.pieces, rows, bias, out, ldo, a.m_off, a.range_flag);
   }
   TCE_CHECK_LAUNCH(name);
diff --git a/tce-rvos_amd/csrc/norm.hip b/tce-rvos_amd/csrc/norm.hip
--- a/tce-rvos_amd/csrc/norm.hip
+++ b/tce-rvos_amd/csrc/norm.hip
@@ -577,17 +577,31 @@
 
 static void groupnorm_stats_launch(const float* x, float* ws, int T, int HW, int C, int G, hipStream_t s);
 
+static thread_local int t_given_nsplit = 0;
+extern "C" int tce_groupnorm_stats_given_next(int32_t nsplit) {
+  TCE_CHECK_ARG(nsplit >= 0, "tce_groupnorm_stats_given_next: nsplit >= 0 (0 clears)");
+  t_given_nsplit = nsplit;
+  return TCE_OK;
+}
+extern "C" int32_t tce_groupnorm_stats_given_pending(void) { return t_given_nsplit; }
+static int groupnorm_take_given() {
+  const int n = t_given_nsplit;
+  t_given_nsplit = 0;
+  return n;
+}
+
 extern "C" int tce_groupnorm_up_add_f32(const float* x, const float* gamma, const float* beta, const float* add, float* out,
                                         float* ws, int32_t T, int32_t h, int32_t w, int32_t ho, int32_t wo, int32_t C, int32_t G,
                                         float eps, int32_t relu, tceStream stream) {
+  const int given = groupnorm_take_given();
   TCE_CHECK_ARG(x && gamma && beta && add && out && ws, "tce_groupnorm_up_add_f32: null pointer");
   TCE_CHECK_ARG(T > 0 && h > 0 && w > 0 && ho > 0 && wo > 0 && C > 0 && G > 0 && G <= 64 && C % G == 0 && C % 4 == 0,
                 "tce_groupnorm_up_add_f32: bad shape (G <= 64)");
   TCE_CHECK_ARG(tce_aligned16(x) && tce_aligned16(out) && tce_aligned16(add), "tce_groupnorm_up_add_f32: x/add/out must be 16-byte aligned");
   TCE_CHECK_ARG(x != out, "tce_groupnorm_up_add_f32: out may alias add, not x");
-  const int HW = h * w, nsplit = tce_cdiv(HW, groupnorm_rows_per(HW));
+  const int HW = h * w, nsplit = given ? given : tce_cdiv(HW, groupnorm_rows_per(HW));
   hipStream_t s = (hipStream_t)stream;
-  groupnorm_stats_launch(x, ws, T, HW, C, G, s);
+  if (!given) groupnorm_stats_launch(x, ws, T, HW, C, G, s);
   const int rows_per_block = 64;
   hipLaunchKernelGGL(groupnorm_apply_up_kernel, dim3(tce_cdiv(ho * wo, rows_per_block), T), dim3(256), (size_t)2 * C * sizeof(float), s,
                      x, ws, gamma, beta, add, out, h, w, ho, wo, C, G, relu, rows_per_block, nsplit, eps);
@@ -609,12 +623,14 @@
 
 extern "C" int tce_groupnorm_f32(const float* x, const float* gamma, const float* beta, float* out, float* ws, int32_t T,
                                  int32_t HW, int32_t C, int32_t G, float eps, int32_t relu, tceStream stream) {
+  const int given = groupnorm_take_given();
   TCE_CHECK_ARG(x && gamma && beta && out && ws, "tce_groupnorm_f32: null pointer");
   TCE_CHECK_ARG(T > 0 && HW > 0 && C > 0 && G > 0 && G <= 64 && C % G == 0 && C % 4 == 0, "tce_groupnorm_f32: bad shape (G <= 64)");
   TCE_CHECK_ARG(tce_aligned16(x) && tce_aligned16(out), "tce_groupnorm_f32: x/out must be 16-byte aligned");
-  const int rows_per = groupnorm_rows_per(HW), nsplit = tce_cdiv(HW, rows_per);
+  const int rows_per = groupnorm_rows_per(HW), nsplit = given ? given : tce_cdiv(HW, rows_per);
   hipStream_t s = (hipStream_t)stream;
-  if (C == 256 && (G == 8 || G == 16 || G == 32 || G == 64)) {
+  if (given) {
+  } else if (C == 256 && (G == 8 || G == 16 || G == 32 || G == 64)) {
     const dim3 grid(nsplit, T);
     if (rows_per == 128) hipLaunchKernelGGL(groupnorm_stats_rows_kernel<32>, grid, dim3(256), 0, s, x, ws, HW, G, rows_per, nsplit);
     else if (rows_per == 32) hipLaunchKernelGGL(groupnorm_stats_rows_kernel<8>, grid, dim3(256), 0, s, x, ws, HW, G, rows_per, nsplit);
diff --git a/tce-rvos_amd/hazard.py b/tce-rvos_amd/hazard.py
--- a/tce-rvos_amd/hazard.py
+++ b/tce-rvos_amd/hazard.py
@@ -226,20 +226,39 @@
     return rd, [dense(_p(packed), b * nb)]
 
 
+def _groupnorm_ws(ws, T, G, HW):
+    given = _lib.lib_raw().tce_groupnorm_stats_given_pending()
+    if given:
+        return [dense(_p(ws), T * G * given * 3 * F)], []
+    w = dense(_p(ws), T * G * (_lib.lib_raw().tce_groupnorm_nsplit(HW) * 3 + 2) * F)
+    return [w], [w]
+
+
 def _groupnorm(a):
     x, gamma, beta, out, ws, T, HW, Cn, G = a[:9]
-    nsplit = _lib.lib_raw().tce_groupnorm_nsplit(HW)
-    w = dense(_p(ws), T * G * (nsplit * 3 + 2) * F)
-    return ([dense(_p(x), T * HW * Cn * F), dense(_p(gamma), Cn * F), dense(_p(beta), Cn * F), w],
-            [dense(_p(out), T * HW * Cn * F), w])
+    wr_, ww_ = _groupnorm_ws(ws, T, G, HW)
+    return ([dense(_p(x), T * HW * Cn * F), dense(_p(gamma), Cn * F), dense(_p(beta), Cn * F)] + wr_,
+            [dense(_p(out), T * HW * Cn * F)] + ww_)
 
 
 def _groupnorm_up_add(a):
     x, gamma, beta, add, out, ws, T, h, w_, ho, wo, Cn, G = a[:13]
-    nsplit = _lib.lib_raw().tce_groupnorm_nsplit(h * w_)
-    w = dense(_p(ws), T * G * (nsplit * 3 + 2) * F)
-    return ([dense(_p(x), T * h * w_ * Cn * F), dense(_p(gamma), Cn * F), dense(_p(beta), Cn * F), dense(_p(add), T * ho * wo * Cn * F), w],
-            [dense(_p(out), T * ho * wo * Cn * F), w])
+    wr_, ww_ = _groupnorm_ws(ws, T, G, h * w_)
+    return ([dense(_p(x), T * h * w_ * Cn * F), dense(_p(gamma), Cn * F), dense(_p(beta), Cn * F), dense(_p(add), T * ho * wo * Cn * F)] + wr_,
+            [dense(_p(out), T * ho * wo * Cn * F)] + ww_)
+
+
+def _conv3x3(a, split):
+    L = _lib.lib_raw()
+    x, ldx, packed, bias, out, ldo, T, H, W, Cin, N = a[:11]
+    rd = [strided(_p(x), Cin * F, (T * H * W, ldx * F)), dense(_p(packed), L.tce_conv3x3_packed_bytes(Cin, N)), dense(_p(bias), N * F)]
+    wr = [strided(_p(out), N * F, (T * H * W, ldo * F))]
+    if split:
+        wr.append(dense(_p(a[11]), L.tce_conv3x3_split_ws_floats(T * H * W, Cin, N) * F))
+    gn = L.tce_conv3x3_gn_stats_pending()
+    if gn:
+        wr.append(dense(gn, T * 8 * L.tce_conv3x3_gn_nsplit(H * W) * 3 * F))
+    return rd, wr
 
 
 def _mask_pack(a):
@@ -479,15 +498,8 @@
     "tce_rowlin_f32": lambda a: _rowlin(_st(a[0])),
     "tce_conv3x3_pack_f32": lambda a: ([dense(_p(a[0]), a[3] * 9 * a[2] * F)],
                                        [dense(_p(a[1]), _lib.lib_raw().tce_conv3x3_packed_bytes(a[2], a[3]))]),
-    "tce_conv3x3_f32": lambda a: (
-        [strided(_p(a[0]), a[9] * F, (a[6] * a[7] * a[8], a[1] * F)), dense(_p(a[2]), _lib.lib_raw().tce_conv3x3_packed_bytes(a[9], a[10])),
-         dense(_p(a[3]), a[10] * F)],
-        [strided(_p(a[4]), a[10] * F, (a[6] * a[7] * a[8], a[5] * F))]),
-    "tce_conv3x3_split_f32": lambda a: (
-        [strided(_p(a[0]), a[9] * F, (a[6] * a[7] * a[8], a[1] * F)), dense(_p(a[2]), _lib.lib_raw().tce_conv3x3_packed_bytes(a[9], a[10])),
-         dense(_p(a[3]), a[10] * F)],
-        [strided(_p(a[4]), a[10] * F, (a[6] * a[7] * a[8], a[5] * F)),
-         dense(_p(a[11]), _lib.lib_raw().tce_conv3x3_split_ws_floats(a[6] * a[7] * a[8], a[9], a[10]) * F)]),
+    "tce_conv3x3_f32": lambda a: _conv3x3(a, False),
+    "tce_conv3x3_split_f32": lambda a: _conv3x3(a, True),
     "tce_fewrow_linear_f32": lambda a: _fewrow(_st(a[0])),
     "tce_thin_partials_f32": lambda a: (
         [(strided(_p(a[0]), a[10] * F, (a[8], a[1] * F)) if a[2] == 0 else dense(_p(a[0]), a[2] * a[8] * a[10] * F)),
@@ -535,6 +547,8 @@
                 "tce_get_gemm_mode", "tce_set_range_flag", "tce_groupnorm_nsplit", "tce_mha_ws_bytes", "tce_ffn_packed_bytes", "tce_ffn_split_ws_floats", "tce_ffn_split_counters",
                 "tce_ffn_set_wg_cap", "tce_ffn_capped_grid",
                 "tce_rowlin_packed_bytes", "tce_conv3x3_packed_bytes", "tce_conv3x3_split_ws_floats",
+                "tce_conv3x3_gn_nsplit", "tce_conv3x3_gn_stats_next", "tce_conv3x3_gn_stats_pending", "tce_groupnorm_stats_given_next",
+                "tce_groupnorm_stats_given_pending",
                 "tce_conv3x3_split_pieces", "tce_conv3x3_split_kstep", "tce_swin_attn_packed_bytes", "tce_thin_linear_splits", "tce_graph_begin", "tce_graph_end", "tce_graph_launch",
                 "tce_graph_destroy", "tce_graph_group", "tce_rle_ws_bytes", "tce_jf_ws_bytes", "tce_rle_decode_ws_bytes", "tce_mask_overlap_ws_bytes",
                 "tce_png_stream_bound", "tce_png_ws_bytes", "tce_png_file_bound", "tce_png_file_ws_bytes"} | set(_lib.DEBUG_SIGNATURES)
@@ -658,6 +672,10 @@
     return best
 
 
+ONE_SHOT = {"tce_conv3x3_f32": "tce_conv3x3_gn_stats_next", "tce_conv3x3_split_f32": "tce_conv3x3_gn_stats_next",
+            "tce_groupnorm_f32": "tce_groupnorm_stats_given_next", "tce_groupnorm_up_add_f32": "tce_groupnorm_stats_given_next"}
+
+
 class _LibProxy:
 
     def __init__(self, real, rec, dry=False):
@@ -671,11 +689,16 @@
         if model is None:
             raise RuntimeError(f"hazard checker: no access model for {name} (add one to hazard.MODELS)")
         rec, dry = self._rec, self._dry
+        disarm = getattr(self._real, ONE_SHOT[name]) if name in ONE_SHOT else None
 
         def call(*a):
             rd, wr = model(a)
             rec.launch(name, a[-1], rd, wr, _site())
-            return 0 if dry else fn(*a)
+            if not dry:
+                return fn(*a)
+            if disarm is not None:
+                disarm(0)
+            return 0
         return call
 
 
diff --git a/tce-rvos_amd/ops.py b/tce-rvos_amd/ops.py
--- a/tce-rvos_amd/ops.py
+++ b/tce-rvos_amd/ops.py
@@ -281,7 +281,7 @@
 
 
 def conv2d_cl(x, w_packed, T, H, W, Cin, kh, kw, stride, pad, bias=None, act=ACT_NONE, out=None, alloc=None, res=None,
-              res_mode=RES_NONE, splitk=1, ws=None):
+              res_mode=RES_NONE, splitk=1, ws=None, gn_stats=None):
     _chk(x, "x")
     _chk(w_packed, "w")
     N = w_packed.shape[0]
@@ -292,7 +292,9 @@
             and M >= CONV3_MIN_PIXELS and get_gemm_mode() != "f32"):
         pk = _ROUTES.conv3.get((w_packed.data_ptr(), N, w_packed.shape[1], get_gemm_mode()))
         if pk is not None and x.stride(0) % 4 == 0:
-            return conv3x3(x, pk, T, H, W, Cin, N, bias=bias, out=out, alloc=alloc), Ho, Wo
+            return conv3x3(x, pk, T, H, W, Cin, N, bias=bias, out=out, alloc=alloc, gn_stats=gn_stats), Ho, Wo
+    if gn_stats is not None:
+        gn_stats[0] = None
     if out is None:
         out = alloc(M, N) if alloc else torch.empty(M, N, dtype=torch.float32, device=x.device)
     g = GemmArgs()
@@ -322,9 +324,20 @@
     return out
 
 
-def groupnorm_cl(x, gamma, beta, T, HW, Cn, G, eps=1e-5, relu=False, out=None, ws=None, alloc=None):
+def _given_stats(stats, T, G, what):
+    ws, nsplit = stats
+    _chk(ws, "stats")
+    if ws.numel() < T * G * nsplit * 3:
+        raise ValueError(f"{what}: {ws.numel()} floats of partials given, {T * G * nsplit * 3} needed")
+    check(lib().tce_groupnorm_stats_given_next(nsplit), "tce_groupnorm_stats_given_next")
+    return ws
+
+
+def groupnorm_cl(x, gamma, beta, T, HW, Cn, G, eps=1e-5, relu=False, out=None, ws=None, alloc=None, stats=None):
     _chk(x, "x")
     nsplit = lib().tce_groupnorm_nsplit(HW)
+    if stats is not None:
+        ws = _given_stats(stats, T, G, "groupnorm_cl")
     if ws is None:
         ws = alloc(T * G * (nsplit * 3 + 2)) if alloc else torch.empty(T * G * (nsplit * 3 + 2), dtype=torch.float32, device=x.device)
     if out is None:
@@ -336,11 +349,14 @@
 
 
 GN_UP_FUSE = os.environ.get("TCE_GN_UP_FUSE", "1") != "0"
-
-
-def groupnorm_up_add(x, gamma, beta, T, h, w, ho, wo, Cn, G, add, out, eps=1e-5, relu=True, ws=None, alloc=None):
+CONV3_GN_STATS = os.environ.get("TCE_CONV3_GN_STATS", "1") != "0"
+
+
+def groupnorm_up_add(x, gamma, beta, T, h, w, ho, wo, Cn, G, add, out, eps=1e-5, relu=True, ws=None, alloc=None, stats=None):
     _chk(x, "x")
     nsplit = lib().tce_groupnorm_nsplit(h * w)
+    if stats is not None:
+        ws = _given_stats(stats, T, G, "groupnorm_up_add")
     if ws is None:
         ws = alloc(T * G * (nsplit * 3 + 2)) if alloc else torch.empty(T * G * (nsplit * 3 + 2), dtype=torch.float32, device=x.device)
     check(lib().tce_groupnorm_up_add_f32(x.data_ptr(), gamma.data_ptr(), beta.data_ptr(), add.data_ptr(), out.data_ptr(), ws.data_ptr(),
@@ -1060,17 +1076,33 @@
     return r.conv3[key]
 
 
-def conv3x3(x, pk, T, H, W, Cin, N, bias=None, out=None, alloc=None):
+def conv3x3_gn_nsplit(HW):
+    return int(lib().tce_conv3x3_gn_nsplit(HW))
+
+
+def conv3x3(x, pk, T, H, W, Cin, N, bias=None, out=None, alloc=None, gn_stats=None):
     _chk(x, "x")
     M = T * H * W
     if out is None:
         out = alloc(M, N) if alloc else torch.empty(M, N, dtype=torch.float32, device=x.device)
+    gws = None
+    if gn_stats is not None:
+        nsp = conv3x3_gn_nsplit(H * W)
+        gws = gn_stats[0]
+        if gws is None:
+            gws = alloc(T * 8 * nsp * 3) if alloc else torch.empty(T * 8 * nsp * 3, dtype=torch.float32, device=x.device)
+        _chk(gws, "gn_stats")
+        if N != 256 or gws.numel() < T * 8 * nsp * 3:
+            raise ValueError("conv3x3: gn_stats needs N = 256 and T * 8 * conv3x3_gn_nsplit(H * W) * 3 floats")
+        gn_stats[0] = (gws, nsp)
 
     nws = conv3x3_split_ws_floats(M, Cin, N) if alloc else 0
     ws = alloc(nws) if nws else None
 
     def go():
         bp = bias.data_ptr() if bias is not None else None
+        if gws is not None:
+            check(lib().tce_conv3x3_gn_stats_next(gws.data_ptr()), "tce_conv3x3_gn_stats_next")
         if ws is not None:
             check(lib().tce_conv3x3_split_f32(x.data_ptr(), x.stride(0), pk.data_ptr(), bp, out.data_ptr(), out.stride(0), T, H, W,
                                               Cin, N, ws.data_ptr(), nws, _stream()), "tce_conv3x3_split_f32")
diff --git a/tce-rvos_amd/pipeline.py b/tce-rvos_amd/pipeline.py
--- a/tce-rvos_amd/pipeline.py
+++ b/tce-rvos_amd/pipeline.py
@@ -1046,22 +1046,31 @@
     A = ar.alloc
     pd = "pixel_decoder."
 
-    def merge_conv(tgt, stage, y, y_hw, due, arx, y_new):
+    gn_st = {}
+
+    def stats_buf(alloc, stage):
         h, ww = sizes[stage - 1]
+        return alloc(T * 8 * ops.conv3x3_gn_nsplit(h * ww) * 3) if ops.CONV3_GN_STATS else None
+
+    def merge_conv(tgt, stage, y, y_hw, due, arx, y_new, st_new=None):
+        h, ww = sizes[stage - 1]
+        box = [st_new] if st_new is not None else None
         if y is not None:
             if due is not None:
                 ops.groupnorm_up_add(y, w[f"{pd}layer_{due}.norm.weight"], w[f"{pd}layer_{due}.norm.bias"], T, y_hw[0], y_hw[1], h, ww,
-                                     D, 8, add=tgt, out=tgt, relu=True, alloc=arx.alloc)
+                                     D, 8, add=tgt, out=tgt, relu=True, alloc=arx.alloc, stats=gn_st.get(due))
             else:
                 ops.resize_nearest(y, T, y_hw[0], y_hw[1], h, ww, D, add=tgt, out=tgt)
         if ops.GN_UP_FUSE and stage > 1:
             with model.arith("pixel.conv"):
-                ops.conv2d_cl(tgt, w[f"{pd}layer_{stage}.weight:cl"], T, h, ww, D, 3, 3, 1, 1, out=y_new, alloc=arx.alloc)
+                ops.conv2d_cl(tgt, w[f"{pd}layer_{stage}.weight:cl"], T, h, ww, D, 3, 3, 1, 1, out=y_new, alloc=arx.alloc, gn_stats=box)
+            if box is not None and box[0] is not None:
+                gn_st[stage] = box[0]
             return stage
         with model.arith("pixel.conv"):
-            conv, _, _ = ops.conv2d_cl(tgt, w[f"{pd}layer_{stage}.weight:cl"], T, h, ww, D, 3, 3, 1, 1, alloc=arx.alloc)
+            conv, _, _ = ops.conv2d_cl(tgt, w[f"{pd}layer_{stage}.weight:cl"], T, h, ww, D, 3, 3, 1, 1, alloc=arx.alloc, gn_stats=box)
         ops.groupnorm_cl(conv, w[f"{pd}layer_{stage}.norm.weight"], w[f"{pd}layer_{stage}.norm.bias"], T, h * ww, D, 8,
-                         relu=True, out=y_new, alloc=arx.alloc)
+                         relu=True, out=y_new, alloc=arx.alloc, stats=box[0] if box is not None else None)
         return None
 
     y = y_hw = due = None
@@ -1077,16 +1086,18 @@
         with fk_c:
             (h4, w4), (h3, w3) = sizes[3], sizes[2]
             y4, y3 = ar3.alloc(T * h4 * w4, D), ar3.alloc(T * h3 * w3, D)
+            s4, s3 = stats_buf(ar3.alloc, 4), stats_buf(ar3.alloc, 3)
             tgt4 = _lateral(c, 4, ar3)
-            due = merge_conv(tgt4, 4, None, None, None, ar3, y4)
+            due = merge_conv(tgt4, 4, None, None, None, ar3, y4, s4)
             fk_l3.join()
-            due = merge_conv(tgt3, 3, y4, (h4, w4), due, ar3, y3)
+            due = merge_conv(tgt3, 3, y4, (h4, w4), due, ar3, y3, s3)
         h, ww = sizes[1]
         y2 = A(T * h * ww, D)
+        s2 = stats_buf(A, 2)
         m0 = ar.mark()
         tgt2 = _lateral(c, 2, ar)
         fk_c.join()
-        due = merge_conv(tgt2, 2, y3, (h3, w3), due, ar, y2)
+        due = merge_conv(tgt2, 2, y3, (h3, w3), due, ar, y2, s2)
         ar.release(m0)
         y, y_hw = y2, (h, ww)
         stages = (1,)
@@ -1094,13 +1105,14 @@
         h, ww = sizes[stage - 1]
         hw = h * ww
         y_new = A(T * hw, D)
+        st_new = stats_buf(A, stage)
         m0 = ar.mark()
         if stage == 1 and lat1 is not None:
             lat1[0].join()
             tgt = lat1[1]
         else:
             tgt = _lateral(c, stage, ar)
-        due = merge_conv(tgt, stage, y, y_hw, due, ar, y_new)
+        due = merge_conv(tgt, stage, y, y_hw, due, ar, y_new, st_new)
         ar.release(m0)
         y, y_hw = y_new, (h, ww)
     assert due is None, f"pixel decoder: the GroupNorm + ReLU of stage {due} was never applied to the map mask_features reads"
```

After: 179.5 clips/s (median of 6 runs). About the same (+0.2%).
